# sephiroce/srf

Hardware: AMD Instinct MI355X
Metric: acoustic frames/sec through SRF (123-d fbank, 3-iter DR) at 1/2/4/8 MI355X (higher is better)
Workload: dtype fp32; 1 GPU; wsj_c4: SRF L=6 PH=CH=16 DIM=32 LPAD=RPAD=2 DR iter=3, train step (fwd+bwd+allreduce+Adam); utterances_per_gpu=28, frames_per_utterance=800, global_batch=28, parallelism=dp1, launch=hipgraph (fwd+CTC+bwd)

## Files before the change

### srf_amd/csrc/route_dr.hip

```cpp
#include <algorithm>
#include <cmath>
#include <type_traits>

#include "srf_common.h"
#include "route_fwd32.h"
#include "../../include/srf.h"
#include "../../include/srf_prof.h"

namespace {

constexpr float kSquashEps = 1e-7f;

thread_local hipEvent_t* t_ev_start = nullptr;
thread_local hipEvent_t* t_ev_stop = nullptr;
thread_local int t_ev_n = 0;
constexpr int MODE_FWD = 0;
constexpr int MODE_BWD = 1;

using srf::DrGeom;

template <int KS>
__device__ __forceinline__ void load_vec(const float* __restrict__ p, float (&v)[KS]) {
  if constexpr (KS % 4 == 0) {
#pragma unroll
// ... 1402 lines not shown
  static_assert(VW == 0 || VW == 2, "0: per-lane loads, 2: image shared by two waves");
  constexpr int D = 32, RV = R - 1, NV = R + RV;
  constexpr int NG = VW == 2 ? 2 : 1;
  constexpr int NT = 256 * NG, CAPW = CAP * NG;
  constexpr int CG = RV * 2 * 4 * 16;
  constexpr int PQ = CG / 4 + 128;
  constexpr int PCB = CG * 4 + 2 * D * 16 * 2;
  constexpr int NQ = (CAPW * PQ + NT - 1) / NT;
  constexpr int IMG = NV * D * 16;
  __shared__ __attribute__((aligned(16))) unsigned char stg[2][CAPW * PCB];
  __shared__ __attribute__((aligned(16))) float vimg[VW == 0 ? 4 : 2 * 4 * IMG];
  const int JD = J * D;
  const size_t FJD = (size_t)F * JD;
  const int Fs = srf::fwd32_frame_stride(F);
  const size_t cblk = (size_t)in_n * JP * Fs;
  const int lane = threadIdx.x & 63, wv = (threadIdx.x >> 6) & 3, wg = threadIdx.x >> 8;
  const int n = lane & 31, h = lane >> 5;
#if SRF_GW16S_XCD
  const int n_cc = (in_n + CAPW - 1) / CAPW, n_tasks = n_cc * n_rt * S;
  const int task = (int)(blockIdx.x & 7) * (int)(gridDim.x >> 3) + (int)(blockIdx.x >> 3);
  if (task >= n_tasks) return;
  const int cc = task % n_cc;
  const int rtg = (task / n_cc) % n_rt;
  const int s = task / n_cc / n_rt;
#else
  int b = blockIdx.x;
  const int s = b % S;
  b /= S;
  const int rtg = b % n_rt;
  const int cc = b / n_rt;
#endif
  const int jw = rtg * 4 + wv;
  const bool wave_on = jw < J;
  const int j = min(jw, J - 1);
  const int row = j * D + n;
  const int Jeff = J - (mask_first ? 1 : 0);
  const float c0 = (wave_on && !(mask_first && j == 0)) ? 1.f / (float)Jeff : 0.f;
  const int i0 = cc * CAPW, ncap = min(in_n, i0 + CAPW) - i0, k0 = wg * CAP;
  const int NFT = Fp >> 4;
  const int ft0 = s * ft_per, ft1 = min(NFT, ft0 + ft_per);
  const int bx = (int)hdr[2];
  const int eg = srf_split_exp(*gumax);
  const float sg = srf_exp2i(eg);

  constexpr int NCPL = CAPW * CG / 4;
  const char* src[NQ];
  int dst[NQ];
  bool cpl[NQ];
#pragma unroll
  for (int q = 0; q < NQ; ++q) {
    const int idx = min(q * NT + (int)threadIdx.x, CAPW * PQ - 1);
    cpl[q] = (q + 1) * NT <= NCPL || (q * NT < NCPL && idx < NCPL);
    if (cpl[q]) {
      const int k = idx / (CG / 4), rem = idx - k * (CG / 4);
      const int i = i0 + min(k, ncap - 1);
      const int fq = rem & 3, jq = (rem >> 2) & 3, cg = rem >> 4;
      const int jj = min(rtg * 4 + jq, JP - 1);
      src[q] = reinterpret_cast<const char*>(((cg & 1) ? glst : cst) + (size_t)(cg >> 1) * cblk +
                                             ((size_t)i * JP + jj) * Fs + 4 * fq);
      dst[q] = k * PCB + rem * 16;
    } else {
      const int x = idx - NCPL, k = x >> 7, xr = x & 127;
      const int p = xr >> 6, e = (xr >> 1) & 31, hf = xr & 1;
      const int i = i0 + min(k, ncap - 1);
      src[q] = reinterpret_cast<const char*>(x16 + (((size_t)i * NFT * 2 + p) * 32 + e) * 16 + hf * 8);
      dst[q] = k * PCB + CG * 4 + p * (D * 16 * 2) + (e * 16 + ((hf ^ ((e >> 3) & 1)) * 8)) * 2;
    }
  }
  f4 sv[NQ];
  auto stage_load = [&](int ft) {
#pragma unroll
    for (int q = 0; q < NQ; ++q) sv[q] = *reinterpret_cast<const f4*>(src[q] + (size_t)ft * (cpl[q] ? 64 : 2 * 32 * 16 * 2));
  };
  auto stage_store = [&](int buf) {
#pragma unroll
    for (int q = 0; q < NQ; ++q) {
      const int idx = q * NT + threadIdx.x;
      if ((CAPW * PQ) % NT != 0 && idx >= CAPW * PQ) continue;
      *reinterpret_cast<f4*>(&stg[buf][dst[q]]) = cpl[q] ? sv[q] * sg : sv[q];
    }
  };
  const uint32_t nrec = (uint32_t)(FJD * 4);
  __amdgpu_buffer_rsrc_t rs_g[R], rs_v[RV];
#pragma unroll
  for (int r = 0; r < R; ++r) {
    rs_g[r] = __builtin_amdgcn_make_buffer_rsrc(const_cast<float*>(gs + (size_t)r * FJD), 0, (int)nrec, 0x00020000);
    if (r > 0)
      rs_v[r - 1] = __builtin_amdgcn_make_buffer_rsrc(const_cast<float*>(saved + (size_t)(2 * (r - 1) + 1) * FJD), 0,
                                                      (int)nrec, 0x00020000);
  }
  const uint32_t vo0 = (uint32_t)((8 * h) * JD + row) * 4;
  f2 nxa[NV][4], nxb[NV][4];
  auto vec_load = [&](f2 (&nx)[NV][4], int ft) {
#pragma unroll
    for (int v = 0; v < 8; ++v) {
      const uint32_t so = (uint32_t)((ft * 16 + v) * JD) * 4;
#pragma unroll
      for (int r = 0; r < R; ++r) {
        nx[r][v >> 1][v & 1] = __builtin_bit_cast(float, __builtin_amdgcn_raw_buffer_load_b32(rs_g[r], vo0, so, 0));
        if (r > 0) nx[R + r - 1][v >> 1][v & 1] = __builtin_bit_cast(float, __builtin_amdgcn_raw_buffer_load_b32(rs_v[r - 1], vo0, so, 0));
      }
    }
  };
  const int rq = lane & 7, fm = lane >> 3;
  const uint32_t wo0 = (uint32_t)((8 * wg + fm) * JD + j * D + 4 * rq) * 4;
  f4 vst[NV];
  auto img_load = [&](int ft) {
    const uint32_t so = (uint32_t)(ft * 16 * JD) * 4;
#pragma unroll
    for (int r = 0; r < R; ++r) {
      vst[r] = __builtin_bit_cast(f4, __builtin_amdgcn_raw_buffer_load_b128(rs_g[r], wo0, so, 0));
      if (r > 0) vst[R + r - 1] = __builtin_bit_cast(f4, __builtin_amdgcn_raw_buffer_load_b128(rs_v[r - 1], wo0, so, 0));
    }
  };
  const int iwo = 4 * rq * 16 + 4 * ((2 * wg + (fm >> 2)) ^ (rq & 3)) + (fm & 3);
  const int iro = n * 16 + 4 * ((2 * h) ^ ((n >> 2) & 3));
  auto img_store = [&](float* im, int v) {
#pragma unroll
    for (int c = 0; c < 4; ++c) im[v * (D * 16) + iwo + c * 16] = vst[v][c];
  };
  auto img_read = [&](const float* im, f2 (&nx)[NV][4]) {
#pragma unroll
    for (int v = 0; v < NV; ++v) {
      const f4 a = ld4(im + v * (D * 16) + iro), b = ld4(im + v * (D * 16) + (iro ^ 4));
      nx[v][0] = f2{a[0], a[1]}, nx[v][1] = f2{a[2], a[3]}, nx[v][2] = f2{b[0], b[1]}, nx[v][3] = f2{b[2], b[3]};
    }
  };

  f16v acc[CAP];
  float gb[CAP];
#pragma unroll
  for (int k = 0; k < CAP; ++k) {
    gb[k] = 0.f;
    acc[k] = f16v{};
  }
  float* const imw = vimg + wv * IMG;
  if (ft0 < ft1) {
    stage_load(ft0);
    if constexpr (VW == 0) vec_load(nxa, ft0);
    else img_load(ft0);
    stage_store(0);
    if (ft0 + 1 < ft1) stage_load(ft0 + 1);
    if constexpr (VW == 2) {
#pragma unroll
      for (int v = 0; v < NV; ++v) img_store(imw, v);
      img_load(min(ft0 + 1, ft1 - 1));
    }
  }
  const int xoff = CG * 4 + (n * 16 + ((h ^ ((n >> 3) & 1)) * 8)) * 2;
  const float s0 = c0 * sg;
  auto caps = [&](int buf, const f2 (&g0)[4], const f2 (&cur)[NV][4], bool img_next) {
    const unsigned char* sb = stg[buf] + k0 * PCB;
#pragma unroll
    for (int k = 0; k < CAP; ++k) {
      const unsigned char* ck = sb + k * PCB;
      const float* ckf = reinterpret_cast<const float*>(ck);
      f2 gu[4];
#pragma unroll
      for (int v = 0; v < 4; ++v) gu[v] = g0[v];
#pragma unroll
      for (int r = 0; r < RV; ++r) {
        const float* cp = ckf + ((r * 2 + 0) * 4 + wv) * 16 + 8 * h;
        const float* gp = ckf + ((r * 2 + 1) * 4 + wv) * 16 + 8 * h;
        const f4 ca = ld4(cp), cb = ld4(cp + 4), ga = ld4(gp), gbv = ld4(gp + 4);
        const f2 c2[4] = {f2{ca[0], ca[1]}, f2{ca[2], ca[3]}, f2{cb[0], cb[1]}, f2{cb[2], cb[3]}};
        const f2 g2[4] = {f2{ga[0], ga[1]}, f2{ga[2], ga[3]}, f2{gbv[0], gbv[1]}, f2{gbv[2], gbv[3]}};
#pragma unroll
        for (int v = 0; v < 4; ++v) {
          gu[v] = __builtin_elementwise_fma(c2[v], cur[r + 1][v], gu[v]);
          gu[v] = __builtin_elementwise_fma(g2[v], cur[R + r][v], gu[v]);
        }
      }
      const f2 gq = (gu[0] + gu[1]) + (gu[2] + gu[3]);
      gb[k] += gq[0] + gq[1];
      h8 bh, bl;
      split8h(gu, bh, bl);
      const h8 xh = *reinterpret_cast<const h8*>(ck + xoff);
      const h8 xl = *reinterpret_cast<const h8*>(ck + xoff + D * 16 * 2);
      acc[k] = mfma32h(xh, bh, acc[k]);
      acc[k] = mfma32h(xh, bl, acc[k]);
      acc[k] = mfma32h(xl, bh, acc[k]);
      if constexpr (VW == 2) {
        if (img_next) {
#pragma unroll
          for (int v = 0; v < NV; ++v)
            if (v * CAP / NV == k) img_store(imw + (buf ^ 1) * (4 * IMG), v);
        }
      }
    }
  };
  auto tile = [&](auto bufc, const f2 (&cur)[NV][4], f2 (&nxt)[NV][4], int ft) {
    constexpr int buf = decltype(bufc)::value;
    f2 g0[4];
#pragma unroll
    for (int v = 0; v < 4; ++v) g0[v] = cur[0][v] * s0;
    __syncthreads();
    if (ft + 1 < ft1) {
      stage_store(buf ^ 1);
      if (ft + 2 < ft1) stage_load(ft + 2);
    }
    vec_load(nxt, ft + 1 < ft1 ? ft + 1 : ft);
    caps(buf, g0, cur, false);
  };
  auto tile_img = [&](auto bufc, int ft) {
    constexpr int buf = decltype(bufc)::value;
    f2 cur[NV][4], g0[4];
    __syncthreads();
    img_read(imw + buf * (4 * IMG), cur);
    if (ft + 1 < ft1) {
      stage_store(buf ^ 1);
      if (ft + 2 < ft1) stage_load(ft + 2);
    }
#pragma unroll
    for (int v = 0; v < 4; ++v) g0[v] = cur[0][v] * s0;
    caps(buf, g0, cur, ft + 1 < ft1);
    __builtin_amdgcn_sched_barrier(0);
    img_load(min(ft + 2, ft1 - 1));
  };
  using S0 = std::integral_constant<int, 0>;
  using S1 = std::integral_constant<int, 1>;
  for (int ft = ft0; ft < ft1; ft += 2) {
    if constexpr (VW == 0) tile(S0{}, nxa, nxb, ft);
    else tile_img(S0{}, ft);
    if (ft + 1 >= ft1) break;
    if constexpr (VW == 0) tile(S1{}, nxb, nxa, ft + 1);
    else tile_img(S1{}, ft + 1);
  }
  float* gw = gwp + (size_t)s * pstride;
  float* gbo = gbp + (size_t)s * pstride;
  const float un = srf_exp2i(-(bx + eg)), ug = srf_exp2i(-eg);
#pragma unroll
  for (int k = 0; k < CAP; ++k) {
    const float a = gb[k];
    float pa, pb;
    xpair32(a, pa, pb);
    if (k0 + k >= ncap || !wave_on) continue;
    const int i = i0 + k0 + k;
    if (h == 0) gbo[(size_t)i * JD + row] = (pa + pb) * ug;
#pragma unroll
    for (int q = 0; q < 4; ++q)
      st4(gw + ((size_t)i * JD + row) * D + 8 * q + 4 * h,
          f4{acc[k][4 * q] * un, acc[k][4 * q + 1] * un, acc[k][4 * q + 2] * un, acc[k][4 * q + 3] * un});
  }
}

__global__ void gw_reduce_kernel(const float* __restrict__ part, int S, size_t n4, size_t stride, float* __restrict__ gW,
                                 size_t nw4, float* __restrict__ gb) {
  const size_t idx = (size_t)blockIdx.x * blockDim.x + threadIdx.x;
  if (idx >= n4) return;
  f4 a = ld4(part + idx * 4);
  for (int s = 1; s < S; ++s) a += ld4(part + (size_t)s * stride + idx * 4);
  if (idx < nw4)
    st4(gW + idx * 4, a);
  else
    st4(gb + (idx - nw4) * 4, a);
}

template <int Q>
__device__ __forceinline__ float qsum(float v) {
#pragma unroll
  for (int o = 1; o < Q; o <<= 1) v += __shfl_xor(v, o, 64);
  return v;
}

struct SlabSplit {
  int n;
  int G, U, in_n, JD;
};

__device__ __forceinline__ int slab_count(const SlabSplit& sp, size_t FJD, size_t off) {
  if (sp.G <= 0) return sp.n;
  const uint32_t f = FJD <= 0xffffffffu ? (uint32_t)off / (uint32_t)sp.JD : (uint32_t)(off / (size_t)sp.JD);
  return srf::bal_tile_slots((int)(f >> 5), sp.in_n, sp.U, sp.G);
}

__device__ __forceinline__ f4 sum_slab4(const float* __restrict__ slab, const SlabSplit& sp, size_t FJD, size_t off) {
  const int n = slab_count(sp, FJD, off);
  f4 a = ld4(slab + off);
#pragma unroll 4
  for (int c = 1; c < n; ++c) a += ld4(slab + (size_t)c * FJD + off);
  return a;
}

template <int DOUT>
__global__ void fwd_finish_kernel(const float* __restrict__ slab, SlabSplit sp, size_t FJD,
                                  const float* __restrict__ vc_in, float* __restrict__ s_out,
                                  float* __restrict__ vc_out, float* __restrict__ v_out) {
  constexpr int Q = DOUT / 4;
  const size_t idx = (size_t)blockIdx.x * blockDim.x + threadIdx.x;
  const bool ok = idx < FJD / 4;
  const size_t off = (ok ? idx : 0) * 4;
  const f4 sv = sum_slab4(slab, sp, FJD, off);
  const float n2 = qsum<Q>((sv.x * sv.x + sv.y * sv.y) + (sv.z * sv.z + sv.w * sv.w));
  if (!ok) return;
  const float fac = n2 / (1.f + n2) / sqrtf(n2 + kSquashEps);
  const f4 v = sv * fac;
  st4(s_out + off, sv);
  if (vc_out) st4(vc_out + off, vc_in ? v + ld4(vc_in + off) : v);
  if (v_out) st4(v_out + off, v);
}

template <int DOUT>
__global__ void bwd_finish_kernel(const float* __restrict__ slab, SlabSplit sp, size_t FJD,
                                  const float* __restrict__ a_init, float* __restrict__ A,
                                  const float* __restrict__ s, float* __restrict__ gs, float* __restrict__ zero4,
                                  size_t nz4, float* __restrict__ zero1) {
  constexpr int Q = DOUT / 4;
  const size_t idx = (size_t)blockIdx.x * blockDim.x + threadIdx.x;
  if (idx < nz4) st4(zero4 + idx * 4, f4{0.f, 0.f, 0.f, 0.f});
  if (zero1 != nullptr && idx == 0) *zero1 = 0.f;
  const bool ok = idx < FJD / 4;
  const size_t off = (ok ? idx : 0) * 4;
  f4 a;
  if (a_init) {
    a = ld4(a_init + off);
    if (ok) st4(A + off, f4{0.f, 0.f, 0.f, 0.f});
  } else {
    a = ld4(A + off) + sum_slab4(slab, sp, FJD, off);
    if (ok) st4(A + off, a);
  }
  const f4 sv = ld4(s + off);
  const float n2 = qsum<Q>((sv.x * sv.x + sv.y * sv.y) + (sv.z * sv.z + sv.w * sv.w));
  const float sa = qsum<Q>((sv.x * a.x + sv.y * a.y) + (sv.z * a.z + sv.w * a.w));
  if (!ok) return;
  const float rs = 1.f / sqrtf(n2 + kSquashEps);
  const float ip = 1.f / (1.f + n2);
  const float gfac = n2 * ip * rs;
  const float dg2 = 2.f * rs * ip * (ip - 0.5f * n2 / (n2 + kSquashEps)) * sa;
  st4(gs + off, a * gfac + sv * dg2);
}

struct PassCfg {
  int TW, NW;
};

PassCfg pass_cfg(const DrGeom& g) {
  const int NT = g.NT();
  int TW = 8;
  int NW = (NT + TW - 1) / TW;
  if (NW > 8) {
    TW = 16;
    NW = (NT + TW - 1) / TW;
  }
  return {TW, NW};
}

int auto_chunks(const DrGeom& g, int NW) {
  const int n_ftiles = (g.F() + 15) / 16;
  const int wg_per_cu = std::max(1, 8 / NW);
  const int slots = 256 * wg_per_cu;
  int best = 1;
  double best_cost = 1e30;
  for (int c = 1; c <= std::min(g.in_n(), 96); ++c) {
    const int rounds = (n_ftiles * c + slots - 1) / slots;
    const int len = (g.in_n() + c - 1) / c;
    double cost = (double)rounds * (len + 2);
    if (8 % c != 0 && c % 8 != 0) cost *= 1.05;
    cost *= 1.0 + 0.002 * c;
    if (cost < best_cost) {
      best_cost = cost;
      best = c;
    }
  }
  return best;
}

template <int D, int TW, int MODE>
void launch_pass(const DrGeom& g, int NW, int n_chunks, const float* emb, const float* W, const float* bias, int r,
                 const float* vc, const float* gsv, float* slab, float* stats, int want_acc, hipStream_t st) {
  const int n_ftiles = (g.F() + 15) / 16;
  const int chunk_len = (g.in_n() + n_chunks - 1) / n_chunks;
  const size_t shmem = (NW > 1) ? (size_t)2 * NW * 48 * sizeof(float) : 16;
  auto kern = r == 0 ? route_pass_kernel<D, D, TW, MODE, true> : route_pass_kernel<D, D, TW, MODE, false>;
  hipLaunchKernelGGL(kern, dim3(n_ftiles * n_chunks), dim3(64 * NW), shmem, st,
                     emb, W, bias, g.F(), g.T, g.N, g.lpad, g.in_n(), g.J, n_chunks, chunk_len, g.mask_first, r,
                     vc, gsv, slab, stats, want_acc);
}

template <int D, int MODE>
void dispatch_pass(const DrGeom& g, const PassCfg& pc, int n_chunks, const float* emb, const float* W,
                   const float* bias, int r, const float* vc, const float* gsv, float* slab, float* stats,
                   int want_acc, hipStream_t st) {
  if (pc.TW == 8)
    launch_pass<D, 8, MODE>(g, pc.NW, n_chunks, emb, W, bias, r, vc, gsv, slab, stats, want_acc, st);
  else
    launch_pass<D, 16, MODE>(g, pc.NW, n_chunks, emb, W, bias, r, vc, gsv, slab, stats, want_acc, st);
}

template <int D>
void launch_fwd_finish(const DrGeom& g, const float* slab, const SlabSplit& sp, const float* vc_in, float* s_out,
                       float* vc_out, float* v_out, hipStream_t st) {
  const size_t FJD = (size_t)g.F() * g.JD();
  hipLaunchKernelGGL((fwd_finish_kernel<D>), dim3((FJD / 4 + 255) / 256), dim3(256), 0, st, slab, sp, FJD,
                     vc_in, s_out, vc_out, v_out);
}

template <int D>
void launch_bwd_finish(const DrGeom& g, const float* slab, const SlabSplit& sp, const float* a_init, float* A,
                       const float* s, float* gs, hipStream_t st, float* zero = nullptr, size_t n_zero = 0,
                       float* zero1 = nullptr) {
  const size_t FJD = (size_t)g.F() * g.JD();
  const size_t nz4 = zero ? n_zero / 4 : 0;
  const size_t n = std::max(FJD / 4, nz4);
  hipLaunchKernelGGL((bwd_finish_kernel<D>), dim3((n + 255) / 256), dim3(256), 0, st, slab, sp, FJD, a_init,
                     A, s, gs, zero, nz4, zero1);
}

constexpr int gu_tw(int d) { return d >= 64 ? 4 : 2; }
constexpr int kGuNW = 4;

inline int gu_wgroups(const DrGeom& g) { return (g.NT() + kGuNW * gu_tw(g.dout) - 1) / (kGuNW * gu_tw(g.dout)); }
inline int padded_frames(const DrGeom& g) { return (g.F() + 15) / 16 * 16; }
inline int gu_window(const DrGeom& g) { return g.lpad + g.rpad + 1; }
inline size_t gu_lds_bytes(const DrGeom& g, int nw, int n_per) {
  return (size_t)nw * (15 + gu_window(g)) * gu_row_stride(n_per, g.din) * sizeof(float);
}
constexpr size_t kGuLdsMax = 64 * 1024;

int gu_n_per(const DrGeom& g, int nw) {
  const int base = (g.F() + 15) / 16 * gu_wgroups(g);
  const int slots = 256 * 4;
  int best = 1;
  double best_cost = 1e30;
  for (int n_per = 1; n_per <= g.N; ++n_per) {
    if (n_per > 1 && gu_lds_bytes(g, nw, n_per) > kGuLdsMax) break;
    const int chunks = (g.N + n_per - 1) / n_per;
    const int rounds = (base * chunks + slots - 1) / slots;
    const double cost = (double)rounds * (gu_window(g) * n_per + 4);
    if (cost < best_cost) {
      best_cost = cost;
      best = n_per;
    }
  }
  return best;
}

inline size_t gux16_lds_bytes(const DrGeom& g, int n_per) {
  return (size_t)kGux16NW * (31 + gu_window(g)) * (n_per * 32 + 4) * sizeof(float);
}
constexpr size_t kGux16LdsMax = (160 / kGux16Occ - 4) * 1024;
int gux16_n_per(const DrGeom& g, int jgpw) {
  const int base = (g.F() + 31) / 32 * ((g.J + kGux16NW - 1) / kGux16NW / jgpw);
  const int slots = 256 * kGux16Occ;
  int best = 1;
  double best_cost = 1e30;
  for (int n_per = 1; n_per <= g.N; ++n_per) {
    if (n_per > 1 && gux16_lds_bytes(g, n_per) > kGux16LdsMax) break;
    const int chunks = (g.N + n_per - 1) / n_per;
    const int rounds = (base * chunks + slots - 1) / slots;
    const double cost = (double)rounds * (gu_window(g) * n_per * jgpw + 4);
    if (cost < best_cost) {
      best_cost = cost;
      best = n_per;
    }
  }
  return best;
}

struct Gw2Plan {
  int cap, n_rt, n_cc, S, ft_per;
  size_t pstride;
};
constexpr int gw3_capsules(int d) { return d <= 16 ? 8 : 4; }

enum class GxPass {
  kRecompute,
  kStored,
  kStored16,
};
enum class GwPass {
  kFromGu,
  kGw2,
  kGw3,
  kGw16s,
};

struct BwdWs {
  size_t A, gs, slab, stats, gu_t, xT, WT;
  size_t gumax;
  size_t p32;
  size_t gl;
  size_t gwpart;
  size_t bytes;
};

struct DrPlan {
  DrGeom g;
  bool fwd32;
  srf::Fwd32Plan p32;
  srf::Fwd32Cpl cpl;
  Gw2Plan gw2;
  bool can_store;
  bool couplings;
  PassCfg pc;
  int chunks;
  int plan_arg;
  GxPass gx;
  GwPass gw;
  size_t fwd_bytes;
  BwdWs ws;
  int JP() const { return p32.JDp / g.dout; }
  const float* hdr(const float* cpl_base) const { return srf::fwd32_hdr(p32, cpl_base + cpl.planes); }
};

#ifndef SRF_GUX16_JGPW
#define SRF_GUX16_JGPW 2
#endif
template <int R>
void launch_gux16(const DrGeom& g, const float* WT, const float* hdr, const float* saved, const float* gs,
                  float* g_emb, const float* cst, const float* glst, int JP, float* gumax, hipStream_t st) {
  const int n_all = (g.J + kGux16NW - 1) / kGux16NW;
  const int jgpw = n_all % SRF_GUX16_JGPW == 0 ? SRF_GUX16_JGPW : 1;
  const int n_wgroups = n_all / jgpw;
  const int n_per = gux16_n_per(g, jgpw);
  const int n_chunks = (g.N + n_per - 1) / n_per;
  int grid = (g.F() + 31) / 32 * n_wgroups * n_chunks;
  if (SRF_GUX16_XCD) grid = (grid + 7) / 8 * 8;
  hipLaunchKernelGGL((route_gux16_kernel<R>), dim3(grid), dim3(64 * kGux16NW), gux16_lds_bytes(g, n_per), st, WT, hdr,
                     g.F(), g.T, g.N, g.lpad, g.in_n(), g.J, g.mask_first, n_wgroups, n_chunks, n_per, saved, gs, g_emb,
                     cst, glst, JP, gumax, jgpw);
}

template <int D, int R>
void launch_gu(const DrPlan& p, const float* emb, const float* W, const float* WT, const float* bias,
               const float* saved, const float* gs, const float* stats, float* gu_t, float* g_emb, hipStream_t st,
               const float* cst, const float* glst, const float* hdr, float* gumax) {
  const DrGeom& g = p.g;
  if constexpr (D == 32 && R >= 2 && R <= 4) {
    if (p.gx == GxPass::kStored16) {
      launch_gux16<R>(g, WT, hdr, saved, gs, g_emb, cst, glst, p.JP(), gumax, st);
      return;
    }
  }
  const int n_ftiles = (g.F() + 15) / 16;
  const int n_wgroups = gu_wgroups(g);
  constexpr int TW = gu_tw(D);
  const int nw = std::min(kGuNW, (g.NT() + TW - 1) / TW);
  const int n_per = gu_n_per(g, nw);
  const int n_chunks = (g.N + n_per - 1) / n_per;
  const int nslots = 15 + gu_window(g);
  const size_t lds = gu_lds_bytes(g, nw, n_per);
  if constexpr (R >= 2 && D <= 32) {
    if (p.gx == GxPass::kStored) {
      hipLaunchKernelGGL((route_gux_kernel<D, TW, R>), dim3(n_ftiles * n_wgroups * n_chunks), dim3(64 * nw), lds, st,
                         WT, g.F(), g.T, g.N, g.lpad, g.in_n(), g.J, g.mask_first, n_wgroups, n_chunks, n_per, saved,
                         gs, g_emb, nslots, cst, glst, p.JP());
      return;
    }
  }
  const bool ldsacc = lds <= kGuLdsMax;
  hipLaunchKernelGGL((ldsacc ? route_gu_kernel<D, D, TW, R, true> : route_gu_kernel<D, D, TW, R, false>),
                     dim3(n_ftiles * n_wgroups * n_chunks), dim3(64 * nw), ldsacc ? lds : 0, st, emb, W, WT, bias, g.F(),
                     padded_frames(g), g.T, g.N, g.lpad, g.rpad, g.in_n(), g.J, g.mask_first, n_wgroups, n_chunks, n_per,
                     saved, gs, stats, gu_t, g_emb, nslots, nullptr, nullptr, 0);
}

template <int V>
using Int = std::integral_constant<int, V>;

template <class Fn>
auto dispatch_iters(int iters, Fn&& fn) {
  switch (iters) {
    case 1: return fn(Int<1>{});
    case 2: return fn(Int<2>{});
    case 3: return fn(Int<3>{});
    case 4: return fn(Int<4>{});
    default: return fn(Int<5>{});
  }
}
template <class Fn>
int dispatch_din(int din, Fn&& fn) {
  switch (din) {
    case 8: return fn(Int<8>{});
    case 16: return fn(Int<16>{});
    case 32: return fn(Int<32>{});
    default: return fn(Int<64>{});
  }
}

template <int D>
int launch_gw2(const DrPlan& pl, const float* xT, const float* saved, const float* gs, const float* cst,
               const float* glst, float* gwp, float* gbp, hipStream_t st, const float* hdr, const float* gumax) {
  static_assert(D <= 32, "couplings are stored by the 32x32 forward");
  const DrGeom& g = pl.g;
  const Gw2Plan& p = pl.gw2;
  const int JP = pl.JP(), Fp = padded_frames(g);
  const int grid = p.n_rt * p.n_cc * p.S;
  if constexpr (D == 32) {
    if (pl.gw == GwPass::kGw16s) {
      constexpr int VW = SRF_GW16S_LDSVEC, NG = VW == 2 ? 2 : 1;
      const int tasks = p.n_rt * ((p.n_cc + NG - 1) / NG) * p.S;
      const int grid16 = SRF_GW16S_XCD ? (tasks + 7) / 8 * 8 : tasks;
      const _Float16* x16 = reinterpret_cast<const _Float16*>(xT);
      hipLaunchKernelGGL((g.iters == 2 ? route_gw16s_kernel<2, kGw16Cap, VW> : route_gw16s_kernel<3, kGw16Cap, VW>),
                         dim3(grid16), dim3(256 * NG), 0, st, x16, hdr, gumax, saved, gs, cst, glst, g.F(), Fp, g.in_n(),
                         g.J, g.mask_first, JP, p.n_rt, p.S, p.ft_per, gwp, gbp, p.pstride);
      SRF_LAUNCH_CHECK("route_gw16s");
      return SRF_OK;
    }
  }
  if (pl.gw == GwPass::kGw3) {
    constexpr int CAP = gw3_capsules(D);
    hipLaunchKernelGGL((g.iters == 2 ? route_gw3_kernel<D, 2, CAP> : route_gw3_kernel<D, 3, CAP>), dim3(grid), dim3(256),
                       0, st, xT, saved, gs, cst, glst, g.F(), Fp, g.in_n(), g.J, g.mask_first, JP, p.n_rt, p.S, p.ft_per,
                       gwp, gbp, p.pstride);
    SRF_LAUNCH_CHECK("route_gw3");
    return SRF_OK;
  }
  hipLaunchKernelGGL((g.iters == 4 ? route_gw2_kernel<D, 4> : route_gw2_kernel<D, 5>), dim3(grid), dim3(256), 0, st, xT,
                     saved, gs, cst, glst, g.F(), Fp, g.in_n(), g.J, g.mask_first, JP, p.n_rt, p.n_cc, p.S, p.ft_per, gwp,
                     gbp, p.pstride);
  SRF_LAUNCH_CHECK("route_gw2");
  return SRF_OK;
}


inline bool use_fwd32(const DrGeom& g) { return srf::fwd32_supported(g.din, g.dout, g.J); }

inline bool use_gux16(const DrGeom& g) {
  return g.din == 32 && g.dout == 32 && g.iters >= 2 && g.iters <= 4 &&
         gux16_lds_bytes(g, 1) <= kGux16LdsMax;
}
inline bool use_gw16s(const DrGeom& g) { return use_gux16(g) && g.iters <= 3; }

inline int gw3_cap(const DrGeom& g) { return g.iters <= 3 && g.din <= 32 ? gw3_capsules(g.din) : 0; }

Gw2Plan gw2_plan(const DrGeom& g, GwPass kind) {
  const bool g16 = kind == GwPass::kGw16s, g3 = kind == GwPass::kGw3;
  Gw2Plan p{};
  const int NT = g.NT();
  const int NCT = g16 ? 2 : (g.din + 15) / 16;
  p.n_rt = g16 ? (g.J + 3) / 4 : (NT + 3) / 4;
  p.cap = g16 ? kGw16Cap : g3 ? gw3_capsules(g.din) : (g.din <= 16 ? 8 : 4);
  const int slots = g16 ? 512 : g3 ? 2 * 768 : 512;
  const double per_tile = g16 ? 120.0 : 200.0;
  p.n_cc = (g.in_n() + p.cap - 1) / p.cap;
  const int NFT = padded_frames(g) / 16;
  p.pstride = (size_t)g.in_n() * g.JD() * (g.din + 1);
  const int base = p.n_rt * p.n_cc;
  double best = 1e30;
  for (int S0 = 1; S0 <= NFT; ++S0) {
    const int ft_per = (NFT + S0 - 1) / S0;
    const int S = (NFT + ft_per - 1) / ft_per;
    const int rounds = (base * S + slots - 1) / slots;
    const double work = (double)rounds * ft_per * p.cap * NCT * per_tile / 2.4e9;
    const double slab = S > 1 ? 2.0 * S * p.pstride * 4 / 4e12 : 0.0;
    if (work + slab < best) {
      best = work + slab;
      p.S = S;
      p.ft_per = ft_per;
    }
  }
  return p;
}

inline bool couplings_ok(const DrGeom& g, const srf::Fwd32Cpl& cpl) {
  if (!use_fwd32(g) || g.iters < 2 || g.din > 32) return false;
  constexpr size_t kLim = size_t(1) << 31;
  const int TW = gu_tw(g.dout);
  const int nw = std::min(kGuNW, (g.NT() + TW - 1) / TW);
  return gu_lds_bytes(g, nw, 1) <= kGuLdsMax && cpl.total * 4 < kLim && (size_t)g.F() * g.JD() * 4 * g.iters < kLim;
}

inline bool plan_balanced(int n_chunks) { return n_chunks > 0 && (n_chunks & srf::kBalFlag) != 0; }
inline bool plan_arg_ok(const DrPlan& p, int n_chunks) {
  return plan_balanced(n_chunks) ? p.fwd32 : (n_chunks >= 1 && n_chunks <= p.g.in_n());
}

void resolve(DrPlan& p, const DrGeom& g, int n_chunks, bool have_couplings) {
  p = DrPlan{};
  p.g = g;
  p.fwd32 = use_fwd32(g);
  p.pc = pass_cfg(g);
  p.chunks = plan_balanced(n_chunks) ? auto_chunks(g, p.pc.NW) : n_chunks;
  p.fwd_bytes = plan_balanced(n_chunks) ? 0 : (size_t)n_chunks * ((size_t)g.B * g.T + 1) * g.J * g.dout * sizeof(float);
  GwPass stored_gw = GwPass::kGw2;
  if (p.fwd32) {
    p.p32 = srf::fwd32_plan(g, n_chunks);
    p.fwd_bytes = std::max(p.fwd_bytes, srf::fwd32_workspace(p.p32));
    p.cpl = srf::fwd32_cpl_layout(p.p32, g);
    stored_gw = use_gw16s(g) ? GwPass::kGw16s : gw3_cap(g) ? GwPass::kGw3 : GwPass::kGw2;
    p.gw2 = gw2_plan(g, stored_gw);
  }
  p.plan_arg = p.fwd32 ? p.p32.plan_arg : n_chunks == 0 ? auto_chunks(g, p.pc.NW) : p.chunks;
  p.can_store = couplings_ok(g, p.cpl);
  p.couplings = have_couplings && p.can_store;
  p.gx = !p.couplings ? GxPass::kRecompute : use_gux16(g) ? GxPass::kStored16 : GxPass::kStored;
  p.gw = p.couplings ? stored_gw : GwPass::kFromGu;

  const size_t F = g.F(), JD = g.JD(), in_n = g.in_n(), Fp = padded_frames(g);
  size_t off = 0;
  auto take = [&](size_t nfloat) {
    const size_t o = off;
    off += srf::align_up(nfloat * sizeof(float), 256);
    return o / sizeof(float);
  };
  BwdWs& w = p.ws;
  w.A = take(F * JD);
  w.gs = take((size_t)g.iters * F * JD);
  w.slab = take((size_t)p.chunks * F * JD);
  w.stats = take((size_t)(g.iters - 1) * F * in_n * 2);
  w.gu_t = take(in_n * (size_t)g.NT() * 16 * Fp);
  w.xT = take(in_n * g.din * Fp);
  w.WT = take(in_n * JD * g.din);
  w.gumax = take(64);
  if (p.fwd32) {
    w.p32 = take((srf::fwd32_scratch_bytes(p.p32) + 3) / 4);
    w.gl = take((size_t)std::max(g.iters - 1, 1) * srf::fwd32_frame_stride(g.F()) * in_n * p.JP());
    w.gwpart = take((size_t)p.gw2.S * p.gw2.pstride);
  }
  w.bytes = off;
}

int check_geom(const DrGeom& g) {
  SRF_REQUIRE(g.B > 0 && g.T > 0 && g.N > 0 && g.J > 1, "bad shape B=%d T=%d N=%d J=%d", g.B, g.T, g.N, g.J);
  SRF_REQUIRE(g.lpad >= 0 && g.rpad >= 0, "negative window pad");
  SRF_REQUIRE(g.iters >= 1 && g.iters <= 5, "routing iterations must be in [1,5], got %d", g.iters);
  SRF_REQUIRE(g.din == 8 || g.din == 16 || g.din == 32 || g.din == 64, "unsupported in_d %d", g.din);
  SRF_REQUIRE(g.dout == g.din, "in_d (%d) != out_d (%d) is not supported", g.din, g.dout);
  SRF_REQUIRE((long long)g.F() * g.in_n() * g.JD() < (1LL << 40), "problem too large");
  return SRF_OK;
}

inline SlabSplit uniform_split(int n) { return SlabSplit{n, 0, 0, 0, 0}; }
inline SlabSplit pass_split(const DrGeom& g, const srf::Fwd32Plan& p) {
  return p.bal_G > 0 ? SlabSplit{p.n_slots, p.bal_G, p.bal_U, g.in_n(), g.JD()} : uniform_split(p.n_chunks);
}

template <int D>
int fwd_impl(const DrPlan& p, const float* emb, const float* W, const float* bias, float* v_out, float* saved,
             float* couplings, float* slab, hipStream_t st) {
  const DrGeom& g = p.g;
  const srf::Fwd32Plan& plan = p.p32;
  const srf::Fwd32Cpl& cl = p.cpl;
  const size_t FJD = (size_t)g.F() * g.JD();
  hipEvent_t* ev0 = t_ev_start;
  hipEvent_t* ev1 = t_ev_stop;
  const int nev = t_ev_n;
  t_ev_start = t_ev_stop = nullptr;
  t_ev_n = 0;
  float* bsum = nullptr;
  void* planes = slab;
  void* scratch = slab;
  if (p.fwd32) {
    float *WT = nullptr, *xT = nullptr;
    if (p.couplings) {
      planes = couplings + cl.planes;
      WT = couplings + cl.WT;
      xT = couplings + cl.xT;
    } else {
      scratch = static_cast<char*>(static_cast<void*>(slab)) + srf::fwd32_planes_bytes(plan);
    }
    const int rc = srf::fwd32_prepare(plan, g, emb, W, bias, planes, scratch, WT, xT, st,
                                      p.gx == GxPass::kStored16, p.gw == GwPass::kGw16s);
    if (rc) return rc;
  } else {
    bsum = slab + (size_t)p.chunks * FJD;
    const int chunk_len = (g.in_n() + p.chunks - 1) / p.chunks;
    hipLaunchKernelGGL(bias_chunk_sum_kernel, dim3((p.chunks * g.JD() + 255) / 256), dim3(256), 0, st, bias,
                       g.in_n(), g.JD(), p.chunks, chunk_len, bsum);
    SRF_LAUNCH_CHECK("bias_chunk_sum");
  }
  for (int r = 0; r < g.iters; ++r) {
    const float* vc = r > 0 ? saved + (size_t)(2 * (r - 1) + 1) * FJD : nullptr;
    if (r < nev) SRF_HIP_TRY(hipEventRecord(ev0[r], st));
    if (p.fwd32 && r == 0 && srf::fwd32_first_full_supported(plan, g)) {
      const int rc = srf::fwd32_first_full(plan, g, planes, scratch, saved, saved + FJD,
                                           g.iters == 1 ? v_out : nullptr, st);
      if (rc) return rc;
      if (r < nev) SRF_HIP_TRY(hipEventRecord(ev1[r], st));
      continue;
    }
    if (p.fwd32) {
      float *cst = nullptr, *lzst = nullptr;
      if (p.couplings && r > 0) {
        const size_t blk = (size_t)srf::fwd32_frame_stride(g.F()) * g.in_n();
        cst = couplings + cl.c + (size_t)(r - 1) * blk * p.JP();
        lzst = couplings + cl.lz + (size_t)(r - 1) * blk;
      }
      const int rc = srf::fwd32_pass(plan, g, r == 0, planes, scratch, vc, cst, lzst, st);
      if (rc) return rc;
    } else {
      dispatch_pass<D, MODE_FWD>(g, p.pc, p.chunks, emb, W, bias, r, vc, r == 0 ? bsum : nullptr, slab, nullptr, 1, st);
    }
    SRF_LAUNCH_CHECK("route_pass(fwd)");
    if (r < nev) SRF_HIP_TRY(hipEventRecord(ev1[r], st));
    const bool last = r == g.iters - 1;
    launch_fwd_finish<D>(g, p.fwd32 ? srf::fwd32_slab(plan, scratch) : slab,
                         !p.fwd32 ? uniform_split(p.chunks) : r == 0 ? uniform_split(plan.n_chunks) : pass_split(g, plan),
                         vc, saved + (size_t)(2 * r) * FJD, last ? nullptr : saved + (size_t)(2 * r + 1) * FJD,
                         last ? v_out : nullptr, st);
    SRF_LAUNCH_CHECK("fwd_finish");
  }
  return SRF_OK;
}

template <int D>
int bwd_weights_impl(const DrPlan& p, const float* emb, float* g_W, float* g_bias, float* ws, hipStream_t st,
                     const float* saved, const float* couplings) {
  const DrGeom& g = p.g;
  const BwdWs& w = p.ws;
  const int Fp = padded_frames(g);
  if constexpr (D <= 32) {
    if (p.gw != GwPass::kFromGu) {
      const Gw2Plan& gp = p.gw2;
      const bool direct = gp.S == 1;
      float* gwp = direct ? g_W : ws + w.gwpart;
      float* gbp = direct ? g_bias : ws + w.gwpart + (size_t)g.in_n() * g.JD() * g.din;
      const int rc = launch_gw2<D>(p, couplings + p.cpl.xT, saved, ws + w.gs, couplings + p.cpl.c, ws + w.gl, gwp, gbp,
                                   st, p.hdr(couplings), ws + w.gumax);
      if (rc || direct) return rc;
      const size_t nw4 = (size_t)g.in_n() * g.JD() * g.din / 4, n4 = gp.pstride / 4;
      hipLaunchKernelGGL(gw_reduce_kernel, dim3((n4 + 255) / 256), dim3(256), 0, st, ws + w.gwpart, gp.S, n4,
                         gp.pstride, g_W, nw4, g_bias);
      SRF_LAUNCH_CHECK("gw_reduce");
      return SRF_OK;
    }
  }
  {
    SRF_REQUIRE(g.din <= 64, "window_xt tile holds din <= 64, got %d", g.din);
    const int tiles = (Fp + kXtFrames - 1) / kXtFrames;
    hipLaunchKernelGGL(window_xt_kernel, dim3(g.in_n() * tiles), dim3(256), 0, st, emb, g.F(), Fp, g.T, g.N, g.din,
                       g.lpad, g.in_n(), ws + w.xT);
    SRF_LAUNCH_CHECK("window_xt");
  }
  {
    const int tasks = g.in_n() * g.NT();
    hipLaunchKernelGGL((route_gw_kernel<D>), dim3((tasks + 3) / 4), dim3(256), 0, st, ws + w.gu_t, ws + w.xT, Fp,
                       g.in_n(), g.JD(), g_W, g_bias);
    SRF_LAUNCH_CHECK("route_gw");
  }
  return SRF_OK;
}

template <int D>
int bwd_impl(const DrPlan& p, const float* emb, const float* W, const float* bias, const float* saved,
             const float* couplings, const float* g_v, float* g_emb, float* g_W, float* g_bias, float* ws,
             hipStream_t st, bool with_weights) {
  const DrGeom& g = p.g;
  const BwdWs& w = p.ws;
  const srf::Fwd32Plan& plan = p.p32;
  const srf::Fwd32Cpl& cl = p.cpl;
  const size_t FJD = (size_t)g.F() * g.JD();
  const int R = g.iters;
  const bool p32 = p.couplings;
  float* const gsv = ws + w.gs;
  const size_t n_emb = (size_t)g.F() * g.N * g.din;
  launch_bwd_finish<D>(g, nullptr, uniform_split(1), g_v, ws + w.A, saved + (size_t)(2 * (R - 1)) * FJD,
                       gsv + (size_t)(R - 1) * FJD, st, p32 ? g_emb : nullptr, n_emb, p32 ? ws + w.gumax : nullptr);
  SRF_LAUNCH_CHECK("bwd_finish");
  for (int r = R - 1; r >= 1; --r) {
    const float* vc = saved + (size_t)(2 * (r - 1) + 1) * FJD;
    float* stats_r = ws + w.stats + (size_t)(r - 1) * g.F() * g.in_n() * 2;
    if (p32) {
      const size_t blk = (size_t)srf::fwd32_frame_stride(g.F()) * g.in_n();
      const int JP = p.JP();
      const int rc = srf::bwd32_pass(plan, g, couplings + cl.planes, ws + w.p32,
                                     couplings + cl.c + (size_t)(r - 1) * blk * JP,
                                     couplings + cl.lz + (size_t)(r - 1) * blk, gsv + (size_t)r * FJD, stats_r,
                                     ws + w.gl + (size_t)(r - 1) * blk * JP, st);
      if (rc) return rc;
      launch_bwd_finish<D>(g, srf::fwd32_slab(plan, ws + w.p32), pass_split(g, plan), nullptr, ws + w.A,
                           saved + (size_t)(2 * (r - 1)) * FJD, gsv + (size_t)(r - 1) * FJD, st);
    } else {
      dispatch_pass<D, MODE_BWD>(g, p.pc, p.chunks, emb, W, bias, r, vc, gsv + (size_t)r * FJD, ws + w.slab, stats_r, 1,
                                 st);
      SRF_LAUNCH_CHECK("route_pass(bwd)");
      launch_bwd_finish<D>(g, ws + w.slab, uniform_split(p.chunks), nullptr, ws + w.A,
                           saved + (size_t)(2 * (r - 1)) * FJD, gsv + (size_t)(r - 1) * FJD, st);
    }
    SRF_LAUNCH_CHECK("bwd_finish");
  }
  if (!p32) {
    const size_t total = (size_t)g.in_n() * g.JD() * g.din + n_emb;
    hipLaunchKernelGGL(transpose_w_kernel, dim3((total + 255) / 256), dim3(256), 0, st, W, g.in_n(), g.JD(), g.din,
                       ws + w.WT, g_emb, n_emb);
    SRF_LAUNCH_CHECK("transpose_w");
  }
  dispatch_iters(R, [&](auto r) {
    launch_gu<D, r>(p, emb, W, p32 ? couplings + cl.WT : ws + w.WT, bias, saved, gsv, ws + w.stats, ws + w.gu_t, g_emb,
                    st, p32 ? couplings + cl.c : nullptr, p32 ? ws + w.gl : nullptr,
                    p32 ? p.hdr(couplings) : nullptr, ws + w.gumax);
  });
  SRF_LAUNCH_CHECK("route_gu");
  return with_weights ? bwd_weights_impl<D>(p, emb, g_W, g_bias, ws, st, saved, couplings) : SRF_OK;
}

int enter(DrPlan& p, const DrGeom& g, int n_chunks, bool pointers, bool have_couplings, bool forward,
          size_t workspace_bytes) {
  if (const int rc = check_geom(g)) return rc;
  SRF_REQUIRE(pointers, "null pointer argument");
  resolve(p, g, n_chunks, have_couplings);
  SRF_REQUIRE(plan_arg_ok(p, n_chunks), "n_chunks %d: neither in [1, %d] nor a balanced plan of the 32x32 passes",
              n_chunks, g.in_n());
  const size_t need = forward ? p.fwd_bytes : p.ws.bytes;
  if (workspace_bytes < need) {
    srf::set_error("%s workspace too small: %zu < %zu", forward ? "forward" : "backward", workspace_bytes, need);
    return SRF_EWORKSPACE;
  }
  return SRF_OK;
}

int route_dr_bwd_entry(const float* emb, const float* W, const float* bias, int B, int T, int N, int din, int lpad,
                       int rpad, int J, int dout, int iters, int mask_first, int n_chunks, const float* saved,
                       const float* couplings, const float* g_v, float* g_emb, float* g_W, float* g_bias,
                       void* workspace, size_t workspace_bytes, void* stream, bool with_weights) {
  DrPlan p;
  const int rc = enter(p, DrGeom{B, T, N, din, lpad, rpad, J, dout, iters, mask_first ? 1 : 0}, n_chunks,
                       emb && W && bias && saved && g_v && g_emb && g_W && g_bias && workspace, couplings != nullptr,
                       false, workspace_bytes);
  if (rc) return rc;
  return dispatch_din(din, [&](auto D) {
    return bwd_impl<D>(p, emb, W, bias, saved, couplings, g_v, g_emb, g_W, g_bias, static_cast<float*>(workspace),
                       static_cast<hipStream_t>(stream), with_weights);
  });
}

DrPlan query(int B, int T, int N, int din, int lpad, int rpad, int J, int dout, int iters, int n_chunks) {
  DrPlan p;
  resolve(p, DrGeom{B, T, N, din, lpad, rpad, J, dout, iters, 0}, n_chunks, false);
  return p;
}

}

extern "C" {

int srf_route_dr_set_timing_events(void* const* starts, void* const* stops, int n) {
  SRF_REQUIRE(n >= 0 && (n == 0 || (starts && stops)), "bad timing event arrays");
  t_ev_start = (hipEvent_t*)starts;
  t_ev_stop = (hipEvent_t*)stops;
  t_ev_n = n;
  return SRF_OK;
}

int srf_route_dr_auto_chunks(int B, int T, int N, int din, int lpad, int rpad, int J, int dout) {
  return query(B, T, N, din, lpad, rpad, J, dout, 1, 0).plan_arg;
}

int srf_route_dr_split_table(int B, int T, int N, int din, int lpad, int rpad, int J, int dout, int n_chunks,
                             int* info, int* table, int capacity) {
  const bool shape_ok = B > 0 && T > 0 && N > 0 && lpad >= 0 && rpad >= 0;
  const DrPlan plan = shape_ok ? query(B, T, N, din, lpad, rpad, J, dout, 1, n_chunks) : DrPlan{};
  SRF_REQUIRE(shape_ok && plan.fwd32, "split_table: not a 32x32-pass shape");
  SRF_REQUIRE(n_chunks == 0 || plan_arg_ok(plan, n_chunks), "split_table: bad plan argument %d", n_chunks);
  SRF_REQUIRE(info != nullptr && capacity >= 0 && (table != nullptr || capacity == 0), "split_table: null argument");
  const srf::Fwd32Plan& p = plan.p32;
  const int in_n = plan.g.in_n();
  const bool bal = p.bal_G > 0;
  const int n_wg = bal ? p.bal_G : p.n_ftiles * p.n_chunks;
  info[0] = bal ? 1 : 0;
  info[1] = n_wg;
  info[2] = p.n_ftiles * in_n;
  info[3] = p.n_slots;
  info[4] = p.plan_arg;
  int n = 0;
  auto emit = [&](int w, int ft, int i0, int i1, int slot) {
    if (n < capacity) {
      int* row = table + (size_t)n * 5;
      row[0] = w, row[1] = ft, row[2] = i0, row[3] = i1, row[4] = slot;
    }
    ++n;
  };
  for (int w = 0; w < n_wg; ++w) {
    if (!bal) {
      const int ft = w / p.n_chunks, slot = w - ft * p.n_chunks;
      const int i0 = slot * p.chunk_len;
      emit(w, ft, std::min(i0, in_n), std::min(in_n, i0 + p.chunk_len), slot);
      continue;
    }
    int u = srf::bal_first(w, p.bal_U, p.bal_G);
    const int u1 = srf::bal_first(w + 1, p.bal_U, p.bal_G);
    while (u < u1) {
      const int ft = u / in_n, i0 = u - ft * in_n, i1 = std::min(in_n, i0 + (u1 - u));
      emit(w, ft, i0, i1, w - srf::bal_owner(ft * in_n, p.bal_U, p.bal_G));
      u += i1 - i0;
    }
  }
  return n;
}

size_t srf_route_dr_saved_floats(int B, int T, int J, int dout, int iters) {
  return (size_t)2 * iters * B * T * J * dout;
}

size_t srf_route_dr_fwd_workspace(int B, int T, int N, int din, int lpad, int rpad, int J, int dout, int iters,
                                  int n_chunks) {
  (void)iters;
  return query(B, T, N, din, lpad, rpad, J, dout, 1, n_chunks).fwd_bytes;
}

size_t srf_route_dr_bwd_workspace(int B, int T, int N, int din, int lpad, int rpad, int J, int dout, int iters,
                                  int n_chunks) {
  return query(B, T, N, din, lpad, rpad, J, dout, iters, n_chunks).ws.bytes;
}

size_t srf_route_dr_coupling_floats(int B, int T, int N, int din, int lpad, int rpad, int J, int dout, int iters) {
  const DrPlan p = query(B, T, N, din, lpad, rpad, J, dout, iters, 0);
  return p.can_store ? p.cpl.total : 0;
}

int srf_route_dr_operand_layout(int B, int T, int N, int din, int lpad, int rpad, int J, int dout, int iters,
                                long long* out) {
  SRF_REQUIRE(out != nullptr, "operand_layout: null argument");
  DrPlan p;
  const DrGeom g{B, T, N, din, lpad, rpad, J, dout, iters, 0};
  if (const int rc = check_geom(g)) return rc;
  resolve(p, g, 0, true);
  if (!p.couplings) {
    srf::set_error("operand_layout: no coupling storage for this shape");
    return SRF_EUNSUPPORTED;
  }
  const srf::Fwd32Shape& s = p.p32;
  const size_t in_n = g.in_n(), Fp = padded_frames(g);
  const size_t pl = p.cpl.planes;
  const size_t v[SRF_DR_LAYOUT_N] = {pl,
                                     2 * in_n * s.JDp * g.din * 2,
                                     pl + s.ws_w / 4,
                                     in_n * s.JDp * 8,
                                     pl + (s.ws_w + s.ws_b) / 4,
                                     2 * s.xplane * 2,
                                     pl + (s.ws_w + s.ws_b + s.ws_x) / 4,
                                     3 * sizeof(float),
                                     p.cpl.WT,
                                     in_n * g.din * ((size_t)g.NT() * 16) * 4,
                                     p.cpl.xT,
                                     in_n * g.din * Fp * 4,
                                     (size_t)s.JDp,
                                     s.xplane,
                                     Fp,
                                     p.gx == GxPass::kStored16 ? 1u : 0u,
                                     p.gw == GwPass::kGw16s ? 1u : 0u};
  for (int k = 0; k < SRF_DR_LAYOUT_N; ++k) out[k] = (long long)v[k];
  return SRF_OK;
}

int srf_route_dr_fwd(const float* emb, const float* W, const float* bias, int B, int T, int N, int din, int lpad,
                     int rpad, int J, int dout, int iters, int mask_first, int n_chunks, float* v_out, float* saved,
                     void* workspace, size_t workspace_bytes, void* stream) {
  return srf_route_dr_fwd_ex(emb, W, bias, B, T, N, din, lpad, rpad, J, dout, iters, mask_first, n_chunks, v_out,
                             saved, nullptr, workspace, workspace_bytes, stream);
}

int srf_route_dr_fwd_ex(const float* emb, const float* W, const float* bias, int B, int T, int N, int din, int lpad,
                        int rpad, int J, int dout, int iters, int mask_first, int n_chunks, float* v_out,
                        float* saved, float* couplings, void* workspace, size_t workspace_bytes, void* stream) {
  DrPlan p;
  const int rc = enter(p, DrGeom{B, T, N, din, lpad, rpad, J, dout, iters, mask_first ? 1 : 0}, n_chunks,
                       emb && W && bias && v_out && saved && workspace, couplings != nullptr, true, workspace_bytes);
  if (rc) return rc;
  return dispatch_din(din, [&](auto D) {
    return fwd_impl<D>(p, emb, W, bias, v_out, saved, couplings, static_cast<float*>(workspace),
                       static_cast<hipStream_t>(stream));
  });
}

int srf_route_dr_bwd(const float* emb, const float* W, const float* bias, int B, int T, int N, int din, int lpad,
                     int rpad, int J, int dout, int iters, int mask_first, int n_chunks, const float* saved,
                     const float* g_v, float* g_emb, float* g_W, float* g_bias, void* workspace,
                     size_t workspace_bytes, void* stream) {
  return route_dr_bwd_entry(emb, W, bias, B, T, N, din, lpad, rpad, J, dout, iters, mask_first, n_chunks, saved,
                            nullptr, g_v, g_emb, g_W, g_bias, workspace, workspace_bytes, stream, true);
}

int srf_route_dr_bwd_ex(const float* emb, const float* W, const float* bias, int B, int T, int N, int din, int lpad,
                        int rpad, int J, int dout, int iters, int mask_first, int n_chunks, const float* saved,
                        const float* couplings, const float* g_v, float* g_emb, float* g_W, float* g_bias,
                        void* workspace, size_t workspace_bytes, void* stream) {
  return route_dr_bwd_entry(emb, W, bias, B, T, N, din, lpad, rpad, J, dout, iters, mask_first, n_chunks, saved,
                            couplings, g_v, g_emb, g_W, g_bias, workspace, workspace_bytes, stream, true);
}

int srf_route_dr_bwd_data(const float* emb, const float* W, const float* bias, int B, int T, int N, int din,
                          int lpad, int rpad, int J, int dout, int iters, int mask_first, int n_chunks,
                          const float* saved, const float* g_v, float* g_emb, void* workspace,
                          size_t workspace_bytes, void* stream) {
  return srf_route_dr_bwd_data_ex(emb, W, bias, B, T, N, din, lpad, rpad, J, dout, iters, mask_first, n_chunks, saved,
                                  nullptr, g_v, g_emb, workspace, workspace_bytes, stream);
}

int srf_route_dr_bwd_data_ex(const float* emb, const float* W, const float* bias, int B, int T, int N, int din,
                             int lpad, int rpad, int J, int dout, int iters, int mask_first, int n_chunks,
                             const float* saved, const float* couplings, const float* g_v, float* g_emb,
                             void* workspace, size_t workspace_bytes, void* stream) {
  float* unused = reinterpret_cast<float*>(workspace);
  return route_dr_bwd_entry(emb, W, bias, B, T, N, din, lpad, rpad, J, dout, iters, mask_first, n_chunks, saved,
                            couplings, g_v, g_emb, unused, unused, workspace, workspace_bytes, stream, false);
}

int srf_route_dr_bwd_weights(const float* emb, int B, int T, int N, int din, int lpad, int rpad, int J, int dout,
                             int iters, int mask_first, int n_chunks, float* g_W, float* g_bias, void* workspace,
                             size_t workspace_bytes, void* stream) {
  return srf_route_dr_bwd_weights_ex(emb, B, T, N, din, lpad, rpad, J, dout, iters, mask_first, n_chunks, nullptr,
                                     nullptr, g_W, g_bias, workspace, workspace_bytes, stream);
}

int srf_route_dr_bwd_weights_ex(const float* emb, int B, int T, int N, int din, int lpad, int rpad, int J, int dout,
                                int iters, int mask_first, int n_chunks, const float* saved, const float* couplings,
                                float* g_W, float* g_bias, void* workspace, size_t workspace_bytes, void* stream) {
  DrPlan p;
  const int rc = enter(p, DrGeom{B, T, N, din, lpad, rpad, J, dout, iters, mask_first ? 1 : 0}, n_chunks,
                       emb && g_W && g_bias && workspace, couplings != nullptr && saved != nullptr, false,
                       workspace_bytes);
  if (rc) return rc;
  return dispatch_din(din, [&](auto D) {
    return bwd_weights_impl<D>(p, emb, g_W, g_bias, static_cast<float*>(workspace),
                               static_cast<hipStream_t>(stream), saved, couplings);
  });
}

}
```

### srf_amd/csrc/route_fwd32.h

```cpp
#pragma once
#include <hip/hip_runtime.h>
#include <cstddef>
#include <cstdint>

namespace srf {

struct DrGeom {
  int B, T, N, din, lpad, rpad, J, dout, iters, mask_first;
  int F() const { return B * T; }
  int in_n() const { return N * (lpad + rpad + 1); }
  int JD() const { return J * dout; }
  int NT() const { return (J * dout + 15) / 16; }
};

constexpr int kFwd32TW = 4;
__host__ __device__ inline int fwd32_frame_stride(int F) { return (F + 31) / 32 * 32; }

__host__ __device__ inline int bal_first(int w, int U, int G) {
  return (int)((uint32_t)w * (uint32_t)U / (uint32_t)G);
}
__host__ __device__ inline int bal_owner(int u, int U, int G) {
  return (int)((((uint32_t)u + 1u) * (uint32_t)G - 1u) / (uint32_t)U);
}
__host__ __device__ inline int bal_tile_slots(int ft, int in_n, int U, int G) {
  return bal_owner((ft + 1) * in_n - 1, U, G) - bal_owner(ft * in_n, U, G) + 1;
}
constexpr int kBalFlag = 1 << 20;

struct Fwd32Shape {
  int NW;
  int TW;
  int JDp;
  int xpad;
  int n_ftiles;
  size_t xplane;
  size_t ws_w, ws_b, ws_x, ws_h;
};
struct Fwd32Split {
  int n_chunks, chunk_len;
  int bal_G, bal_U;
  int n_slots;
  int plan_arg;
  size_t ws_bsum, ws_slab;
};
struct Fwd32Plan : Fwd32Shape, Fwd32Split {};

bool fwd32_supported(int din, int dout, int J);
Fwd32Plan fwd32_plan(const DrGeom& g, int n_chunks = 0);
size_t fwd32_planes_bytes(const Fwd32Shape& p);
size_t fwd32_scratch_bytes(const Fwd32Split& p);
size_t fwd32_workspace(const Fwd32Plan& p);
size_t fwd32_lds(const Fwd32Shape& p);
float* fwd32_slab(const Fwd32Split& p, void* scratch);
const float* fwd32_hdr(const Fwd32Shape& p, const void* planes);
int fwd32_prepare(const Fwd32Plan& p, const DrGeom& g, const float* emb, const float* W, const float* bias,
                  void* planes, void* scratch, float* WT, float* xT, hipStream_t st, bool wt16 = false,
                  bool xt16 = false);
int fwd32_pass(const Fwd32Plan& p, const DrGeom& g, bool first, const void* planes, void* scratch, const float* vc,
               float* cst, float* lzst, hipStream_t st);
bool fwd32_first_full_supported(const Fwd32Shape& p, const DrGeom& g);
int fwd32_first_full(const Fwd32Plan& p, const DrGeom& g, const void* planes, void* scratch, float* s_out,
                     float* vc_out, float* v_out, hipStream_t st);
struct Fwd32Cpl {
  size_t c, lz, planes, WT, xT, total;
};
Fwd32Cpl fwd32_cpl_layout(const Fwd32Shape& p, const DrGeom& g);
int bwd32_pass(const Fwd32Plan& p, const DrGeom& g, const void* planes, void* scratch, const float* cst,
               const float* lz, const float* gs, float* stats, float* glst, hipStream_t st);

}
```

### srf_amd/csrc/route_fwd32.hip

```cpp
#include <cmath>
#include <cstdint>
#include <cstdlib>
#include <algorithm>
#include <type_traits>

#include "srf_common.h"
#include "route_fwd32.h"


#ifndef SRF_DR_IL
#define SRF_DR_IL 1
#endif

#ifndef SRF_DR_BAL_AUTO
#define SRF_DR_BAL_AUTO 1
#endif

#ifndef SRF_PREP32_ONEPASS
#define SRF_PREP32_ONEPASS 1
#endif

namespace {

typedef __bf16 bf8 __attribute__((ext_vector_type(8)));
// ... 170 lines not shown
  }
  if (blk == 0 && tid < 8) {
    const h8 z = {};
    *reinterpret_cast<h8*>(P.xs + (size_t)(tid >> 2) * P.xplane + (P.xplane - 32) + (tid & 3) * 8) = z;
  }
  const float sc = exp2i(wave_split_exp(P.part, 1));
#pragma unroll
  for (int it = 0; it < kIt; ++it) {
    const int k = tid + it * 256, r = k >> 3, e4 = k & 7;
    const int fr = f0 - P.lpad + r;
    if (r >= nrow) continue;
    uint32_t w[4];
    split4w(v[it], sc, w);
    if (P.xT) {
#pragma unroll
      for (int j = 0; j < 4; ++j) img[(4 * e4 + j) * kXImgStride + r] = w[j];
    }
    if (r >= P.lpad && r < P.lpad + kXtTile && fr < P.F) {
      _Float16* d = P.xs + ((size_t)n * P.F + fr) * 32 + 4 * e4;
      *reinterpret_cast<u2v*>(d) = u2v{pack_hi(w[0], w[1]), pack_hi(w[2], w[3])};
      *reinterpret_cast<u2v*>(d + P.xplane) = u2v{pack_lo(w[0], w[1]), pack_lo(w[2], w[3])};
    }
  }
  if (!P.xT) return;
  __syncthreads();
  const int e = tid & 31, hf = (tid >> 5) & 1, kb = tid >> 6;
  const int fb = f0 + kb * 16;
  if (fb >= P.Fp) return;
  int t8[8];
  {
    const u4v a = *reinterpret_cast<const u4v*>(&tt[kb * 16 + hf * 8]);
    const u4v b = *reinterpret_cast<const u4v*>(&tt[kb * 16 + hf * 8 + 4]);
#pragma unroll
    for (int q = 0; q < 4; ++q) t8[q] = (int)a[q] - P.lpad, t8[4 + q] = (int)b[q] - P.lpad;
  }
  _Float16* x16 = reinterpret_cast<_Float16*>(P.xT);
  const uint32_t* col = img + e * kXImgStride + kb * 16 + hf * 8;
  const int nwin = P.lpad + P.rpad + 1;
  for (int w = 0; w < nwin; ++w) {
    uint32_t c[8];
#pragma unroll
    for (int q = 0; q < 8; ++q) c[q] = (uint32_t)(t8[q] + w) < (uint32_t)P.T ? col[w + q] : 0u;
    const size_t i = (size_t)w * P.N + n;
    const size_t base = ((i * (P.Fp / 16) + fb / 16) * 2 * 32 + e) * 16 + hf * 8;
    *reinterpret_cast<u4v*>(x16 + base) =
        u4v{pack_hi(c[0], c[1]), pack_hi(c[2], c[3]), pack_hi(c[4], c[5]), pack_hi(c[6], c[7])};
    *reinterpret_cast<u4v*>(x16 + base + 32 * 16) =
        u4v{pack_lo(c[0], c[1]), pack_lo(c[2], c[3]), pack_lo(c[4], c[5]), pack_lo(c[6], c[7])};
  }
}

__device__ __forceinline__ void prep_w_rows(const PrepArgs& P, int blk, uint32_t* lds) {
  const int i = blk / P.w_bpc, rb = blk - i * P.w_bpc;
  const int lane = threadIdx.x & 63, wv = threadIdx.x >> 6;
  const int e4 = lane & 7, g = lane >> 3;
  const int rw0 = rb * 256 + wv * 64;
  const bool active = rw0 < P.JDp;
  uint32_t* const t = lds + wv * 64 * kWTileStride;
  f4 v[8];
#pragma unroll
  for (int k = 0; k < 8; ++k) {
    const int row = rw0 + g * 8 + k;
    v[k] = f4{0.f, 0.f, 0.f, 0.f};
    if (row < P.JD) v[k] = *reinterpret_cast<const f4*>(P.W + ((size_t)i * P.JD + row) * 32 + 4 * e4);
  }
  const float s = exp2i(wave_split_exp(P.part, 0));
#pragma unroll
  for (int k = 0; k < 8; ++k) {
    uint32_t w[4];
    split4w(v[k], s, w);
    *reinterpret_cast<u4v*>(t + (g * 8 + k) * kWTileStride + 4 * e4) = u4v{w[0], w[1], w[2], w[3]};
  }
  __syncthreads();
  if (!active) return;
  const size_t nw = (size_t)P.in_n * P.JDp * 32;
#pragma unroll
  for (int it = 0; it < 4; ++it) {
    const int rl = it * 16 + (lane >> 2), c8 = (lane & 3) * 8;
    const u4v a = *reinterpret_cast<const u4v*>(t + rl * kWTileStride + c8);
    const u4v b = *reinterpret_cast<const u4v*>(t + rl * kWTileStride + c8 + 4);
    _Float16* d = P.Ws + ((size_t)i * P.JDp + rw0 + rl) * 32 + c8;
    *reinterpret_cast<u4v*>(d) = u4v{pack_hi(a[0], a[1]), pack_hi(a[2], a[3]), pack_hi(b[0], b[1]), pack_hi(b[2], b[3])};
    *reinterpret_cast<u4v*>(d + nw) =
        u4v{pack_lo(a[0], a[1]), pack_lo(a[2], a[3]), pack_lo(b[0], b[1]), pack_lo(b[2], b[3])};
  }
  if (P.WT == nullptr) return;
  const int nt16 = (P.JD + 15) / 16;
  const int e = lane & 31;
#pragma unroll
  for (int it = 0; it < 4; ++it) {
    const int g2 = it * 2 + (lane >> 5);
    const int r0 = rw0 + g2 * 8;
    if (r0 >= nt16 * 16) continue;
    uint32_t c[8];
#pragma unroll
    for (int q = 0; q < 8; ++q) c[q] = t[(g2 * 8 + q) * kWTileStride + e];
    _Float16* d = reinterpret_cast<_Float16*>(P.WT) + (((size_t)i * nt16 * 2 + r0 / 8) * 32 + e) * 8;
    *reinterpret_cast<u4v*>(d) = u4v{pack_hi(c[0], c[1]), pack_hi(c[2], c[3]), pack_hi(c[4], c[5]), pack_hi(c[6], c[7])};
    *reinterpret_cast<u4v*>(d + P.n_e * 8) =
        u4v{pack_lo(c[0], c[1]), pack_lo(c[2], c[3]), pack_lo(c[4], c[5]), pack_lo(c[6], c[7])};
  }
}

__global__ __launch_bounds__(256) void prep32_onepass_kernel(PrepArgs P) {
  __shared__ __attribute__((aligned(16))) uint32_t lds[kPrepLdsWords];
  int blk = blockIdx.x;
  if (blk < P.n_xblk) return prep_x_tile(P, blk, lds);
  blk -= P.n_xblk;
  if (blk < P.n_wblk) return prep_w_rows(P, blk, lds);
  blk -= P.n_wblk;
  const int aw = wave_split_exp(P.part, 0), bx = wave_split_exp(P.part, 1);
  if (blk == 0 && threadIdx.x == 0) {
    P.hdr[0] = exp2i(-(aw + bx));
    P.hdr[1] = (float)aw;
    P.hdr[2] = (float)bx;
  }
  size_t idx = (size_t)blk * blockDim.x + threadIdx.x;
  if (idx < P.n_b) return prep_bs(P, idx, aw, bx);
  idx -= P.n_b;
  if (idx < P.n_c) prep_bsum(P, idx);
}

__global__ __launch_bounds__(256) void prep32_kernel(PrepArgs P) {
  if (P.n_f && blockIdx.x >= P.xt_block0) {
    __shared__ float tile[kXtTile][32 + 1];
    __shared__ int sbx;
    const int ntile = (P.Fp + kXtTile - 1) / kXtTile;
    const int blk = blockIdx.x - (int)P.xt_block0;
    const int i = blk / ntile, f0 = (blk - i * ntile) * kXtTile;
    const int w = i / P.N, n = i - w * P.N;
    if (P.xt16 && threadIdx.x < 64) {
      float m = 0.f;
      for (int k = threadIdx.x; k < kAbsBlocks; k += 64) m = fmaxf(m, P.part[kAbsBlocks + k]);
#pragma unroll
      for (int o = 32; o >= 1; o >>= 1) m = fmaxf(m, __shfl_xor(m, o, 64));
      if (threadIdx.x == 0) sbx = split_exp(m);
    }
    for (int k = threadIdx.x; k < kXtTile * P.din; k += blockDim.x) {
      const int fl = k / P.din, e = k - fl * P.din;
      const int f = f0 + fl;
      float v = 0.f;
      if (f < P.F) {
        const int b = f / P.T, t = f - b * P.T;
        const int ts = t + w - P.lpad;
        if (ts >= 0 && ts < P.T) v = P.emb[((size_t)(b * P.T + ts) * P.N + n) * P.din + e];
      }
      tile[fl][e] = v;
    }
    __syncthreads();
    if (P.xt16) {
      const float sc = exp2i(sbx);
      _Float16* x16 = reinterpret_cast<_Float16*>(P.xT);
      for (int k = threadIdx.x; k < (kXtTile / 16) * 32 * 2; k += blockDim.x) {
        const int hf = k & 1, e = (k >> 1) & 31, kb = k >> 6;
        const int fb = f0 + kb * 16;
        if (fb >= P.Fp) continue;
        h8 p1, p2;
#pragma unroll
        for (int q = 0; q < 8; ++q) {
          _Float16 a1, a2;
          split2h(tile[kb * 16 + hf * 8 + q][e] * sc, a1, a2);
          p1[q] = a1;
          p2[q] = a2;
        }
        const size_t base = (((size_t)i * (P.Fp / 16) + fb / 16) * 2 * 32 + e) * 16 + hf * 8;
        *reinterpret_cast<h8*>(x16 + base) = p1;
        *reinterpret_cast<h8*>(x16 + base + 32 * 16) = p2;
      }
      return;
    }
    for (int k = threadIdx.x; k < kXtTile * P.din; k += blockDim.x) {
      const int e = k / kXtTile, fl = k - e * kXtTile;
      const int f = f0 + fl;
      if (f < P.Fp) P.xT[((size_t)i * P.din + e) * P.Fp + f] = tile[fl][e];
    }
    return;
  }
  __shared__ int sexp[2];
  const size_t b0 = (size_t)blockIdx.x * blockDim.x, b1 = b0 + blockDim.x;
  const size_t ec = P.n_a + P.n_b, sd = ec + P.n_c, ed = sd + P.n_d;
  const bool split_work = b0 < ec || (b1 > sd && b0 < ed) || (P.wt16 && b1 > ed && b0 < ed + P.n_e);
  if (split_work && threadIdx.x < 128) {
    const int y = threadIdx.x >> 6, l = threadIdx.x & 63;
    float m = 0.f;
    for (int k = l; k < kAbsBlocks; k += 64) m = fmaxf(m, P.part[y * kAbsBlocks + k]);
#pragma unroll
    for (int o = 32; o >= 1; o >>= 1) m = fmaxf(m, __shfl_xor(m, o, 64));
    if (l == 0) sexp[y] = split_exp(m);
  }
  if (split_work) __syncthreads();
  const int aw = split_work ? sexp[0] : 0, bx = split_work ? sexp[1] : 0;
  if (blockIdx.x == 0 && threadIdx.x == 0) {
    P.hdr[0] = exp2i(-(aw + bx));
    P.hdr[1] = (float)aw;
    P.hdr[2] = (float)bx;
  }
  size_t idx = (size_t)blockIdx.x * blockDim.x + threadIdx.x;
  if (idx < P.n_a) {
    const size_t e0 = idx * 8;
    const int e = e0 % P.din;
    const size_t rr = e0 / P.din;
    const int row = rr % P.JDp;
    const size_t i = rr / P.JDp;
    const size_t nw = (size_t)P.in_n * P.JDp * P.din;
    split8h(P.W + (i * P.JD + min(row, P.JD - 1)) * P.din + e, row < P.JD, exp2i(aw), P.Ws + e0, P.Ws + nw + e0);
    return;
  }
  idx -= P.n_a;
  if (idx < P.n_b) {
    prep_bs(P, idx, aw, bx);
    return;
  }
  idx -= P.n_b;
  if (idx < P.n_c) {
    prep_bsum(P, idx);
    return;
  }
  idx -= P.n_c;
  if (idx < P.n_d) {
    const size_t e0 = idx * 8;
    const size_t n_data = (size_t)P.F * P.N * P.din;
    const int e = e0 % P.din;
    const size_t rr = e0 / P.din;
    const int f = rr % P.F;
    const int n = rr / P.F;
    const bool ok = e0 < n_data;
    split8h(P.emb + ((size_t)(ok ? f : 0) * P.N + (ok ? n : 0)) * P.din + (ok ? e : 0), ok, exp2i(bx), P.xs + e0,
            P.xs + P.xplane + e0);
    return;
  }
  idx -= P.n_d;
  if (P.wt16 && idx < P.n_e) {
    const int e = idx % P.din;
    const size_t r1 = idx / P.din;
    const int h = r1 % 2;
    const size_t r2 = r1 / 2;
    const int nt16 = (P.JD + 15) / 16;
    const int t = r2 % nt16;
    const size_t i = r2 / nt16;
    const int row = t * 16 + 8 * h;
    const float* w = P.W + (i * P.JD + min(row, P.JD - 1)) * P.din + e;
    const float s = exp2i(aw);
    h8 p1, p2;
#pragma unroll
    for (int k = 0; k < 8; ++k) {
      _Float16 a1, a2;
      split2h(row + k < P.JD ? w[(size_t)k * P.din] * s : 0.f, a1, a2);
      p1[k] = a1;
      p2[k] = a2;
    }
    _Float16* d = reinterpret_cast<_Float16*>(P.WT);
    *reinterpret_cast<h8*>(d + idx * 8) = p1;
    *reinterpret_cast<h8*>(d + P.n_e * 8 + idx * 8) = p2;
    return;
  }
  if (idx < P.n_e) {
    const int e = idx % P.din;
    const size_t r1 = idx / P.din;
    const int g = r1 % 4;
    const size_t r2 = r1 / 4;
    const int nt16 = (P.JD + 15) / 16;
    const int t = r2 % nt16;
    const size_t i = r2 / nt16;
    const int row = t * 16 + 4 * g;
    const float* w = P.W + (i * P.JD + min(row, P.JD - 1)) * P.din + e;
    f4 v;
#pragma unroll
    for (int q = 0; q < 4; ++q) v[q] = row + q < P.JD ? w[(size_t)q * P.din] : 0.f;
    *reinterpret_cast<f4*>(P.WT + idx * 4) = v;
    return;
  }

}

constexpr int kTW = srf::kFwd32TW;
constexpr int kMaxNW = 32 / kTW;
constexpr int kWavesPerEU = 8 / kTW;

template <int DIN>
struct SplitFrags {
  static constexpr int NA = DIN / 8;
  static constexpr int NB = DIN == 32 ? 4 : 2;
};

template <int DIN, int TW>
struct Frags32 {
  h8 a[TW][SplitFrags<DIN>::NA];
  bf8 bias[TW];
  h8 b[SplitFrags<DIN>::NB];
};

struct Rsrc3 {
  __amdgpu_buffer_rsrc_t w, b, x;
};

__device__ __forceinline__ h8 hload(__amdgpu_buffer_rsrc_t rs, uint32_t voff, uint32_t soff) {
  return __builtin_bit_cast(h8, __builtin_amdgcn_raw_buffer_load_b128(rs, voff, soff, 0));
}

__device__ __forceinline__ __amdgpu_buffer_rsrc_t make_rsrc(const void* p, size_t bytes) {
  return __builtin_amdgcn_make_buffer_rsrc(const_cast<void*>(p), 0, (int)bytes, 0x00020000);
}

constexpr uint32_t kNoStore = 0x80000000u;
__device__ __forceinline__ void bstore(__amdgpu_buffer_rsrc_t rs, float v, uint32_t voff, uint32_t soff) {
  __builtin_amdgcn_raw_buffer_store_b32(__float_as_uint(v), rs, voff, soff, 0);
}

template <int DIN>
__device__ __forceinline__ uint32_t x_voff(int i, int N, int lpad, int T, int F, int f, int ft, bool fvalid, int h,
                                           uint32_t zero_off) {
  const int w = i / N, n = i - w * N;
  const int ts = ft + w - lpad;
  const bool ok = fvalid && ts >= 0 && ts < T;
  const uint32_t o = (uint32_t)(((n * F + f + w - lpad) * DIN) * 2 + (DIN >= 16 ? 16 * h : 0));
  return ok ? o : zero_off;
}

template <int DIN>
__device__ __forceinline__ void fetch_x(const Rsrc3& rs, uint32_t xvo, int h, uint32_t xplane_b, uint32_t zero_off,
                                        h8 (&b)[SplitFrags<DIN>::NB]) {
  if constexpr (DIN == 32) {
    b[0] = hload(rs.x, xvo, 0);
    b[1] = hload(rs.x, xvo, xplane_b);
    b[2] = hload(rs.x, xvo, 32);
    b[3] = hload(rs.x, xvo, xplane_b + 32);
  } else if constexpr (DIN == 16) {
    b[0] = hload(rs.x, xvo, 0);
    b[1] = hload(rs.x, xvo, xplane_b);
  } else {
    b[0] = hload(rs.x, xvo, 0);
    b[1] = hload(rs.x, h ? zero_off : xvo, h ? 0u : xplane_b);
  }
}

template <int DIN>
__device__ __forceinline__ void fetch_w(const Rsrc3& rs, uint32_t vo, int h, uint32_t wplane_b, uint32_t wcap_b,
                                        h8 (&a)[SplitFrags<DIN>::NA]) {
  if constexpr (DIN == 32) {
    a[0] = hload(rs.w, vo, wcap_b);
    a[1] = hload(rs.w, vo, wcap_b + wplane_b);
    a[2] = hload(rs.w, vo, wcap_b + 32);
    a[3] = hload(rs.w, vo, wcap_b + wplane_b + 32);
  } else if constexpr (DIN == 16) {
    a[0] = hload(rs.w, vo, wcap_b);
    a[1] = hload(rs.w, vo, wcap_b + wplane_b);
  } else {
    a[0] = hload(rs.w, vo + (h ? wplane_b : 0), wcap_b);
  }
}

template <int DIN, int TW, bool BIAS>
__device__ __forceinline__ void fetch32(const Rsrc3& rs, uint32_t wvo, uint32_t bvo, uint32_t xvo, int h,
                                        uint32_t wplane_b, uint32_t xplane_b, uint32_t zero_off, uint32_t wcap_b,
                                        uint32_t bcap_b, Frags32<DIN, TW>& fr) {
  constexpr uint32_t TSTEP = 32 * DIN * 2;
  fetch_x<DIN>(rs, xvo, h, xplane_b, zero_off, fr.b);
#pragma unroll
  for (int t = 0; t < TW; ++t) {
    fetch_w<DIN>(rs, wvo + t * TSTEP, h, wplane_b, wcap_b, fr.a[t]);
    if constexpr (BIAS) {
      const auto v2 = __builtin_amdgcn_raw_buffer_load_b64(rs.b, bvo + t * 32 * 8, bcap_b, 0);
      fr.bias[t] = __builtin_bit_cast(bf8, (unsigned __attribute__((ext_vector_type(4)))){v2[0], v2[1], 0u, 0u});
    }
  }
}

template <int DIN>
__device__ __forceinline__ f16v pose_chain(const h8 (&a)[SplitFrags<DIN>::NA], const h8 (&b)[SplitFrags<DIN>::NB],
                                           f16v acc) {
  if constexpr (DIN == 32) {
    acc = mfma32h(a[1], b[0], acc);
    acc = mfma32h(a[3], b[2], acc);
    acc = mfma32h(a[0], b[1], acc);
    acc = mfma32h(a[2], b[3], acc);
    acc = mfma32h(a[0], b[0], acc);
    acc = mfma32h(a[2], b[2], acc);
  } else if constexpr (DIN == 16) {
    acc = mfma32h(a[1], b[0], acc);
    acc = mfma32h(a[0], b[1], acc);
    acc = mfma32h(a[0], b[0], acc);
  } else {
    acc = mfma32h(a[0], b[1], acc);
    acc = mfma32h(a[0], b[0], acc);
  }
  return acc;
}

constexpr int kXlPiece = 1024;
__device__ __forceinline__ h8 xl_read(const char* p) {
  h8 r;
  asm volatile("ds_read_b128 %0, %1" : "=v"(r) : "v"((uint32_t)reinterpret_cast<uintptr_t>(p)));
  return r;
}
template <int DIN, int TW, bool XL = false, bool XJ = false>
__device__ __forceinline__ void pose_prog(Frags32<DIN, TW>& fr, const bf8& ones, f16v (&u)[TW],
                                          const Rsrc3& rs, uint32_t wvo, uint32_t bvo, uint32_t xvo, int h,
                                          uint32_t wplane_b, uint32_t xplane_b, uint32_t zero_off, uint32_t wcap_b,
                                          uint32_t bcap_b, const char* xl = nullptr) {
  constexpr uint32_t TSTEP = 32 * DIN * 2;
  static_assert(!XJ || (XL && DIN == 32), "XJ: the shared x fragments of din 32");
  if constexpr (XJ) {
#pragma unroll
    for (int q = 0; q < 4; ++q) fr.b[q] = xl_read(xl + q * kXlPiece);
  } else if constexpr (XL) {
    asm volatile("s_waitcnt lgkmcnt(0)" : "+v"(fr.b[0]), "+v"(fr.b[1]), "+v"(fr.b[2]), "+v"(fr.b[3]));
  }
#pragma unroll
  for (int t = 0; t < TW; ++t) u[t] = mfma32(fr.bias[t], ones, f16v{});
  __builtin_amdgcn_sched_barrier(0);
  {
#pragma unroll
    for (int t = 0; t < TW; ++t) {
      const auto v2 = __builtin_amdgcn_raw_buffer_load_b64(rs.b, bvo + t * 32 * 8, bcap_b, 0);
      fr.bias[t] = __builtin_bit_cast(bf8, (unsigned __attribute__((ext_vector_type(4)))){v2[0], v2[1], 0u, 0u});
    }
  }
  __builtin_amdgcn_sched_barrier(0);
  if constexpr (XJ)
    asm volatile("s_waitcnt lgkmcnt(0)" : "+v"(fr.b[0]), "+v"(fr.b[1]), "+v"(fr.b[2]), "+v"(fr.b[3]));
  if constexpr (DIN == 32) {
#pragma unroll
    for (int t = 0; t < TW; ++t) {
      u[t] = mfma32h(fr.a[t][1], fr.b[0], u[t]);
      u[t] = mfma32h(fr.a[t][3], fr.b[2], u[t]);
    }
    __builtin_amdgcn_sched_barrier(0);
#pragma unroll
    for (int t = 0; t < TW; ++t) {
      fr.a[t][1] = hload(rs.w, wvo + t * TSTEP, wcap_b + wplane_b);
      fr.a[t][3] = hload(rs.w, wvo + t * TSTEP, wcap_b + wplane_b + 32);
    }
    __builtin_amdgcn_sched_barrier(0);
#pragma unroll
    for (int t = 0; t < TW; ++t) {
      u[t] = mfma32h(fr.a[t][0], fr.b[1], u[t]);
      u[t] = mfma32h(fr.a[t][2], fr.b[3], u[t]);
    }
    __builtin_amdgcn_sched_barrier(0);
    if constexpr (XJ) {
    } else if constexpr (XL) {
      fr.b[1] = xl_read(xl + 1 * kXlPiece);
      fr.b[3] = xl_read(xl + 3 * kXlPiece);
    } else {
      fr.b[1] = hload(rs.x, xvo, xplane_b);
      fr.b[3] = hload(rs.x, xvo, xplane_b + 32);
    }
    __builtin_amdgcn_sched_barrier(0);
#pragma unroll
    for (int t = 0; t < TW; ++t) {
      u[t] = mfma32h(fr.a[t][0], fr.b[0], u[t]);
      u[t] = mfma32h(fr.a[t][2], fr.b[2], u[t]);
    }
    __builtin_amdgcn_sched_barrier(0);
#pragma unroll
    for (int t = 0; t < TW; ++t) {
      fr.a[t][0] = hload(rs.w, wvo + t * TSTEP, wcap_b);
      fr.a[t][2] = hload(rs.w, wvo + t * TSTEP, wcap_b + 32);
    }
    if constexpr (XJ) {
    } else if constexpr (XL) {
      fr.b[0] = xl_read(xl);
      fr.b[2] = xl_read(xl + 2 * kXlPiece);
    } else {
      fr.b[0] = hload(rs.x, xvo, 0);
      fr.b[2] = hload(rs.x, xvo, 32);
    }
    __builtin_amdgcn_sched_barrier(0);
    return;
  } else if constexpr (DIN == 16) {
#pragma unroll
    for (int t = 0; t < TW; ++t) u[t] = mfma32h(fr.a[t][1], fr.b[0], u[t]);
    __builtin_amdgcn_sched_barrier(0);
    {
#pragma unroll
      for (int t = 0; t < TW; ++t) fr.a[t][1] = hload(rs.w, wvo + t * TSTEP, wcap_b + wplane_b);
    }
    __builtin_amdgcn_sched_barrier(0);
#pragma unroll
    for (int t = 0; t < TW; ++t) u[t] = mfma32h(fr.a[t][0], fr.b[1], u[t]);
    __builtin_amdgcn_sched_barrier(0);
    fr.b[1] = hload(rs.x, xvo, xplane_b);
    __builtin_amdgcn_sched_barrier(0);
  } else {
#pragma unroll
    for (int t = 0; t < TW; ++t) u[t] = mfma32h(fr.a[t][0], fr.b[1], u[t]);
    __builtin_amdgcn_sched_barrier(0);
    fr.b[1] = hload(rs.x, h ? zero_off : xvo, h ? 0u : xplane_b);
    __builtin_amdgcn_sched_barrier(0);
  }
#pragma unroll
  for (int t = 0; t < TW; ++t) u[t] = mfma32h(fr.a[t][0], fr.b[0], u[t]);
  __builtin_amdgcn_sched_barrier(0);
  {
#pragma unroll
    for (int t = 0; t < TW; ++t) fr.a[t][0] = hload(rs.w, wvo + t * TSTEP + (DIN == 8 && h ? wplane_b : 0), wcap_b);
    fr.b[0] = hload(rs.x, xvo, 0);
  }
  __builtin_amdgcn_sched_barrier(0);
}

template <int K, int V>
__device__ __forceinline__ void mfma_valu_hint() {
#pragma unroll
  for (int k = 0; k < K; ++k) {
    __builtin_amdgcn_sched_group_barrier(0x008, 1, 0);
    __builtin_amdgcn_sched_group_barrier(0x002, V, 0);
  }
}

template <int TW, int V1, int V2, int V3, class Fill>
__device__ __forceinline__ void pose_prog32i(Frags32<32, TW>& fr, const bf8& ones, f16v (&u)[TW], const Rsrc3& rs,
                                             uint32_t wvo, uint32_t bvo, uint32_t wplane_b, uint32_t wcap_b,
                                             uint32_t bcap_b, const char* xl, Fill&& fill) {
  constexpr uint32_t TSTEP = 32 * 32 * 2;
  asm volatile("s_waitcnt lgkmcnt(0)" : "+v"(fr.b[0]), "+v"(fr.b[1]), "+v"(fr.b[2]), "+v"(fr.b[3]));
  fill(std::integral_constant<int, 0>{});
#pragma unroll
  for (int t = 0; t < TW; ++t) u[t] = mfma32(fr.bias[t], ones, f16v{});
  __builtin_amdgcn_sched_barrier(0);
#pragma unroll
  for (int t = 0; t < TW; ++t) {
    const auto v2 = __builtin_amdgcn_raw_buffer_load_b64(rs.b, bvo + t * 32 * 8, bcap_b, 0);
    fr.bias[t] = __builtin_bit_cast(bf8, (unsigned __attribute__((ext_vector_type(4)))){v2[0], v2[1], 0u, 0u});
  }
  __builtin_amdgcn_sched_barrier(0);
#pragma unroll
  for (int t = 0; t < TW; ++t) {
    u[t] = mfma32h(fr.a[t][1], fr.b[0], u[t]);
    u[t] = mfma32h(fr.a[t][3], fr.b[2], u[t]);
  }
  fill(std::integral_constant<int, 1>{});
  mfma_valu_hint<2 * TW, V1>();
  __builtin_amdgcn_sched_barrier(0);
#pragma unroll
  for (int t = 0; t < TW; ++t) {
    fr.a[t][1] = hload(rs.w, wvo + t * TSTEP, wcap_b + wplane_b);
    fr.a[t][3] = hload(rs.w, wvo + t * TSTEP, wcap_b + wplane_b + 32);
  }
  __builtin_amdgcn_sched_barrier(0);
#pragma unroll
  for (int t = 0; t < TW; ++t) {
    u[t] = mfma32h(fr.a[t][0], fr.b[1], u[t]);
    u[t] = mfma32h(fr.a[t][2], fr.b[3], u[t]);
  }
  fill(std::integral_constant<int, 2>{});
  mfma_valu_hint<2 * TW, V2>();
  __builtin_amdgcn_sched_barrier(0);
  fr.b[1] = xl_read(xl + 1 * kXlPiece);
  fr.b[3] = xl_read(xl + 3 * kXlPiece);
  __builtin_amdgcn_sched_barrier(0);
#pragma unroll
  for (int t = 0; t < TW; ++t) {
    u[t] = mfma32h(fr.a[t][0], fr.b[0], u[t]);
    u[t] = mfma32h(fr.a[t][2], fr.b[2], u[t]);
  }
  fill(std::integral_constant<int, 3>{});
  mfma_valu_hint<2 * TW, V3>();
  __builtin_amdgcn_sched_barrier(0);
#pragma unroll
  for (int t = 0; t < TW; ++t) {
    fr.a[t][0] = hload(rs.w, wvo + t * TSTEP, wcap_b);
    fr.a[t][2] = hload(rs.w, wvo + t * TSTEP, wcap_b + 32);
  }
  fr.b[0] = xl_read(xl);
  fr.b[2] = xl_read(xl + 2 * kXlPiece);
  __builtin_amdgcn_sched_barrier(0);
}

__device__ __forceinline__ bf8 ones_frag(int h) {
  const __bf16 o = (__bf16)(h == 0 ? 1.f : 0.f), z = (__bf16)0.f;
  bf8 v = {o, o, o, z, z, z, z, z};
  return v;
}

template <int DOUT>
__device__ __forceinline__ constexpr int kpart(int t, int v) {
  return DOUT == 8 ? 4 * t + (v >> 2) : DOUT == 16 ? 2 * t + (v >> 3) : t;
}

struct Args32 {
  const void *Ws, *bs, *xs;
  const float* hdr;
  size_t ws_bytes, bs_bytes, xs_bytes;
  uint32_t wplane_b, xplane_b, zero_off;
  int F, T, N, lpad, in_n, J, JDp, n_chunks, chunk_len, mask_first, n_tgroups;
  const float* vc;
  const float* bsum;
  float* slab;
  float* cst;
  float* lzst;
  int JP, Fs;
  int bal_G, bal_U;
};

struct Seg32 {
  int ft, i0, i1, slot;
};

typedef const __attribute__((address_space(4))) char* kernarg_ptr;
template <class T>
__device__ __forceinline__ const __attribute__((address_space(4))) T* kernarg_reload(uint32_t off) {
  kernarg_ptr p = (kernarg_ptr)__builtin_amdgcn_kernarg_segment_ptr();
  asm volatile("" : "+s"(p));
  return (const __attribute__((address_space(4))) T*)(p + off);
}

template <class ArgsT>
__device__ __forceinline__ Seg32 seg32_at(const ArgsT& A, int bid, int u, int u1) {
  int ft, i0, i1, slot;
  if (A.bal_G > 0) {
    ft = (int)((uint32_t)u / (uint32_t)A.in_n);
    i0 = u - ft * A.in_n;
    i1 = min(A.in_n, i0 + (u1 - u));
    slot = bid - srf::bal_owner(ft * A.in_n, A.bal_U, A.bal_G);
  } else {
    ft = bid / A.n_chunks;
    slot = bid - ft * A.n_chunks;
    i0 = slot * A.chunk_len;
    i1 = min(A.in_n, i0 + A.chunk_len);
  }
  return Seg32{__builtin_amdgcn_readfirstlane(ft), __builtin_amdgcn_readfirstlane(i0),
               __builtin_amdgcn_readfirstlane(i1), __builtin_amdgcn_readfirstlane(slot)};
}

struct SegWalk {
  int u;
  __device__ __forceinline__ SegWalk(const Args32& A) : u(0) {
    if (A.bal_G > 0) u = __builtin_amdgcn_readfirstlane(srf::bal_first((int)blockIdx.x, A.bal_U, A.bal_G));
  }
  __device__ __forceinline__ Seg32 seg() const {
    const auto* K = kernarg_reload<Args32>(0);
    const int bid = blockIdx.x;
    return seg32_at(*K, bid, u, K->bal_G > 0 ? srf::bal_first(bid + 1, K->bal_U, K->bal_G) : 0);
  }
  __device__ __forceinline__ bool next(const Seg32& sg) {
    const auto* K = kernarg_reload<Args32>(0);
    if (K->bal_G <= 0) return false;
    u += sg.i1 - sg.i0;
    if (u >= __builtin_amdgcn_readfirstlane(srf::bal_first((int)blockIdx.x + 1, K->bal_U, K->bal_G))) return false;
    asm volatile("s_waitcnt vmcnt(0)" ::: "memory");
    __syncthreads();
    return true;
  }
};



constexpr int kFTW = 2;
constexpr int kFFB = 2;

template <int DIN>
struct FirstFrags {
  h8 a[kFTW][SplitFrags<DIN>::NA];
  h8 b[kFFB][SplitFrags<DIN>::NB];
};

template <int DIN, int DOUT>
__global__ __launch_bounds__(256) __attribute__((amdgpu_waves_per_eu(2))) void route_fwd32_first_kernel(Args32 A) {
  const int lane = threadIdx.x & 63, r = lane & 31, h = lane >> 5;
  int blk = blockIdx.x;
  {
    const int nb = gridDim.x, q = nb >> 3, rem = nb & 7, x = blk & 7, idx = blk >> 3;
    blk = (x < rem ? x * (q + 1) : rem * (q + 1) + (x - rem) * q) + idx;
  }
  const int task = blk * 4 + (threadIdx.x >> 6);
  const int nfp = (A.F + 32 * kFFB - 1) / (32 * kFFB);
  const int tg = task % A.n_tgroups;
  const int rest = task / A.n_tgroups;
  const int fp = rest % nfp, chunk = rest / nfp;
  if (chunk >= A.n_chunks) return;
  const int tbase = tg * kFTW;
  const int JD = A.J * DOUT;
  const Rsrc3 rs{make_rsrc(A.Ws, A.ws_bytes), make_rsrc(A.bs, A.bs_bytes), make_rsrc(A.xs, A.xs_bytes)};
  int f[kFFB], ftt[kFFB];
  bool fv[kFFB];
#pragma unroll
  for (int b = 0; b < kFFB; ++b) {
    f[b] = (fp * kFFB + b) * 32 + r;
    const int fc = min(f[b], A.F - 1);
    ftt[b] = fc - (fc / A.T) * A.T;
    fv[b] = f[b] < A.F;
  }
  const uint32_t wvo = (uint32_t)(((tbase * 32 + r) * DIN + (DIN >= 16 ? 8 * h : 0)) * 2);
  const int i0 = chunk * A.chunk_len, i1 = min(A.in_n, i0 + A.chunk_len);
  const uint32_t capb = (uint32_t)A.JDp * DIN * 2;
  constexpr uint32_t TSTEP = 32 * DIN * 2;
  f16v acc[kFTW][kFFB];
#pragma unroll
  for (int t = 0; t < kFTW; ++t)
#pragma unroll
    for (int b = 0; b < kFFB; ++b) acc[t][b] = f16v{};
  auto fetch = [&](int i, FirstFrags<DIN>& fr) {
#pragma unroll
    for (int b = 0; b < kFFB; ++b)
      fetch_x<DIN>(rs, x_voff<DIN>(i, A.N, A.lpad, A.T, A.F, f[b], ftt[b], fv[b], h, A.zero_off), h, A.xplane_b,
                   A.zero_off, fr.b[b]);
#pragma unroll
    for (int t = 0; t < kFTW; ++t) fetch_w<DIN>(rs, wvo + t * TSTEP, h, A.wplane_b, (uint32_t)i * capb, fr.a[t]);
  };
  auto mfmas = [&](const FirstFrags<DIN>& fr) {
#pragma unroll
    for (int t = 0; t < kFTW; ++t)
#pragma unroll
      for (int b = 0; b < kFFB; ++b) acc[t][b] = pose_chain<DIN>(fr.a[t], fr.b[b], acc[t][b]);
  };
  if (i0 < i1) {
    FirstFrags<DIN> f0, f1;
    fetch(i0, f0);
    int i = i0;
    for (; i + 1 < i1; i += 2) {
      fetch(i + 1, f1);
      mfmas(f0);
      if (i + 2 < i1) fetch(i + 2, f0);
      mfmas(f1);
    }
    if (i < i1) mfmas(f0);
  }
  const int Jeff = A.J - (A.mask_first ? 1 : 0);
  const float inv = A.hdr[0];
#pragma unroll
  for (int t = 0; t < kFTW; ++t)
#pragma unroll
    for (int q = 0; q < 4; ++q) {
      const int row = (tbase + t) * 32 + 8 * q + 4 * h;
      const int j = row / DOUT;
      const float c0 = (j < A.J && !(A.mask_first && j == 0)) ? 1.f / (float)Jeff : 0.f;
      if (row < JD) {
        const f4 bsv = *reinterpret_cast<const f4*>(A.bsum + (size_t)chunk * JD + row);
#pragma unroll
        for (int b = 0; b < kFFB; ++b) {
          if (!fv[b]) continue;
          f4 v = {acc[t][b][4 * q], acc[t][b][4 * q + 1], acc[t][b][4 * q + 2], acc[t][b][4 * q + 3]};
          *reinterpret_cast<f4*>(A.slab + ((size_t)chunk * A.F + f[b]) * JD + row) = (v * inv + bsv) * c0;
        }
      }
    }
}

constexpr int kFfBM = 128;
constexpr int kFfA = 2 * kFfBM * 64;
template <int BN>
constexpr int ff_stage() { return kFfA + 2 * BN * 64; }


__device__ __forceinline__ uint32_t ff_slot(int r, int c) { return (uint32_t)(4 * r + (c ^ ((r >> 2) & 3))); }

__device__ __forceinline__ void glds16(const void* src, char* lds_dst) {
  __builtin_amdgcn_global_load_lds((const __attribute__((address_space(1))) void*)src,
                                   (__attribute__((address_space(3))) void*)lds_dst, 16, 0, 0);
}

__device__ __forceinline__ void x_dma(const char* xs, uint32_t xplane_b, uint32_t xvo, int wv, char* dst) {
  const int q = __builtin_amdgcn_readfirstlane(wv) & 3;
  const char* base = xs + (q & 1) * xplane_b + (q >> 1) * 32;
  const uint32_t m0 = __builtin_amdgcn_readfirstlane((uint32_t)reinterpret_cast<uintptr_t>(dst + q * kXlPiece));
  asm volatile("s_mov_b32 m0, %0\n\ts_nop 0\n\tglobal_load_lds_dwordx4 %1, %2" ::"s"(m0), "v"(xvo), "s"(base)
               : "memory", "m0");
}
__device__ __forceinline__ int lane_asm() {
  int lid;
  asm volatile("v_mbcnt_lo_u32_b32 %0, -1, 0\n\tv_mbcnt_hi_u32_b32 %0, -1, %0" : "=v"(lid));
  return lid;
}
template <int K = 0>
__device__ __forceinline__ void xl_wait() {
  asm volatile("s_waitcnt vmcnt(%0)" ::"n"(K) : "memory");
}

template <int BN, int CPS = 1>
__global__ __launch_bounds__(64 * 2 * (BN / 32)) void route_fwd32_first_full_kernel(
    Args32 A, float* __restrict__ s_out, float* __restrict__ vc_out, float* __restrict__ v_out) {
  constexpr int NWF = BN / 32, NWV = 2 * NWF;
  constexpr int NPA = kFfA / 1024, NPB = 2 * BN * 64 / 1024, NP = NPA + NPB;
  constexpr int NPW = (NP + NWV - 1) / NWV;
  constexpr int BPP = BN / 16;
  constexpr int kCap = ff_stage<BN>();
  constexpr int kStage = CPS * kCap;
  extern __shared__ __attribute__((aligned(16))) char smem[];
  const int tid = threadIdx.x, lane = tid & 63, wv = tid >> 6;
  const int r32 = lane & 31, h = lane >> 5;
  const int n_rt = A.JDp / kFfBM;
  int blk = blockIdx.x;
  {
    const int nb = gridDim.x, q = nb >> 3, rem = nb & 7, x = blk & 7, idx = blk >> 3;
    blk = (x < rem ? x * (q + 1) : rem * (q + 1) + (x - rem) * q) + idx;
  }
  const int rt = blk % n_rt, ft = blk / n_rt;
  const int row0 = rt * kFfBM, f0 = ft * BN;
  const int wr = wv / NWF, wc = wv - wr * NWF;
  const char* Wb = static_cast<const char*>(A.Ws);
  const char* Xb = static_cast<const char*>(A.xs);
  const size_t capb = (size_t)A.JDp * 64;
  uint32_t src_o[NPW];
  const char* src_b[NPW];
  bool is_b[NPW], live[NPW];
  int bf_[NPW], btt[NPW];
  bool bok[NPW];
#pragma unroll
  for (int k = 0; k < NPW; ++k) {
    const int q = wv + k * NWV;
    live[k] = q < NP;
    is_b[k] = q >= NPA;
    if (!is_b[k]) {
      const int slot = (q & 7) * 64 + lane, r = slot >> 2, c = (slot & 3) ^ ((r >> 2) & 3);
      src_b[k] = Wb + (size_t)(q >> 3) * A.wplane_b;
      src_o[k] = (uint32_t)((row0 + r) * 64 + c * 16);
      bf_[k] = 0, btt[k] = 0, bok[k] = false;
    } else {
      const int qb = q - NPA;
      const int slot = (qb % BPP) * 64 + lane, r = slot >> 2, c = (slot & 3) ^ ((r >> 2) & 3);
      src_b[k] = Xb + (size_t)(qb / BPP) * A.xplane_b;
      src_o[k] = (uint32_t)(c * 16);
      bf_[k] = f0 + r;
      bok[k] = bf_[k] < A.F;
      const int fc = min(bf_[k], A.F - 1);
      btt[k] = fc - (fc / A.T) * A.T;
    }
  }
  auto stage = [&](int i0, int buf) {
#pragma unroll
    for (int c = 0; c < CPS; ++c) {
      const int i = min(i0 + c, A.in_n - 1);
      char* dst = smem + buf * kStage + c * kCap;
#pragma unroll
      for (int k = 0; k < NPW; ++k) {
        if (!live[k]) continue;
        const int q = wv + k * NWV;
        if (!is_b[k])
          glds16(src_b[k] + (size_t)i * capb + src_o[k], dst + q * 1024);
        else
          glds16(src_b[k] +
                     x_voff<32>(i, A.N, A.lpad, A.T, A.F, bf_[k], btt[k], bok[k] && i0 + c < A.in_n, 0,
                                A.zero_off) +
                     src_o[k],
                 dst + q * 1024);
      }
    }
  };
  auto afrag = [&](const char* base, int t, int plane, int sstep) -> h8 {
    const int r = wr * 64 + t * 32 + r32;
    return *reinterpret_cast<const h8*>(base + plane * (kFfBM * 64) + ff_slot(r, 2 * sstep + h) * 16);
  };
  auto bfrag = [&](const char* base, int plane, int sstep) -> h8 {
    const int r = wc * 32 + r32;
    return *reinterpret_cast<const h8*>(base + kFfA + plane * (BN * 64) + ff_slot(r, 2 * sstep + h) * 16);
  };
  f16v acc[2] = {f16v{}, f16v{}};
  const int n_in = A.in_n;
  stage(0, 0);
  for (int i = 0, buf = 0; i < n_in; i += CPS, buf ^= 1) {
    asm volatile("s_waitcnt vmcnt(0)" ::: "memory");
    __syncthreads();
    if (i + CPS < n_in) stage(i + CPS, buf ^ 1);
    auto frags = [&](const char* base, h8 (&b)[4], h8 (&a)[2][4]) {
#pragma unroll
      for (int s = 0; s < 4; ++s) b[s] = bfrag(base, s & 1, s >> 1);
#pragma unroll
      for (int t = 0; t < 2; ++t)
#pragma unroll
        for (int s = 0; s < 4; ++s) a[t][s] = afrag(base, t, s & 1, s >> 1);
    };
    auto pose2 = [&](const h8 (&a)[2][4], const h8 (&b)[4]) {
      constexpr int ka[6] = {1, 3, 0, 2, 0, 2}, kb[6] = {0, 2, 1, 3, 0, 2};
#pragma unroll
      for (int k = 0; k < 6; ++k)
#pragma unroll
        for (int t = 0; t < 2; ++t) acc[t] = mfma32h(a[t][ka[k]], b[kb[k]], acc[t]);
    };
    const char* base0 = smem + buf * kStage;
    h8 b0[4], a0[2][4];
    frags(base0, b0, a0);
    if constexpr (CPS == 2) {
      h8 b1[4], a1[2][4];
      __builtin_amdgcn_sched_barrier(0);
      frags(base0 + kCap, b1, a1);
      pose2(a0, b0);
#pragma unroll
      for (int k = 0; k < 12; ++k) {
        __builtin_amdgcn_sched_group_barrier(0x008, 1, 0);
        __builtin_amdgcn_sched_group_barrier(0x100, 1, 0);
      }
      __builtin_amdgcn_sched_barrier(0);
      pose2(a1, b1);
    } else {
      pose2(a0, b0);
    }
  }
  const int f = f0 + wc * 32 + r32;
  const bool fv = f < A.F;
  const int JD = A.J * 32;
  const int Jeff = A.J - (A.mask_first ? 1 : 0);
  const float inv = A.hdr[0];
#pragma unroll
  for (int t = 0; t < 2; ++t) {
    const int rbase = row0 + wr * 64 + t * 32;
    const int j = rbase / 32;
    const float c0 = (j < A.J && !(A.mask_first && j == 0)) ? 1.f / (float)Jeff : 0.f;
    f4 sv[4];
    float n2 = 0.f;
#pragma unroll
    for (int q = 0; q < 4; ++q) {
      const int row = rbase + 8 * q + 4 * h;
      f4 bs = {0.f, 0.f, 0.f, 0.f};
      if (row < JD)
        for (int ch = 0; ch < A.n_chunks; ++ch) bs += *reinterpret_cast<const f4*>(A.bsum + (size_t)ch * JD + row);
      const f4 u = {acc[t][4 * q], acc[t][4 * q + 1], acc[t][4 * q + 2], acc[t][4 * q + 3]};
      sv[q] = (u * inv + bs) * c0;
      n2 += (sv[q].x * sv[q].x + sv[q].y * sv[q].y) + (sv[q].z * sv[q].z + sv[q].w * sv[q].w);
    }
    n2 = xor32_sum(n2);
    const float fac = n2 / (1.f + n2) / sqrtf(n2 + 1e-7f);
    if (fv && rbase < JD) {
#pragma unroll
      for (int q = 0; q < 4; ++q) {
        const size_t o = (size_t)f * JD + rbase + 8 * q + 4 * h;
        *reinterpret_cast<f4*>(s_out + o) = sv[q];
        const f4 v = sv[q] * fac;
        *reinterpret_cast<f4*>(vc_out + o) = v;
        if (v_out) *reinterpret_cast<f4*>(v_out + o) = v;
      }
    }
  }
}

template <int DIN, int DOUT, int NW, int TW>
__global__ __launch_bounds__(64 * NW) __attribute__((amdgpu_waves_per_eu(kWavesPerEU))) void route_fwd32_kernel(Args32 A) {
  constexpr int CP = TW * 32 / DOUT;
  constexpr int OWN = CP / 2;
  extern __shared__ __attribute__((aligned(16))) float lds[];
  const int wv = threadIdx.x >> 6;
  const int wvu = __builtin_amdgcn_readfirstlane(wv);
  const int tbase = __builtin_amdgcn_readfirstlane(wv * TW);
  const int j0 = tbase * 32 / DOUT;
  const Rsrc3 rs{make_rsrc(A.Ws, A.ws_bytes), make_rsrc(A.bs, A.bs_bytes), make_rsrc(A.xs, A.xs_bytes)};
  if (DIN <= 16 && NW > 1 && wv >= NW / 2) __builtin_amdgcn_s_setprio(1);
  const __amdgpu_buffer_rsrc_t crs = make_rsrc(A.cst, A.cst ? (size_t)A.in_n * A.JP * A.Fs * 4 : 0);
  const __amdgpu_buffer_rsrc_t lzs = make_rsrc(A.lzst, A.cst ? (size_t)A.in_n * A.Fs * 4 : 0);

  f4* vcl = reinterpret_cast<f4*>(lds) + (size_t)tbase * 4 * 64;
  float2* st = reinterpret_cast<float2*>(lds + (size_t)NW * TW * 4 * 64 * 4);
  constexpr bool XJ = DIN == 32 && NW > 1;
  __shared__ __attribute__((aligned(16))) char xls[XJ ? 2 * 4 * kXlPiece : 16];
  const char* xs_b = static_cast<const char*>(A.xs);
  auto xbuf = [&](int c) { return xls + (c & 1) * 4 * kXlPiece; };
  for (SegWalk sw(A);;) {
  const Seg32 sg = sw.seg();
  const int ft = sg.ft, i0 = sg.i0, i1 = sg.i1;
  const int lane = lane_asm(), r = lane & 31, h = lane >> 5;
  const uint32_t wvo = (uint32_t)(((tbase * 32 + r) * DIN + (DIN >= 16 ? 8 * h : 0)) * 2);
  const uint32_t bvo = (uint32_t)((tbase * 32 + r) * 8);
  const int JD = kernarg_reload<Args32>(0)->J * DOUT;
  const int Tk = kernarg_reload<Args32>(0)->T;
  const int f = ft * 32 + r;
  const int fc = min(f, A.F - 1);
  const int fb = fc / Tk, ftt = fc - fb * Tk;
  const bool fvalid = f < A.F;
  auto xsrc = [&](int c) { return x_voff<DIN>(min(c, i1 - 1), A.N, A.lpad, A.T, A.F, f, ftt, fvalid, h, A.zero_off); };
#pragma unroll
  for (int t = 0; t < TW; ++t)
#pragma unroll
    for (int q = 0; q < 4; ++q) {
      const int row = (tbase + t) * 32 + 8 * q + 4 * h;
      f4 v = {0.f, 0.f, 0.f, 0.f};
      if (fvalid && row < JD) v = *reinterpret_cast<const f4*>(kernarg_reload<Args32>(0)->vc + (size_t)f * JD + row);
      vcl[(t * 4 + q) * 64 + lane] = v;
    }
  float mk[OWN];
#pragma unroll
  for (int a = 0; a < OWN; ++a) {
    const int j = j0 + 2 * a + h;
    mk[a] = (j < A.J && !(A.mask_first && j == 0)) ? 0.f : -INFINITY;
  }
  const bf8 ones = ones_frag(h);
  const float inv = A.hdr[0];
  f16v acc[TW];
#pragma unroll
  for (int t = 0; t < TW; ++t) acc[t] = f16v{};
  int par = 0;
  if (i0 < i1) {
    Frags32<DIN, TW> fr;
    fetch32<DIN, TW, true>(rs, wvo, bvo, x_voff<DIN>(i0, A.N, A.lpad, A.T, A.F, f, ftt, fvalid, h, A.zero_off), h,
                           A.wplane_b, A.xplane_b, A.zero_off, (uint32_t)i0 * A.JDp * DIN * 2, (uint32_t)i0 * A.JDp * 8,
                           fr);
    if constexpr (XJ) {
      x_dma(xs_b, A.xplane_b, xsrc(i0), wv, xbuf(i0));
      x_dma(xs_b, A.xplane_b, xsrc(i0 + 1), wv, xbuf(i0 + 1));
      xl_wait();
      __syncthreads();
    }
    for (int i = i0; i < i1; ++i) {
      f16v u[TW];
      f2 P2[CP];
#pragma unroll
      for (int k = 0; k < CP; ++k) P2[k] = f2{0.f, 0.f};
      if constexpr (DIN <= 16) {
      {
        constexpr uint32_t TSTEP = 32 * DIN * 2;
        const int in = min(i + 1, i1 - 1);
        const uint32_t wcap = (uint32_t)in * A.JDp * DIN * 2, bcap = (uint32_t)in * A.JDp * 8;
        const uint32_t xvn = x_voff<DIN>(in, A.N, A.lpad, A.T, A.F, f, ftt, fvalid, h, A.zero_off);
        f4 vv[4];
        auto dots = [&](int t) {
#pragma unroll
          for (int q = 0; q < 4; ++q) {
            const int k = kpart<DOUT>(t, 4 * q);
            P2[k] += f2{u[t][4 * q], u[t][4 * q + 1]} * f2{vv[q].x, vv[q].y};
            P2[k] += f2{u[t][4 * q + 2], u[t][4 * q + 3]} * f2{vv[q].z, vv[q].w};
          }
        };
#pragma unroll
        for (int t = 0; t < TW; ++t) {
          if (t > 0) {
#pragma unroll
            for (int q = 0; q < 4; ++q) vv[q] = vcl[((t - 1) * 4 + q) * 64 + lane];
          }
          __builtin_amdgcn_sched_barrier(0);
          u[t] = pose_chain<DIN>(fr.a[t], fr.b, mfma32(fr.bias[t], ones, f16v{}));
          __builtin_amdgcn_sched_barrier(0);
          fetch_w<DIN>(rs, wvo + t * TSTEP, h, A.wplane_b, wcap, fr.a[t]);
          {
            const auto v2 = __builtin_amdgcn_raw_buffer_load_b64(rs.b, bvo + t * 32 * 8, bcap, 0);
            fr.bias[t] = __builtin_bit_cast(bf8, (unsigned __attribute__((ext_vector_type(4)))){v2[0], v2[1], 0u, 0u});
          }
          if (t == TW - 1) fetch_x<DIN>(rs, xvn, h, A.xplane_b, A.zero_off, fr.b);
          __builtin_amdgcn_sched_barrier(0);
          if (t > 0) dots(t - 1);
          __builtin_amdgcn_sched_barrier(0);
        }
#pragma unroll
        for (int q = 0; q < 4; ++q) vv[q] = vcl[((TW - 1) * 4 + q) * 64 + lane];
        dots(TW - 1);
      }
      } else {
      const int in = min(i + 1, i1 - 1);
      pose_prog<DIN, TW, XJ, XJ>(fr, ones, u, rs, wvo, bvo,
                                 x_voff<DIN>(in, A.N, A.lpad, A.T, A.F, f, ftt, fvalid, h, A.zero_off), h,
                                 A.wplane_b, A.xplane_b, A.zero_off, (uint32_t)in * A.JDp * DIN * 2,
                                 (uint32_t)in * A.JDp * 8, xbuf(i) + lane * 16);
#pragma unroll
      for (int t = 0; t < TW; ++t)
#pragma unroll
        for (int q = 0; q < 4; ++q) {
          const f4 vv = vcl[(t * 4 + q) * 64 + lane];
          const int k = kpart<DOUT>(t, 4 * q);
          P2[k] += f2{u[t][4 * q], u[t][4 * q + 1]} * f2{vv.x, vv.y};
          P2[k] += f2{u[t][4 * q + 2], u[t][4 * q + 3]} * f2{vv.z, vv.w};
        }
      }
      float L[OWN], e[OWN];
      float m = -1e30f;
#pragma unroll
      for (int a = 0; a < OWN; ++a) {
        const float pa = P2[2 * a].x + P2[2 * a].y, pb = P2[2 * a + 1].x + P2[2 * a + 1].y;
        const auto sw = __builtin_amdgcn_permlane32_swap(__float_as_uint(pa), __float_as_uint(pb), false, false);
        L[a] = (__uint_as_float(sw[0]) + __uint_as_float(sw[1])) * inv + mk[a];
        m = fmaxf(m, L[a]);
      }
      float z = 0.f;
#pragma unroll
      for (int a = 0; a < OWN; ++a) {
        e[a] = __expf(L[a] - m);
        z += e[a];
      }
      float M, Z;
      {
        float m0, m1, z0, z1;
        xpair32(m, m0, m1);
        xpair32(z, z0, z1);
        M = fmaxf(m0, m1);
        Z = z0 * __expf(m0 - M) + z1 * __expf(m1 - M);
      }
      if constexpr (NW > 1) {
        int lid;
        asm volatile("v_mbcnt_lo_u32_b32 %0, -1, 0\n\tv_mbcnt_hi_u32_b32 %0, -1, %0" : "=v"(lid));
        const int sr = lid & 31, sh = lid >> 5;
        float2* slot = st + par * NW * 32;
        if (sh == 0) slot[wvu * 32 + sr] = make_float2(M, Z);
        if constexpr (XJ) xl_wait<5 * TW + OWN + 1>();
        __syncthreads();
        if constexpr (XJ) x_dma(xs_b, A.xplane_b, xsrc(i + 2), wv, xbuf(i + 2));
        constexpr int HW = NW / 2;
        float2 sv[HW];
#pragma unroll
        for (int w = 0; w < HW; ++w) sv[w] = slot[(sh * HW + w) * 32 + sr];
        float mh = sv[0].x;
#pragma unroll
        for (int w = 1; w < HW; ++w) mh = fmaxf(mh, sv[w].x);
        float zh = 0.f;
#pragma unroll
        for (int w = 0; w < HW; ++w) zh += sv[w].y * __expf(sv[w].x - mh);
        float m0, m1, z0, z1;
        xpair32(mh, m0, m1);
        xpair32(zh, z0, z1);
        const float MM = fmaxf(m0, m1);
        Z = z0 * __expf(m0 - MM) + z1 * __expf(m1 - MM);
        M = MM;
        par ^= 1;
      }
      __builtin_amdgcn_sched_barrier(0);
      const float sc = __expf(m - M) * __builtin_amdgcn_rcpf(Z);
      {
#pragma unroll
        for (int a = 0; a < OWN; ++a)
          bstore(crs, fvalid ? e[a] * sc : 0.f, (uint32_t)((j0 + h + 2 * a) * A.Fs + f) * 4u,
                 (uint32_t)i * A.JP * A.Fs * 4u);
        bstore(lzs, M + __builtin_amdgcn_logf(Z) * 0.69314718f, (h == 0 && wv == 0 && fvalid) ? (uint32_t)f * 4u : kNoStore,
               (uint32_t)i * A.Fs * 4u);
      }
      float c[CP];
#pragma unroll
      for (int a = 0; a < OWN; ++a) {
        float c0, c1;
        xpair32(e[a] * sc, c0, c1);
        c[2 * a] = c0;
        c[2 * a + 1] = c1;
      }
#pragma unroll
      for (int t = 0; t < TW; ++t)
#pragma unroll
        for (int v = 0; v < 16; v += 2) {
          const float cv = c[kpart<DOUT>(t, v)];
          f2 a2 = {acc[t][v], acc[t][v + 1]};
          a2 += f2{cv, cv} * f2{u[t][v], u[t][v + 1]};
          acc[t][v] = a2.x;
          acc[t][v + 1] = a2.y;
        }
    }
  }
  {
    const auto* K = kernarg_reload<Args32>(0);
    const int JD = K->J * DOUT;
    const int le = lane_asm(), fe = ft * 32 + (le & 31), he = le >> 5;
    float* const sl = K->slab + (size_t)sg.slot * A.F * JD;
#pragma unroll
    for (int t = 0; t < TW; ++t)
#pragma unroll
      for (int q = 0; q < 4; ++q) {
        const int row = (tbase + t) * 32 + 8 * q + 4 * he;
        if (fe < A.F && row < JD) {
          f4 v = {acc[t][4 * q], acc[t][4 * q + 1], acc[t][4 * q + 2], acc[t][4 * q + 3]};
          *reinterpret_cast<f4*>(sl + (size_t)fe * JD + row) = v * inv;
        }
      }
  }
  if (!sw.next(sg)) break;
  }
}


template <int DIN, int DOUT, int NW, int TW>
__global__ __launch_bounds__(64 * NW) __attribute__((amdgpu_waves_per_eu(kWavesPerEU))) void route_fwd32p_kernel(Args32 A) {
  constexpr int CP = TW * 32 / DOUT;
  constexpr int OWN = CP / 2;
  static_assert(NW > 1, "the pipelined pass exchanges softmax stats between waves");
  extern __shared__ __attribute__((aligned(16))) float lds[];
  const int lane = threadIdx.x & 63, wv = threadIdx.x >> 6;
  const int r = lane & 31, h = lane >> 5;
  const int tbase = __builtin_amdgcn_readfirstlane(wv * TW);
  const int j0 = tbase * 32 / DOUT;
  const Rsrc3 rs{make_rsrc(A.Ws, A.ws_bytes), make_rsrc(A.bs, A.bs_bytes), make_rsrc(A.xs, A.xs_bytes)};
  const uint32_t wvo = (uint32_t)(((tbase * 32 + r) * DIN + (DIN >= 16 ? 8 * h : 0)) * 2);
  const uint32_t bvo = (uint32_t)((tbase * 32 + r) * 8);
  const __amdgpu_buffer_rsrc_t crs = make_rsrc(A.cst, A.cst ? (size_t)A.in_n * A.JP * A.Fs * 4 : 0);
  const __amdgpu_buffer_rsrc_t lzs = make_rsrc(A.lzst, A.cst ? (size_t)A.in_n * A.Fs * 4 : 0);
  float2* st = reinterpret_cast<float2*>(lds);
  constexpr bool XL = DIN == 32;
  f4 vcr[TW][4];
  __shared__ __attribute__((aligned(16))) char xls[XL ? 2 * 4 * kXlPiece : 16];
  char* xb = xls;
  const char* xs_b = static_cast<const char*>(A.xs);
  auto xbuf = [&](int c) { return xb + (c & 1) * 4 * kXlPiece; };
  for (SegWalk sw(A);;) {
  const Seg32 sg = sw.seg();
  const int ft = sg.ft, i0 = sg.i0, i1 = sg.i1;
  const int JD = kernarg_reload<Args32>(0)->J * DOUT;
  const int f = ft * 32 + r;
  const int fc = min(f, A.F - 1);
  const int fb = fc / A.T, ftt = fc - fb * A.T;
  const bool fvalid = f < A.F;
  auto xsrc = [&](int c) { return x_voff<DIN>(min(c, i1 - 1), A.N, A.lpad, A.T, A.F, f, ftt, fvalid, h, A.zero_off); };
#pragma unroll
  for (int t = 0; t < TW; ++t)
#pragma unroll
    for (int q = 0; q < 4; ++q) {
      const int row = (tbase + t) * 32 + 8 * q + 4 * h;
      f4 v = {0.f, 0.f, 0.f, 0.f};
      if (fvalid && row < JD) v = *reinterpret_cast<const f4*>(kernarg_reload<Args32>(0)->vc + (size_t)f * JD + row);
      vcr[t][q] = v;
    }
  float mk[OWN];
#pragma unroll
  for (int a = 0; a < OWN; ++a) {
    const int j = j0 + 2 * a + h;
    mk[a] = (j < A.J && !(A.mask_first && j == 0)) ? 0.f : -INFINITY;
  }
  const bf8 ones = ones_frag(h);
  const float inv = A.hdr[0];
  f16v acc[TW];
#pragma unroll
  for (int t = 0; t < TW; ++t) acc[t] = f16v{};
  if (i0 < i1) {
    Frags32<DIN, TW> fr;
    fetch32<DIN, TW, true>(rs, wvo, bvo, x_voff<DIN>(i0, A.N, A.lpad, A.T, A.F, f, ftt, fvalid, h, A.zero_off), h,
                           A.wplane_b, A.xplane_b, A.zero_off, (uint32_t)i0 * A.JDp * DIN * 2, (uint32_t)i0 * A.JDp * 8,
                           fr);
    f16v uc[TW], un[TW];
    float e[OWN], m;
    if constexpr (XL) {
      x_dma(xs_b, A.xplane_b, xsrc(i0 + 1), wv, xbuf(i0 + 1));
      x_dma(xs_b, A.xplane_b, xsrc(i0 + 2), wv, xbuf(i0 + 2));
      xl_wait();
      __syncthreads();
    }
    auto logits = [&](const f16v (&u)[TW], int slot_par) {
      f2 P2[CP];
#pragma unroll
      for (int k = 0; k < CP; ++k) P2[k] = f2{0.f, 0.f};
#pragma unroll
      for (int t = 0; t < TW; ++t)
#pragma unroll
        for (int q = 0; q < 4; ++q) {
          const f4 vv = vcr[t][q];
          const int k = kpart<DOUT>(t, 4 * q);
          P2[k] += f2{u[t][4 * q], u[t][4 * q + 1]} * f2{vv.x, vv.y};
          P2[k] += f2{u[t][4 * q + 2], u[t][4 * q + 3]} * f2{vv.z, vv.w};
        }
      float L[OWN];
      m = -1e30f;
#pragma unroll
      for (int a = 0; a < OWN; ++a) {
        const float pa = P2[2 * a].x + P2[2 * a].y, pb = P2[2 * a + 1].x + P2[2 * a + 1].y;
        const auto sw = __builtin_amdgcn_permlane32_swap(__float_as_uint(pa), __float_as_uint(pb), false, false);
        L[a] = (__uint_as_float(sw[0]) + __uint_as_float(sw[1])) * inv + mk[a];
        m = fmaxf(m, L[a]);
      }
      float z = 0.f;
#pragma unroll
      for (int a = 0; a < OWN; ++a) {
        e[a] = __expf(L[a] - m);
        z += e[a];
      }
      float m0, m1, z0, z1;
      xpair32(m, m0, m1);
      xpair32(z, z0, z1);
      const float M = fmaxf(m0, m1);
      const float Z = z0 * __expf(m0 - M) + z1 * __expf(m1 - M);
      if (h == 0) st[(slot_par * NW + wv) * 32 + r] = make_float2(M, Z);
    };
    int par = 0;
    pose_prog<DIN, TW, XL>(fr, ones, uc, rs, wvo, bvo,
                           x_voff<DIN>(min(i0 + 1, i1 - 1), A.N, A.lpad, A.T, A.F, f, ftt, fvalid, h, A.zero_off), h,
                           A.wplane_b, A.xplane_b, A.zero_off, (uint32_t)min(i0 + 1, i1 - 1) * A.JDp * DIN * 2,
                           (uint32_t)min(i0 + 1, i1 - 1) * A.JDp * 8, xbuf(i0 + 1) + lane * 16);
    logits(uc, par);
    __syncthreads();
    auto step_il = [&](int i, f16v (&ucur)[TW], f16v (&unext)[TW]) __attribute__((always_inline)) {
      if constexpr (DIN == 32) {
      const bool more = i + 1 < i1;
      x_dma(xs_b, A.xplane_b, xsrc(i + 3), wv, xbuf(i + 3));
      constexpr int HW = NW / 2;
      float2 sv[HW];
      float M, Z, sc;
      float c[CP];
      auto cfma = [&](int t0, int t1) __attribute__((always_inline)) {
#pragma unroll
        for (int t = t0; t < t1; ++t) {
#pragma unroll
          for (int v = 0; v < 16; ++v) acc[t][v] = fmaf(c[kpart<DOUT>(t, v)], ucur[t][v], acc[t][v]);
          asm volatile("" : "+v"(acc[t]));
        }
      };
      auto fill = [&](auto stage) __attribute__((always_inline)) {
        constexpr int S = decltype(stage)::value;
        if constexpr (S == 0) {
          const float2* slot = st + par * NW * 32;
#pragma unroll
          for (int w = 0; w < HW; ++w) sv[w] = slot[(h * HW + w) * 32 + r];
        } else if constexpr (S == 1) {
          float mh = sv[0].x;
#pragma unroll
          for (int w = 1; w < HW; ++w) mh = fmaxf(mh, sv[w].x);
          float zh = 0.f;
#pragma unroll
          for (int w = 0; w < HW; ++w) zh += sv[w].y * __expf(sv[w].x - mh);
          float m0, m1, z0, z1;
          xpair32(mh, m0, m1);
          xpair32(zh, z0, z1);
          M = fmaxf(m0, m1);
          Z = z0 * __expf(m0 - M) + z1 * __expf(m1 - M);
          sc = __expf(m - M) * __builtin_amdgcn_rcpf(Z);
        } else if constexpr (S == 2) {
#pragma unroll
          for (int a = 0; a < OWN; ++a)
            bstore(crs, fvalid ? e[a] * sc : 0.f, (uint32_t)((j0 + h + 2 * a) * A.Fs + f) * 4u,
                   (uint32_t)i * A.JP * A.Fs * 4u);
          bstore(lzs, M + __builtin_amdgcn_logf(Z) * 0.69314718f,
                 (h == 0 && wv == 0 && fvalid) ? (uint32_t)f * 4u : kNoStore, (uint32_t)i * A.Fs * 4u);
#pragma unroll
          for (int a = 0; a < OWN; ++a) {
            float c0, c1;
            xpair32(e[a] * sc, c0, c1);
            c[2 * a] = c0;
            c[2 * a + 1] = c1;
          }
          cfma(0, TW / 2);
        } else {
          cfma(TW / 2, TW);
        }
      };
      {
        const int in = min(i + 2, i1 - 1);
        pose_prog32i<TW, 6, 6, 5>(fr, ones, unext, rs, wvo, bvo, A.wplane_b, (uint32_t)in * A.JDp * DIN * 2,
                                  (uint32_t)in * A.JDp * 8, xbuf(i + 2) + lane * 16, fill);
      }
      if (more) {
        par ^= 1;
        logits(unext, par);
        xl_wait<5 * TW + OWN + 1>();
        __syncthreads();
      }
      }
    };
    auto step = [&](int i, f16v (&ucur)[TW], f16v (&unext)[TW]) __attribute__((always_inline)) {
      const bool more = i + 1 < i1;
      if constexpr (XL)
        x_dma(xs_b, A.xplane_b, xsrc(i + 3), wv, xbuf(i + 3));
      if (more) {
        const int in = min(i + 2, i1 - 1);
        pose_prog<DIN, TW, XL>(fr, ones, unext, rs, wvo, bvo,
                               x_voff<DIN>(in, A.N, A.lpad, A.T, A.F, f, ftt, fvalid, h, A.zero_off), h, A.wplane_b,
                               A.xplane_b, A.zero_off, (uint32_t)in * A.JDp * DIN * 2, (uint32_t)in * A.JDp * 8,
                               xbuf(i + 2) + lane * 16);
      }
      float M, Z;
      {
        constexpr int HW = NW / 2;
        const float2* slot = st + par * NW * 32;
        float2 sv[HW];
#pragma unroll
        for (int w = 0; w < HW; ++w) sv[w] = slot[(h * HW + w) * 32 + r];
        float mh = sv[0].x;
#pragma unroll
        for (int w = 1; w < HW; ++w) mh = fmaxf(mh, sv[w].x);
        float zh = 0.f;
#pragma unroll
        for (int w = 0; w < HW; ++w) zh += sv[w].y * __expf(sv[w].x - mh);
        float m0, m1, z0, z1;
        xpair32(mh, m0, m1);
        xpair32(zh, z0, z1);
        M = fmaxf(m0, m1);
        Z = z0 * __expf(m0 - M) + z1 * __expf(m1 - M);
      }
      const float sc = __expf(m - M) * __builtin_amdgcn_rcpf(Z);
#pragma unroll
      for (int a = 0; a < OWN; ++a)
        bstore(crs, fvalid ? e[a] * sc : 0.f, (uint32_t)((j0 + h + 2 * a) * A.Fs + f) * 4u,
               (uint32_t)i * A.JP * A.Fs * 4u);
      bstore(lzs, M + __builtin_amdgcn_logf(Z) * 0.69314718f, (h == 0 && wv == 0 && fvalid) ? (uint32_t)f * 4u : kNoStore,
             (uint32_t)i * A.Fs * 4u);
      float c[CP];
#pragma unroll
      for (int a = 0; a < OWN; ++a) {
        float c0, c1;
        xpair32(e[a] * sc, c0, c1);
        c[2 * a] = c0;
        c[2 * a + 1] = c1;
      }
#pragma unroll
      for (int t = 0; t < TW; ++t)
#pragma unroll
        for (int v = 0; v < 16; v += 2) {
          const float cv = c[kpart<DOUT>(t, v)];
          f2 a2 = {acc[t][v], acc[t][v + 1]};
          a2 += f2{cv, cv} * f2{ucur[t][v], ucur[t][v + 1]};
          acc[t][v] = a2.x;
          acc[t][v + 1] = a2.y;
        }
      if (more) {
        par ^= 1;
        logits(unext, par);
        if constexpr (XL) xl_wait<5 * TW + OWN + 1>();
        __syncthreads();
      }
    };
    if constexpr (XL && SRF_DR_IL) {
      for (int i = i0; i < i1; i += 2) {
        step_il(i, uc, un);
        if (i + 1 < i1) step_il(i + 1, un, uc);
      }
    } else {
      for (int i = i0; i < i1; i += 2) {
        step(i, uc, un);
        if (i + 1 < i1) step(i + 1, un, uc);
      }
    }
    if constexpr (XL) xl_wait();
  }
  {
    const auto* K = kernarg_reload<Args32>(0);
    const int JD = K->J * DOUT;
    const int le = lane_asm(), fe = ft * 32 + (le & 31), he = le >> 5;
    float* const sl = K->slab + (size_t)sg.slot * A.F * JD;
#pragma unroll
    for (int t = 0; t < TW; ++t)
#pragma unroll
      for (int q = 0; q < 4; ++q) {
        const int row = (tbase + t) * 32 + 8 * q + 4 * he;
        if (fe < A.F && row < JD) {
          f4 v = {acc[t][4 * q], acc[t][4 * q + 1], acc[t][4 * q + 2], acc[t][4 * q + 3]};
          *reinterpret_cast<f4*>(sl + (size_t)fe * JD + row) = v * inv;
        }
      }
  }
  if (!sw.next(sg)) break;
  }
}

struct Bwd32Args {
  const float* cst;
  const float* lz;
  const float* gs;
  float* stats;
  float* glst;
};

template <int OWN>
__device__ __forceinline__ void load_c(const float* __restrict__ p, size_t fs, float (&c)[OWN]) {
#pragma unroll
  for (int a = 0; a < OWN; ++a) c[a] = p[2 * a * fs];
}

template <int DIN, int DOUT, int NW, int TW>
__global__ __launch_bounds__(64 * NW) __attribute__((amdgpu_waves_per_eu(kWavesPerEU))) void route_bwd32_kernel(
    Args32 A, Bwd32Args Bk) {
  constexpr int CP = TW * 32 / DOUT;
  constexpr int OWN = CP / 2;
  extern __shared__ __attribute__((aligned(16))) float lds[];
  const int wv = threadIdx.x >> 6;
  const int wvu = __builtin_amdgcn_readfirstlane(wv);
  const int tbase = __builtin_amdgcn_readfirstlane(wv * TW);
  const int j0 = tbase * 32 / DOUT;
  const Rsrc3 rs{make_rsrc(A.Ws, A.ws_bytes), make_rsrc(A.bs, A.bs_bytes), make_rsrc(A.xs, A.xs_bytes)};
  if (DIN <= 16 && NW > 1 && wv >= NW / 2) __builtin_amdgcn_s_setprio(1);
  const __amdgpu_buffer_rsrc_t lzr = make_rsrc(Bk.lz, (size_t)A.in_n * A.Fs * 4);

  f4* gsl = reinterpret_cast<f4*>(lds) + (size_t)tbase * 4 * 64;
  float* st = lds + (size_t)NW * TW * 4 * 64 * 4;
  constexpr bool XJ = DIN == 32 && NW > 1;
  __shared__ __attribute__((aligned(16))) char xls[XJ ? 2 * 4 * kXlPiece : 16];
  const char* xs_b = static_cast<const char*>(A.xs);
  auto xbuf = [&](int c) { return xls + (c & 1) * 4 * kXlPiece; };
  for (SegWalk sw(A);;) {
  const Seg32 sg = sw.seg();
  const int ft = sg.ft, i0 = sg.i0, i1 = sg.i1;
  const int lane = lane_asm(), r = lane & 31, h = lane >> 5;
  const uint32_t wvo = (uint32_t)(((tbase * 32 + r) * DIN + (DIN >= 16 ? 8 * h : 0)) * 2);
  const uint32_t bvo = (uint32_t)((tbase * 32 + r) * 8);
  const int JD = kernarg_reload<Args32>(0)->J * DOUT;
  const int Tk = kernarg_reload<Args32>(0)->T;
  const int f = ft * 32 + r;
  const int fc = min(f, A.F - 1);
  const int fb = fc / Tk, ftt = fc - fb * Tk;
  const bool fvalid = f < A.F;
  auto xsrc = [&](int c) { return x_voff<DIN>(min(c, i1 - 1), A.N, A.lpad, A.T, A.F, f, ftt, fvalid, h, A.zero_off); };
#pragma unroll
  for (int t = 0; t < TW; ++t)
#pragma unroll
    for (int q = 0; q < 4; ++q) {
      const int row = (tbase + t) * 32 + 8 * q + 4 * h;
      f4 v = {0.f, 0.f, 0.f, 0.f};
      if (fvalid && row < JD) v = *reinterpret_cast<const f4*>(kernarg_reload<Bwd32Args>(sizeof(Args32))->gs + (size_t)f * JD + row);
      gsl[(t * 4 + q) * 64 + lane] = v;
    }
  const bf8 ones = ones_frag(h);
  const float inv = A.hdr[0];
  f16v acc[TW];
#pragma unroll
  for (int t = 0; t < TW; ++t) acc[t] = f16v{};
  const float* crow = Bk.cst + (size_t)(j0 + h) * A.Fs + fc;
  const __amdgpu_buffer_rsrc_t sts = make_rsrc(Bk.stats, (size_t)A.F * A.in_n * 8);
  const size_t cstep = (size_t)A.JP * A.Fs;
  int par = 0;
  if (i0 < i1) {
    Frags32<DIN, TW> fr;
    fetch32<DIN, TW, true>(rs, wvo, bvo, x_voff<DIN>(i0, A.N, A.lpad, A.T, A.F, f, ftt, fvalid, h, A.zero_off), h,
                           A.wplane_b, A.xplane_b, A.zero_off, (uint32_t)i0 * A.JDp * DIN * 2, (uint32_t)i0 * A.JDp * 8,
                           fr);
    if constexpr (XJ) {
      x_dma(xs_b, A.xplane_b, xsrc(i0), wv, xbuf(i0));
      x_dma(xs_b, A.xplane_b, xsrc(i0 + 1), wv, xbuf(i0 + 1));
      xl_wait();
      __syncthreads();
    }
    for (int i = i0; i < i1; ++i) {
      f16v u[TW];
      f2 P2[CP];
#pragma unroll
      for (int k = 0; k < CP; ++k) P2[k] = f2{0.f, 0.f};
      float cc[OWN];
      if constexpr (DIN <= 16) {
      load_c<OWN>(crow + (size_t)i * cstep, A.Fs, cc);
      {
        constexpr uint32_t TSTEP = 32 * DIN * 2;
        const int in = min(i + 1, i1 - 1);
        const uint32_t wcap = (uint32_t)in * A.JDp * DIN * 2, bcap = (uint32_t)in * A.JDp * 8;
        const uint32_t xvn = x_voff<DIN>(in, A.N, A.lpad, A.T, A.F, f, ftt, fvalid, h, A.zero_off);
        f4 gq[4];
        auto dots = [&](int t) {
#pragma unroll
          for (int q = 0; q < 4; ++q) {
            const int k = kpart<DOUT>(t, 4 * q);
            P2[k] += f2{u[t][4 * q], u[t][4 * q + 1]} * f2{gq[q].x, gq[q].y};
            P2[k] += f2{u[t][4 * q + 2], u[t][4 * q + 3]} * f2{gq[q].z, gq[q].w};
          }
        };
#pragma unroll
        for (int t = 0; t < TW; ++t) {
          if (t > 0) {
#pragma unroll
            for (int q = 0; q < 4; ++q) gq[q] = gsl[((t - 1) * 4 + q) * 64 + lane];
          }
          __builtin_amdgcn_sched_barrier(0);
          u[t] = pose_chain<DIN>(fr.a[t], fr.b, mfma32(fr.bias[t], ones, f16v{}));
          __builtin_amdgcn_sched_barrier(0);
          fetch_w<DIN>(rs, wvo + t * TSTEP, h, A.wplane_b, wcap, fr.a[t]);
          {
            const auto v2 = __builtin_amdgcn_raw_buffer_load_b64(rs.b, bvo + t * 32 * 8, bcap, 0);
            fr.bias[t] = __builtin_bit_cast(bf8, (unsigned __attribute__((ext_vector_type(4)))){v2[0], v2[1], 0u, 0u});
          }
          if (t == TW - 1) fetch_x<DIN>(rs, xvn, h, A.xplane_b, A.zero_off, fr.b);
          __builtin_amdgcn_sched_barrier(0);
          if (t > 0) dots(t - 1);
          __builtin_amdgcn_sched_barrier(0);
        }
#pragma unroll
        for (int q = 0; q < 4; ++q) gq[q] = gsl[((TW - 1) * 4 + q) * 64 + lane];
        dots(TW - 1);
      }
      } else {
      const int in = min(i + 1, i1 - 1);
      pose_prog<DIN, TW, XJ, XJ>(fr, ones, u, rs, wvo, bvo,
                                 x_voff<DIN>(in, A.N, A.lpad, A.T, A.F, f, ftt, fvalid, h, A.zero_off), h,
                                 A.wplane_b, A.xplane_b, A.zero_off, (uint32_t)in * A.JDp * DIN * 2,
                                 (uint32_t)in * A.JDp * 8, xbuf(i) + lane_asm() * 16);
      load_c<OWN>(crow + (size_t)i * cstep, A.Fs, cc);
#pragma unroll
      for (int t = 0; t < TW; ++t)
#pragma unroll
        for (int q = 0; q < 4; ++q) {
          const f4 gv = gsl[(t * 4 + q) * 64 + lane];
          const int k = kpart<DOUT>(t, 4 * q);
          P2[k] += f2{u[t][4 * q], u[t][4 * q + 1]} * f2{gv.x, gv.y};
          P2[k] += f2{u[t][4 * q + 2], u[t][4 * q + 3]} * f2{gv.z, gv.w};
        }
      }
      float Q[OWN];
      float sp = 0.f;
#pragma unroll
      for (int a = 0; a < OWN; ++a) {
        const float pa = P2[2 * a].x + P2[2 * a].y, pb = P2[2 * a + 1].x + P2[2 * a + 1].y;
        const auto sw = __builtin_amdgcn_permlane32_swap(__float_as_uint(pa), __float_as_uint(pb), false, false);
        Q[a] = (__uint_as_float(sw[0]) + __uint_as_float(sw[1])) * inv;
        sp += cc[a] * Q[a];
      }
      float S;
      {
        float s0, s1;
        xpair32(sp, s0, s1);
        S = s0 + s1;
      }
      if constexpr (NW > 1) {
        int lid;
        asm volatile("v_mbcnt_lo_u32_b32 %0, -1, 0\n\tv_mbcnt_hi_u32_b32 %0, -1, %0" : "=v"(lid));
        const int sr = lid & 31, shf = lid >> 5;
        float* slot = st + par * NW * 32;
        if (shf == 0) slot[wvu * 32 + sr] = S;
        if constexpr (XJ) xl_wait();
        __syncthreads();
        if constexpr (XJ) x_dma(xs_b, A.xplane_b, xsrc(i + 2), wv, xbuf(i + 2));
        constexpr int HW = NW / 2;
        float sh = 0.f;
#pragma unroll
        for (int w = 0; w < HW; ++w) sh += slot[(shf * HW + w) * 32 + sr];
        float s0, s1;
        xpair32(sh, s0, s1);
        S = s0 + s1;
        par ^= 1;
      }
      const float lzv =
          __builtin_bit_cast(float, __builtin_amdgcn_raw_buffer_load_b32(lzr, (uint32_t)fc * 4u, (uint32_t)i * A.Fs * 4u, 0));
      __builtin_amdgcn_sched_barrier(0);
      {
        __builtin_amdgcn_raw_buffer_store_b64(
            (unsigned __attribute__((ext_vector_type(2)))){__float_as_uint(lzv), __float_as_uint(S)}, sts,
            (wv == 0 && h == 0 && fvalid) ? (uint32_t)(f * A.in_n) * 8u : kNoStore, (uint32_t)i * 8u, 0);
      }
      float gown[OWN];
#pragma unroll
      for (int a = 0; a < OWN; ++a) gown[a] = cc[a] * (Q[a] - S);
      {
        float* dst = Bk.glst + ((size_t)i * A.JP + j0 + h) * A.Fs + f;
#pragma unroll
        for (int a = 0; a < OWN; ++a) dst[(size_t)2 * a * A.Fs] = fvalid ? gown[a] : 0.f;
      }
      float g[CP];
#pragma unroll
      for (int a = 0; a < OWN; ++a) {
        float g0, g1;
        xpair32(gown[a], g0, g1);
        g[2 * a] = g0;
        g[2 * a + 1] = g1;
      }
#pragma unroll
      for (int t = 0; t < TW; ++t)
#pragma unroll
        for (int v = 0; v < 16; v += 2) {
          const float gv = g[kpart<DOUT>(t, v)];
          f2 a2 = {acc[t][v], acc[t][v + 1]};
          a2 += f2{gv, gv} * f2{u[t][v], u[t][v + 1]};
          acc[t][v] = a2.x;
          acc[t][v + 1] = a2.y;
        }
    }
  }
  {
    const auto* K = kernarg_reload<Args32>(0);
    const int JD = K->J * DOUT;
    const int le = lane_asm(), fe = ft * 32 + (le & 31), he = le >> 5;
    float* const sl = K->slab + (size_t)sg.slot * A.F * JD;
#pragma unroll
    for (int t = 0; t < TW; ++t)
#pragma unroll
      for (int q = 0; q < 4; ++q) {
        const int row = (tbase + t) * 32 + 8 * q + 4 * he;
        if (fe < A.F && row < JD) {
          f4 v = {acc[t][4 * q], acc[t][4 * q + 1], acc[t][4 * q + 2], acc[t][4 * q + 3]};
          *reinterpret_cast<f4*>(sl + (size_t)fe * JD + row) = v * inv;
        }
      }
  }
  if (!sw.next(sg)) break;
  }
}


template <int DIN, int DOUT, int NW, int TW>
__global__ __launch_bounds__(64 * NW) __attribute__((amdgpu_waves_per_eu(kWavesPerEU))) void route_bwd32p_kernel(
    Args32 A, Bwd32Args Bk) {
  constexpr int CP = TW * 32 / DOUT;
  constexpr int OWN = CP / 2;
  static_assert(NW > 1, "the pipelined pass exchanges sigma partials between waves");
  extern __shared__ __attribute__((aligned(16))) float lds[];
  const int lane = threadIdx.x & 63, wv = threadIdx.x >> 6;
  const int r = lane & 31, h = lane >> 5;
  const int tbase = __builtin_amdgcn_readfirstlane(wv * TW);
  const int j0 = tbase * 32 / DOUT;
  const Rsrc3 rs{make_rsrc(A.Ws, A.ws_bytes), make_rsrc(A.bs, A.bs_bytes), make_rsrc(A.xs, A.xs_bytes)};
  const uint32_t wvo = (uint32_t)(((tbase * 32 + r) * DIN + (DIN >= 16 ? 8 * h : 0)) * 2);
  const uint32_t bvo = (uint32_t)((tbase * 32 + r) * 8);
  f4* gsl = reinterpret_cast<f4*>(lds) + (size_t)wv * TW * 4 * 64;
  float* st = lds + (size_t)NW * TW * 4 * 64 * 4;
  constexpr bool XL = DIN == 32;
  __shared__ __attribute__((aligned(16))) char xls[XL ? 2 * 4 * kXlPiece : 16];
  char* xb = xls;
  const char* xs_b = static_cast<const char*>(A.xs);
  auto xbuf = [&](int c) { return xb + (c & 1) * 4 * kXlPiece; };
  for (SegWalk sw(A);;) {
  const Seg32 sg = sw.seg();
  const int ft = sg.ft, i0 = sg.i0, i1 = sg.i1;
  const int JD = kernarg_reload<Args32>(0)->J * DOUT;
  const int f = ft * 32 + r;
  const int fc = min(f, A.F - 1);
  const int fb = fc / A.T, ftt = fc - fb * A.T;
  const bool fvalid = f < A.F;
  auto xsrc = [&](int c) { return x_voff<DIN>(min(c, i1 - 1), A.N, A.lpad, A.T, A.F, f, ftt, fvalid, h, A.zero_off); };
#pragma unroll
  for (int t = 0; t < TW; ++t)
#pragma unroll
    for (int q = 0; q < 4; ++q) {
      const int row = (tbase + t) * 32 + 8 * q + 4 * h;
      f4 v = {0.f, 0.f, 0.f, 0.f};
      if (fvalid && row < JD) v = *reinterpret_cast<const f4*>(kernarg_reload<Bwd32Args>(sizeof(Args32))->gs + (size_t)f * JD + row);
      gsl[(t * 4 + q) * 64 + lane] = v;
    }
  const bf8 ones = ones_frag(h);
  const float inv = A.hdr[0];
  f16v acc[TW];
#pragma unroll
  for (int t = 0; t < TW; ++t) acc[t] = f16v{};
  const float* crow = Bk.cst + (size_t)(j0 + h) * A.Fs + fc;
  const __amdgpu_buffer_rsrc_t sts = make_rsrc(Bk.stats, (size_t)A.F * A.in_n * 8);
  const size_t cstep = (size_t)A.JP * A.Fs;
  if (i0 < i1) {
    Frags32<DIN, TW> fr;
    fetch32<DIN, TW, true>(rs, wvo, bvo, x_voff<DIN>(i0, A.N, A.lpad, A.T, A.F, f, ftt, fvalid, h, A.zero_off), h,
                           A.wplane_b, A.xplane_b, A.zero_off, (uint32_t)i0 * A.JDp * DIN * 2, (uint32_t)i0 * A.JDp * 8,
                           fr);
    f16v uc[TW], un[TW];
    float cc[OWN], cn[OWN], Q[OWN];
    auto dots = [&](const f16v (&u)[TW], const float (&c)[OWN], int slot_par) {
      f2 P2[CP];
#pragma unroll
      for (int k = 0; k < CP; ++k) P2[k] = f2{0.f, 0.f};
#pragma unroll
      for (int t = 0; t < TW; ++t)
#pragma unroll
        for (int q = 0; q < 4; ++q) {
          const f4 gv = gsl[(t * 4 + q) * 64 + lane];
          const int k = kpart<DOUT>(t, 4 * q);
          P2[k] += f2{u[t][4 * q], u[t][4 * q + 1]} * f2{gv.x, gv.y};
          P2[k] += f2{u[t][4 * q + 2], u[t][4 * q + 3]} * f2{gv.z, gv.w};
        }
      float sp = 0.f;
#pragma unroll
      for (int a = 0; a < OWN; ++a) {
        const float pa = P2[2 * a].x + P2[2 * a].y, pb = P2[2 * a + 1].x + P2[2 * a + 1].y;
        const auto sw = __builtin_amdgcn_permlane32_swap(__float_as_uint(pa), __float_as_uint(pb), false, false);
        Q[a] = (__uint_as_float(sw[0]) + __uint_as_float(sw[1])) * inv;
        sp += c[a] * Q[a];
      }
      float s0, s1;
      xpair32(sp, s0, s1);
      if (h == 0) st[(slot_par * NW + wv) * 32 + r] = s0 + s1;
    };
    int par = 0;
    if constexpr (XL) {
      x_dma(xs_b, A.xplane_b, xsrc(i0 + 1), wv, xbuf(i0 + 1));
      x_dma(xs_b, A.xplane_b, xsrc(i0 + 2), wv, xbuf(i0 + 2));
      xl_wait();
      __syncthreads();
    }
    load_c<OWN>(crow + (size_t)i0 * cstep, A.Fs, cc);
    pose_prog<DIN, TW, XL>(fr, ones, uc, rs, wvo, bvo,
                           x_voff<DIN>(min(i0 + 1, i1 - 1), A.N, A.lpad, A.T, A.F, f, ftt, fvalid, h, A.zero_off), h,
                           A.wplane_b, A.xplane_b, A.zero_off, (uint32_t)min(i0 + 1, i1 - 1) * A.JDp * DIN * 2,
                           (uint32_t)min(i0 + 1, i1 - 1) * A.JDp * 8, xbuf(i0 + 1) + lane * 16);
    dots(uc, cc, par);
    __syncthreads();
    auto step_il = [&](int i, f16v (&ucur)[TW], f16v (&unext)[TW], float (&ccur)[OWN], float (&cnext)[OWN])
        __attribute__((always_inline)) {
      if constexpr (DIN == 32) {
      const bool more = i + 1 < i1;
      x_dma(xs_b, A.xplane_b, xsrc(i + 3), wv, xbuf(i + 3));
      const float lzv = Bk.lz[(size_t)i * A.Fs + fc];
      load_c<OWN>(crow + (size_t)min(i + 1, i1 - 1) * cstep, A.Fs, cnext);
      constexpr int HW = NW / 2;
      float sv[HW];
      float g[CP];
      auto gfma = [&](int t0, int t1) __attribute__((always_inline)) {
#pragma unroll
        for (int t = t0; t < t1; ++t) {
#pragma unroll
          for (int v = 0; v < 16; ++v) acc[t][v] = fmaf(g[kpart<DOUT>(t, v)], ucur[t][v], acc[t][v]);
          asm volatile("" : "+v"(acc[t]));
        }
      };
      auto fill = [&](auto stage) __attribute__((always_inline)) {
        constexpr int S = decltype(stage)::value;
        if constexpr (S == 0) {
          const float* slot = st + par * NW * 32;
#pragma unroll
          for (int w = 0; w < HW; ++w) sv[w] = slot[(h * HW + w) * 32 + r];
        } else if constexpr (S == 1) {
          float sh = 0.f;
#pragma unroll
          for (int w = 0; w < HW; ++w) sh += sv[w];
          float s0, s1;
          xpair32(sh, s0, s1);
          const float Sg = s0 + s1;
          __builtin_amdgcn_raw_buffer_store_b64(
              (unsigned __attribute__((ext_vector_type(2)))){__float_as_uint(lzv), __float_as_uint(Sg)}, sts,
              (wv == 0 && h == 0 && fvalid) ? (uint32_t)(f * A.in_n) * 8u : kNoStore, (uint32_t)i * 8u, 0);
          float gown[OWN];
#pragma unroll
          for (int a = 0; a < OWN; ++a) gown[a] = ccur[a] * (Q[a] - Sg);
          float* dst = Bk.glst + ((size_t)i * A.JP + j0 + h) * A.Fs + f;
#pragma unroll
          for (int a = 0; a < OWN; ++a) dst[(size_t)2 * a * A.Fs] = fvalid ? gown[a] : 0.f;
#pragma unroll
          for (int a = 0; a < OWN; ++a) {
            float g0, g1;
            xpair32(gown[a], g0, g1);
            g[2 * a] = g0;
            g[2 * a + 1] = g1;
          }
        } else if constexpr (S == 2) {
          gfma(0, TW / 2);
        } else {
          gfma(TW / 2, TW);
        }
      };
      {
        const int in = min(i + 2, i1 - 1);
        pose_prog32i<TW, 4, 6, 6>(fr, ones, unext, rs, wvo, bvo, A.wplane_b, (uint32_t)in * A.JDp * DIN * 2,
                                  (uint32_t)in * A.JDp * 8, xbuf(i + 2) + lane * 16, fill);
      }
      if (more) {
        par ^= 1;
        dots(unext, cnext, par);
        xl_wait<1 + OWN + 5 * TW + 1 + OWN>();
        __syncthreads();
      }
      }
    };
    auto step = [&](int i, f16v (&ucur)[TW], f16v (&unext)[TW], float (&ccur)[OWN], float (&cnext)[OWN])
        __attribute__((always_inline)) {
      const bool more = i + 1 < i1;
      if constexpr (XL)
        x_dma(xs_b, A.xplane_b, xsrc(i + 3), wv, xbuf(i + 3));
      const float lzv = Bk.lz[(size_t)i * A.Fs + fc];
      {
        load_c<OWN>(crow + (size_t)min(i + 1, i1 - 1) * cstep, A.Fs, cnext);
        const int in = min(i + 2, i1 - 1);
        pose_prog<DIN, TW, XL>(fr, ones, unext, rs, wvo, bvo,
                               x_voff<DIN>(in, A.N, A.lpad, A.T, A.F, f, ftt, fvalid, h, A.zero_off), h, A.wplane_b,
                               A.xplane_b, A.zero_off, (uint32_t)in * A.JDp * DIN * 2, (uint32_t)in * A.JDp * 8,
                               xbuf(i + 2) + lane * 16);
      }
      float S;
      {
        constexpr int HW = NW / 2;
        const float* slot = st + par * NW * 32;
        float sh = 0.f;
#pragma unroll
        for (int w = 0; w < HW; ++w) sh += slot[(h * HW + w) * 32 + r];
        float s0, s1;
        xpair32(sh, s0, s1);
        S = s0 + s1;
      }
      __builtin_amdgcn_raw_buffer_store_b64(
          (unsigned __attribute__((ext_vector_type(2)))){__float_as_uint(lzv), __float_as_uint(S)}, sts,
          (wv == 0 && h == 0 && fvalid) ? (uint32_t)(f * A.in_n) * 8u : kNoStore, (uint32_t)i * 8u, 0);
      float gown[OWN];
#pragma unroll
      for (int a = 0; a < OWN; ++a) gown[a] = ccur[a] * (Q[a] - S);
      {
        float* dst = Bk.glst + ((size_t)i * A.JP + j0 + h) * A.Fs + f;
#pragma unroll
        for (int a = 0; a < OWN; ++a) dst[(size_t)2 * a * A.Fs] = fvalid ? gown[a] : 0.f;
      }
      float g[CP];
#pragma unroll
      for (int a = 0; a < OWN; ++a) {
        float g0, g1;
        xpair32(gown[a], g0, g1);
        g[2 * a] = g0;
        g[2 * a + 1] = g1;
      }
#pragma unroll
      for (int t = 0; t < TW; ++t)
#pragma unroll
        for (int v = 0; v < 16; v += 2) {
          const float gv = g[kpart<DOUT>(t, v)];
          f2 a2 = {acc[t][v], acc[t][v + 1]};
          a2 += f2{gv, gv} * f2{ucur[t][v], ucur[t][v + 1]};
          acc[t][v] = a2.x;
          acc[t][v + 1] = a2.y;
        }
      if (more) {
        par ^= 1;
        dots(unext, cnext, par);
        if constexpr (XL) xl_wait<1 + OWN + 5 * TW + 1 + OWN>();
        __syncthreads();
      }
    };
    if constexpr (XL && SRF_DR_IL) {
      for (int i = i0; i < i1; i += 2) {
        step_il(i, uc, un, cc, cn);
        if (i + 1 < i1) step_il(i + 1, un, uc, cn, cc);
      }
    } else {
      for (int i = i0; i < i1; i += 2) {
        step(i, uc, un, cc, cn);
        if (i + 1 < i1) step(i + 1, un, uc, cn, cc);
      }
    }
    if constexpr (XL) xl_wait();
  }
  {
    const auto* K = kernarg_reload<Args32>(0);
    const int JD = K->J * DOUT;
    const int le = lane_asm(), fe = ft * 32 + (le & 31), he = le >> 5;
    float* const sl = K->slab + (size_t)sg.slot * A.F * JD;
#pragma unroll
    for (int t = 0; t < TW; ++t)
#pragma unroll
      for (int q = 0; q < 4; ++q) {
        const int row = (tbase + t) * 32 + 8 * q + 4 * he;
        if (fe < A.F && row < JD) {
          f4 v = {acc[t][4 * q], acc[t][4 * q + 1], acc[t][4 * q + 2], acc[t][4 * q + 3]};
          *reinterpret_cast<f4*>(sl + (size_t)fe * JD + row) = v * inv;
        }
      }
  }
  if (!sw.next(sg)) break;
  }
}

}

namespace srf {

bool fwd32_supported(int din, int dout, int J) {
  return (din == 8 || din == 16 || din == 32) && (dout == 8 || dout == 16 || dout == 32) && din <= dout &&
         J * dout <= 32 * kTW * kMaxNW && (J * dout) % 8 == 0;
}

static int plan_tw(int din, int JD) {
  if (din <= 16) return JD <= 128 ? 2 : kTW;
  return (din == 32 && JD <= 32 * 2 * kMaxNW) ? 2 : kTW;
}

static Fwd32Shape fwd32_shape(const DrGeom& g) {
  Fwd32Shape p;
  const int NT = (g.JD() + 31) / 32;
  p.TW = plan_tw(g.din, g.JD());
  p.NW = 1;
  while (p.NW * p.TW < NT) p.NW *= 2;
  p.JDp = p.NW * p.TW * 32;
  p.xpad = g.din == 32 ? 32 : 16;
  p.n_ftiles = (g.F() + 31) / 32;
  p.xplane = (size_t)g.F() * g.N * g.din + p.xpad;
  p.ws_w = srf::align_up((size_t)2 * g.in_n() * p.JDp * g.din * 2, 256);
  p.ws_b = srf::align_up((size_t)g.in_n() * p.JDp * 4 * 2, 256);
  p.ws_x = srf::align_up((size_t)2 * p.xplane * 2, 256);
  p.ws_h = (size_t)(2 * kAbsBlocks + 64) * 4;
  return p;
}

Fwd32Plan fwd32_plan(const DrGeom& g, int n_chunks) {
  Fwd32Plan p;
  static_cast<Fwd32Shape&>(p) = fwd32_shape(g);
  const int in_n = g.in_n(), JD = g.JD(), F = g.F(), din = g.din, n_ftiles = p.n_ftiles;
  constexpr int kSegCost = 3;
  const int per_cu = std::max(1, std::min(8 / p.NW, (int)(160 * 1024 / fwd32_lds(p))));
  const int slots = p.NW > 1 ? 256 * per_cu : 1024;
  int best = 1;
  double best_cost = 1e30;
  const bool force_bal = n_chunks > 0 && (n_chunks & kBalFlag) != 0;
  const int forced = force_bal ? 0 : n_chunks;
  for (int c = 1; c <= std::min(in_n, 96); ++c) {
    const int rounds = (n_ftiles * c + slots - 1) / slots;
    const int len = (in_n + c - 1) / c;
    double cost = (double)rounds * (len + kSegCost) * (1.0 + 0.002 * c);
    if (forced > 0) cost = (c == std::min(forced, in_n)) ? 0.0 : 1.0;
    if (cost < best_cost) {
      best_cost = cost;
      best = c;
    }
  }
  p.n_chunks = best;
  p.chunk_len = (in_n + best - 1) / best;
  p.bal_G = 0;
  p.bal_U = 0;
  p.n_slots = best;
  p.plan_arg = best;
  {
    const long long U = (long long)n_ftiles * in_n;
    long long G = force_bal ? (n_chunks & (kBalFlag - 1)) : 0;
    if (G <= 0) G = slots;
    G = std::min(G, U);
    const bool fits = U * (G + 1) < (1ll << 31);
    if (fits && forced <= 0) {
      const int len = (int)((U + G - 1) / G);
      const int segs = (len - 1 + in_n - 1) / in_n + 1;
      int n_slots = 1;
      for (int ft = 0; ft < n_ftiles; ++ft) n_slots = std::max(n_slots, bal_tile_slots(ft, in_n, (int)U, (int)G));
      const double cost = (double)(len + kSegCost * segs) * (1.0 + 0.002 * n_slots);
      if (force_bal || (SRF_DR_BAL_AUTO && din == 32 && p.NW > 1 && p.TW == 2 && cost < best_cost)) {
        p.bal_G = (int)G;
        p.bal_U = (int)U;
        p.n_slots = n_slots;
        p.plan_arg = kBalFlag | (int)G;
      }
    }
  }
  p.ws_bsum = srf::align_up((size_t)best * JD * 4, 256);
  p.ws_slab = srf::align_up((size_t)std::max(best, p.n_slots) * F * JD * 4, 256);
  return p;
}

const float* fwd32_hdr(const Fwd32Shape& p, const void* planes) {
  return reinterpret_cast<const float*>(static_cast<const char*>(planes) + p.ws_w + p.ws_b + p.ws_x);
}
size_t fwd32_planes_bytes(const Fwd32Shape& p) { return p.ws_w + p.ws_b + p.ws_x + p.ws_h; }
size_t fwd32_scratch_bytes(const Fwd32Split& p) { return p.ws_bsum + p.ws_slab; }
size_t fwd32_workspace(const Fwd32Plan& p) { return fwd32_planes_bytes(p) + fwd32_scratch_bytes(p); }
float* fwd32_slab(const Fwd32Split& p, void* scratch) {
  return reinterpret_cast<float*>(static_cast<char*>(scratch) + p.ws_bsum);
}

size_t fwd32_lds(const Fwd32Shape& p) {
  return (size_t)p.NW * p.TW * 4 * 64 * 16 + (p.NW > 1 ? (size_t)2 * 32 * p.NW * 8 : 0);
}

int fwd32_prepare(const Fwd32Plan& p, const DrGeom& g, const float* emb, const float* W, const float* bias,
                  void* planes, void* scratch, float* WT, float* xT, hipStream_t st, bool wt16, bool xt16) {
  char* base = static_cast<char*>(planes);
  float* hdr = reinterpret_cast<float*>(base + p.ws_w + p.ws_b + p.ws_x);
  const int din = g.din;
  hipLaunchKernelGGL(absmax_kernel, dim3(kAbsBlocks, 2), dim3(kAbsThreads), 0, st, W,
                     (size_t)g.in_n() * g.JD() * din, emb, (size_t)g.F() * g.N * din, hdr + 64);
  SRF_LAUNCH_CHECK("absmax");
  PrepArgs P;
  P.W = W;
  P.bias = bias;
  P.emb = emb;
  P.Ws = reinterpret_cast<_Float16*>(base);
  P.bs = reinterpret_cast<__bf16*>(base + p.ws_w);
  P.xs = reinterpret_cast<_Float16*>(base + p.ws_w + p.ws_b);
  P.part = hdr + 64;
  P.hdr = hdr;
  P.bsum = reinterpret_cast<float*>(scratch);
  P.WT = WT;
  P.xT = xT;
  P.T = g.T;
  P.lpad = g.lpad;
  P.Fp = (g.F() + 15) / 16 * 16;
  P.in_n = g.in_n();
  P.JD = g.JD();
  P.JDp = p.JDp;
  P.din = din;
  P.n_chunks = p.n_chunks;
  P.chunk_len = p.chunk_len;
  P.F = g.F();
  P.N = g.N;
  P.xplane = p.xplane;
  P.n_a = (size_t)P.in_n * p.JDp * din / 8;
  P.n_b = (size_t)P.in_n * p.JDp;
  P.n_c = (size_t)p.n_chunks * P.JD;
  P.n_d = p.xplane / 8;
  SRF_REQUIRE(!wt16 || din == 32, "prep32: split W^T planes need din 32, got %d", din);
  P.wt16 = wt16 ? 1 : 0;
  SRF_REQUIRE(!xt16 || din == 32, "prep32: split x^T planes need din 32, got %d", din);
  P.xt16 = xt16 ? 1 : 0;
  P.n_e = WT ? (size_t)P.in_n * ((P.JD + 15) / 16) * (wt16 ? 2 : 4) * din : 0;
  P.rpad = g.rpad;
  P.n_xblk = P.n_wblk = P.w_bpc = 0;
  P.n_f = P.xt_block0 = 0;
  if (SRF_PREP32_ONEPASS && din == 32 && (!WT || wt16) && (!xT || xt16) && P.JD % 8 == 0 &&
      g.lpad + g.rpad <= kXHaloMax) {
    const size_t n_xblk = (size_t)((P.F + kXtTile - 1) / kXtTile) * P.N;
    P.w_bpc = (P.JDp + 255) / 256;
    const size_t n_wblk = (size_t)P.in_n * P.w_bpc;
    const size_t n_blk = n_xblk + n_wblk + (P.n_b + P.n_c + 255) / 256;
    SRF_REQUIRE(n_blk < (1ull << 31), "prep32: %zu blocks", n_blk);
    P.n_xblk = (int)n_xblk;
    P.n_wblk = (int)n_wblk;
    hipLaunchKernelGGL(prep32_onepass_kernel, dim3((unsigned)n_blk), dim3(256), 0, st, P);
    SRF_LAUNCH_CHECK("prep32_onepass");
    return SRF_OK;
  }
  SRF_REQUIRE(din <= 32, "prep32: xT tile holds din <= 32, got %d", din);
  P.n_f = xT ? (size_t)P.in_n * ((P.Fp + kXtTile - 1) / kXtTile) : 0;
  P.xt_block0 = (P.n_a + P.n_b + P.n_c + P.n_d + P.n_e + 255) / 256;
  hipLaunchKernelGGL(prep32_kernel, dim3(P.xt_block0 + P.n_f), dim3(256), 0, st, P);
  SRF_LAUNCH_CHECK("prep32");
  return SRF_OK;
}

template <int V>
using Int = std::integral_constant<int, V>;

template <class Fn>
static int dispatch_row(const DrGeom& g, const char* what, Fn&& fn) {
  if (g.din == g.dout) {
    switch (g.din) {
      case 8: return fn(Int<8>{}, Int<8>{});
      case 16: return fn(Int<16>{}, Int<16>{});
      case 32: return fn(Int<32>{}, Int<32>{});
    }
  }
  srf::set_error("%s: unsupported din %d dout %d", what, g.din, g.dout);
  return SRF_EUNSUPPORTED;
}

template <int DIN, class Fn>
static int dispatch_tiles(const Fwd32Shape& p, Fn&& fn) {
  if (p.TW == 2) {
    if constexpr (DIN <= 16) {
      return p.NW == 1 ? fn(Int<1>{}, Int<2>{}) : fn(Int<2>{}, Int<2>{});
    } else {
      switch (p.NW) {
        case 1: return fn(Int<1>{}, Int<2>{});
        case 2: return fn(Int<2>{}, Int<2>{});
        case 4: return fn(Int<4>{}, Int<2>{});
        default: return fn(Int<8>{}, Int<2>{});
      }
    }
  }
  switch (p.NW) {
    case 1: return fn(Int<1>{}, Int<kTW>{});
    case 2: return fn(Int<2>{}, Int<kTW>{});
    case 4: return fn(Int<4>{}, Int<kTW>{});
    default: return fn(Int<kMaxNW>{}, Int<kTW>{});
  }
}

template <int NW, int TW, class Kern, class... Args>
static int launch_rpass(const Fwd32Plan& p, const char* name, Kern piped, Kern plain, hipStream_t st,
                        const Args&... args) {
  const size_t lds = fwd32_lds(p);
  const Kern kern = (NW > 1 && TW <= 2) ? piped : plain;
  if (lds > 64 * 1024)
    SRF_HIP_TRY(hipFuncSetAttribute((const void*)kern, hipFuncAttributeMaxDynamicSharedMemorySize, (int)lds));
  hipLaunchKernelGGL(kern, dim3(p.bal_G > 0 ? p.bal_G : p.n_ftiles * p.n_chunks), dim3(64 * NW), lds, st, args...);
  SRF_LAUNCH_CHECK(name);
  return SRF_OK;
}

static Args32 make_args32(const Fwd32Plan& p, const DrGeom& g, const void* planes, void* scratch) {
  const int in_n = g.in_n();
  const char* base = static_cast<const char*>(planes);
  Args32 a{};
  a.Ws = base;
  a.bs = base + p.ws_w;
  a.xs = base + p.ws_w + p.ws_b;
  a.hdr = reinterpret_cast<const float*>(base + p.ws_w + p.ws_b + p.ws_x);
  a.ws_bytes = p.ws_w;
  a.bs_bytes = (size_t)in_n * p.JDp * 8;
  a.xs_bytes = 2 * p.xplane * 2;
  a.wplane_b = (uint32_t)((size_t)in_n * p.JDp * g.din * 2);
  a.xplane_b = (uint32_t)(p.xplane * 2);
  a.zero_off = (uint32_t)((p.xplane - p.xpad) * 2);
  a.F = g.F();
  a.T = g.T;
  a.N = g.N;
  a.lpad = g.lpad;
  a.in_n = in_n;
  a.J = g.J;
  a.JDp = p.JDp;
  a.n_chunks = p.n_chunks;
  a.chunk_len = p.chunk_len;
  a.mask_first = g.mask_first;
  a.n_tgroups = p.NW;
  a.vc = nullptr;
  a.bsum = reinterpret_cast<const float*>(scratch);
  a.slab = fwd32_slab(p, scratch);
  a.cst = nullptr;
  a.lzst = nullptr;
  a.JP = p.JDp / g.dout;
  a.Fs = fwd32_frame_stride(g.F());
  a.bal_G = p.bal_G;
  a.bal_U = p.bal_U;
  return a;
}

Fwd32Cpl fwd32_cpl_layout(const Fwd32Shape& p, const DrGeom& g) {
  Fwd32Cpl c{};
  const size_t in_n = g.in_n();
  const size_t blk = (size_t)fwd32_frame_stride(g.F()) * in_n;
  const int R1 = std::max(g.iters - 1, 0);
  c.c = 0;
  c.lz = (size_t)R1 * blk * (p.JDp / g.dout);
  size_t off = c.lz + (size_t)R1 * blk;
  off = (off + 63) / 64 * 64;
  c.planes = off;
  off += (fwd32_planes_bytes(p) + 255) / 256 * 64;
  c.WT = off;
  off += (in_n * g.din * ((g.JD() + 15) / 16 * 16) + 63) / 64 * 64;
  c.xT = off;
  off += (in_n * g.din * ((g.F() + 15) / 16 * 16) + 63) / 64 * 64;
  c.total = off;
  return c;
}

bool fwd32_first_full_supported(const Fwd32Shape& p, const DrGeom& g) {
  return g.din == 32 && g.dout == 32 && p.JDp % kFfBM == 0;
}

#ifndef SRF_FF_BN
#define SRF_FF_BN 0
#endif
static int ff_frames(int n_rt, int F) {
  if (SRF_FF_BN) return SRF_FF_BN;
  int dev = 0, cus = 256;
  if (hipGetDevice(&dev) != hipSuccess || hipDeviceGetAttribute(&cus, hipDeviceAttributeMultiprocessorCount, dev) != hipSuccess)
    cus = 256;
  for (int bn : {192, 128, 96})
    if ((long)n_rt * ((F + bn - 1) / bn) >= cus * 9 / 10) return bn;
  return 64;
}

int fwd32_first_full(const Fwd32Plan& p, const DrGeom& g, const void* planes, void* scratch, float* s_out,
                     float* vc_out, float* v_out, hipStream_t st) {
  SRF_REQUIRE(fwd32_first_full_supported(p, g), "fwd32_first_full: din %d dout %d JDp %d", g.din, g.dout, p.JDp);
  SRF_REQUIRE(2 * p.xplane * 2 < (1ull << 31) && p.ws_w < (1ull << 31), "fwd32: operand planes exceed 2 GiB");
  const Args32 a = make_args32(p, g, planes, scratch);
  const int bn = ff_frames(p.JDp / kFfBM, g.F());
  const int nb = (p.JDp / kFfBM) * ((g.F() + bn - 1) / bn);
#define SRF_FF_LAUNCH(BN)                                                                                          \
  if (bn == BN) {                                                                                                 \
    constexpr int CPS_ = BN >= 96 ? 2 : 1;                                                                        \
    const size_t lds = 2 * CPS_ * (size_t)ff_stage<BN>();                                                        \
    if (lds > 64 * 1024)                                                                                          \
      SRF_HIP_TRY(hipFuncSetAttribute((const void*)route_fwd32_first_full_kernel<BN, CPS_>,                       \
                                      hipFuncAttributeMaxDynamicSharedMemorySize, (int)lds));                      \
    hipLaunchKernelGGL((route_fwd32_first_full_kernel<BN, CPS_>), dim3(nb), dim3(64 * 2 * (BN / 32)), lds, st, a, \
                       s_out, vc_out, v_out);                                                                     \
  }
  SRF_FF_LAUNCH(64)
  SRF_FF_LAUNCH(96)
  SRF_FF_LAUNCH(128)
  SRF_FF_LAUNCH(192)
#undef SRF_FF_LAUNCH
  SRF_LAUNCH_CHECK("route_fwd32_first_full");
  return SRF_OK;
}

int fwd32_pass(const Fwd32Plan& p, const DrGeom& g, bool first, const void* planes, void* scratch, const float* vc,
               float* cst, float* lzst, hipStream_t st) {
  Args32 a = make_args32(p, g, planes, scratch);
  a.vc = vc;
  a.cst = first ? nullptr : cst;
  a.lzst = first ? nullptr : lzst;
  SRF_REQUIRE(2 * p.xplane * 2 < (1ull << 31) && p.ws_w < (1ull << 31), "fwd32: operand planes exceed 2 GiB");
  return dispatch_row(g, "fwd32", [&](auto di, auto dout) {
    if (first) {
      Args32 b = a;
      b.n_tgroups = p.JDp / (32 * kFTW);
      const int tasks = (p.n_ftiles + kFFB - 1) / kFFB * b.n_tgroups * p.n_chunks;
      hipLaunchKernelGGL((route_fwd32_first_kernel<di, dout>), dim3((tasks + 3) / 4), dim3(256), 0, st, b);
      SRF_LAUNCH_CHECK("route_fwd32_first");
      return SRF_OK;
    }
    return dispatch_tiles<di>(p, [&](auto nw, auto tw) {
      return launch_rpass<nw, tw>(p, "route_fwd32", route_fwd32p_kernel<di, dout, (nw > 1 ? nw : 2), (tw <= 2 ? tw : 2)>,
                                  route_fwd32_kernel<di, dout, nw, tw>, st, a);
    });
  });
}

int bwd32_pass(const Fwd32Plan& p, const DrGeom& g, const void* planes, void* scratch, const float* cst,
               const float* lz, const float* gs, float* stats, float* glst, hipStream_t st) {
  Args32 a = make_args32(p, g, planes, scratch);
  a.mask_first = 0;
  const Bwd32Args b{cst, lz, gs, stats, glst};
  return dispatch_row(g, "bwd32", [&](auto di, auto dout) {
    return dispatch_tiles<di>(p, [&](auto nw, auto tw) {
      return launch_rpass<nw, tw>(p, "route_bwd32", route_bwd32p_kernel<di, dout, (nw > 1 ? nw : 2), (tw <= 2 ? tw : 2)>,
                                  route_bwd32_kernel<di, dout, nw, tw>, st, a, b);
    });
  });
}

}
```

Baseline: 3.122 million frames/s.

## Drop unused log-partition and stats stores from fwd32/bwd32 route passes

Removes the per-frame log-partition (lz) store in the forward route kernels and the lz load plus stats store in the backward route kernels, which were apparently not consumed on the coupling path. The backward finish kernel now takes separate input and output accumulator pointers, so the first and last iterations skip reading or writing the A buffer and the initial zeroing store goes away. Wait counts are adjusted to match the fewer outstanding memory ops, and a c-load is moved earlier in one backward loop. The risk is that the stats buffer was still read by something downstream, and that the hand-tuned vmcnt values no longer match the issued loads.

```diff
diff --git a/srf_amd/csrc/route_dr.hip b/srf_amd/csrc/route_dr.hip
--- a/srf_amd/csrc/route_dr.hip
+++ b/srf_amd/csrc/route_dr.hip
@@ -1728,7 +1728,7 @@
 
 template <int DOUT>
 __global__ void bwd_finish_kernel(const float* __restrict__ slab, SlabSplit sp, size_t FJD,
-                                  const float* __restrict__ a_init, float* __restrict__ A,
+                                  const float* __restrict__ a_init, const float* a_in, float* a_out,
                                   const float* __restrict__ s, float* __restrict__ gs, float* __restrict__ zero4,
                                   size_t nz4, float* __restrict__ zero1) {
   constexpr int Q = DOUT / 4;
@@ -1740,10 +1740,10 @@
   f4 a;
   if (a_init) {
     a = ld4(a_init + off);
-    if (ok) st4(A + off, f4{0.f, 0.f, 0.f, 0.f});
   } else {
-    a = ld4(A + off) + sum_slab4(slab, sp, FJD, off);
-    if (ok) st4(A + off, a);
+    a = sum_slab4(slab, sp, FJD, off);
+    if (a_in) a = ld4(a_in + off) + a;
+    if (a_out && ok) st4(a_out + off, a);
   }
   const f4 sv = ld4(s + off);
   const float n2 = qsum<Q>((sv.x * sv.x + sv.y * sv.y) + (sv.z * sv.z + sv.w * sv.w));
@@ -1822,14 +1822,14 @@
 }
 
 template <int D>
-void launch_bwd_finish(const DrGeom& g, const float* slab, const SlabSplit& sp, const float* a_init, float* A,
-                       const float* s, float* gs, hipStream_t st, float* zero = nullptr, size_t n_zero = 0,
-                       float* zero1 = nullptr) {
+void launch_bwd_finish(const DrGeom& g, const float* slab, const SlabSplit& sp, const float* a_init,
+                       const float* a_in, float* a_out, const float* s, float* gs, hipStream_t st,
+                       float* zero = nullptr, size_t n_zero = 0, float* zero1 = nullptr) {
   const size_t FJD = (size_t)g.F() * g.JD();
   const size_t nz4 = zero ? n_zero / 4 : 0;
   const size_t n = std::max(FJD / 4, nz4);
   hipLaunchKernelGGL((bwd_finish_kernel<D>), dim3((n + 255) / 256), dim3(256), 0, st, slab, sp, FJD, a_init,
-                     A, s, gs, zero, nz4, zero1);
+                     a_in, a_out, s, gs, zero, nz4, zero1);
 }
 
 constexpr int gu_tw(int d) { return d >= 64 ? 4 : 2; }
@@ -2198,13 +2198,12 @@
       continue;
     }
     if (p.fwd32) {
-      float *cst = nullptr, *lzst = nullptr;
+      float* cst = nullptr;
       if (p.couplings && r > 0) {
         const size_t blk = (size_t)srf::fwd32_frame_stride(g.F()) * g.in_n();
         cst = couplings + cl.c + (size_t)(r - 1) * blk * p.JP();
-        lzst = couplings + cl.lz + (size_t)(r - 1) * blk;
-      }
-      const int rc = srf::fwd32_pass(plan, g, r == 0, planes, scratch, vc, cst, lzst, st);
+      }
+      const int rc = srf::fwd32_pass(plan, g, r == 0, planes, scratch, vc, cst, st);
       if (rc) return rc;
     } else {
       dispatch_pass<D, MODE_FWD>(g, p.pc, p.chunks, emb, W, bias, r, vc, r == 0 ? bsum : nullptr, slab, nullptr, 1, st);
@@ -2272,27 +2271,28 @@
   const bool p32 = p.couplings;
   float* const gsv = ws + w.gs;
   const size_t n_emb = (size_t)g.F() * g.N * g.din;
-  launch_bwd_finish<D>(g, nullptr, uniform_split(1), g_v, ws + w.A, saved + (size_t)(2 * (R - 1)) * FJD,
+  launch_bwd_finish<D>(g, nullptr, uniform_split(1), g_v, nullptr, nullptr, saved + (size_t)(2 * (R - 1)) * FJD,
                        gsv + (size_t)(R - 1) * FJD, st, p32 ? g_emb : nullptr, n_emb, p32 ? ws + w.gumax : nullptr);
   SRF_LAUNCH_CHECK("bwd_finish");
   for (int r = R - 1; r >= 1; --r) {
     const float* vc = saved + (size_t)(2 * (r - 1) + 1) * FJD;
     float* stats_r = ws + w.stats + (size_t)(r - 1) * g.F() * g.in_n() * 2;
+    const float* a_in = r == R - 1 ? nullptr : ws + w.A;
+    float* a_out = r == 1 ? nullptr : ws + w.A;
     if (p32) {
       const size_t blk = (size_t)srf::fwd32_frame_stride(g.F()) * g.in_n();
       const int JP = p.JP();
       const int rc = srf::bwd32_pass(plan, g, couplings + cl.planes, ws + w.p32,
-                                     couplings + cl.c + (size_t)(r - 1) * blk * JP,
-                                     couplings + cl.lz + (size_t)(r - 1) * blk, gsv + (size_t)r * FJD, stats_r,
+                                     couplings + cl.c + (size_t)(r - 1) * blk * JP, gsv + (size_t)r * FJD,
                                      ws + w.gl + (size_t)(r - 1) * blk * JP, st);
       if (rc) return rc;
-      launch_bwd_finish<D>(g, srf::fwd32_slab(plan, ws + w.p32), pass_split(g, plan), nullptr, ws + w.A,
+      launch_bwd_finish<D>(g, srf::fwd32_slab(plan, ws + w.p32), pass_split(g, plan), nullptr, a_in, a_out,
                            saved + (size_t)(2 * (r - 1)) * FJD, gsv + (size_t)(r - 1) * FJD, st);
     } else {
       dispatch_pass<D, MODE_BWD>(g, p.pc, p.chunks, emb, W, bias, r, vc, gsv + (size_t)r * FJD, ws + w.slab, stats_r, 1,
                                  st);
       SRF_LAUNCH_CHECK("route_pass(bwd)");
-      launch_bwd_finish<D>(g, ws + w.slab, uniform_split(p.chunks), nullptr, ws + w.A,
+      launch_bwd_finish<D>(g, ws + w.slab, uniform_split(p.chunks), nullptr, a_in, a_out,
                            saved + (size_t)(2 * (r - 1)) * FJD, gsv + (size_t)(r - 1) * FJD, st);
     }
     SRF_LAUNCH_CHECK("bwd_finish");
diff --git a/srf_amd/csrc/route_fwd32.h b/srf_amd/csrc/route_fwd32.h
--- a/srf_amd/csrc/route_fwd32.h
+++ b/srf_amd/csrc/route_fwd32.h
@@ -57,7 +57,7 @@
                   void* planes, void* scratch, float* WT, float* xT, hipStream_t st, bool wt16 = false,
                   bool xt16 = false);
 int fwd32_pass(const Fwd32Plan& p, const DrGeom& g, bool first, const void* planes, void* scratch, const float* vc,
-               float* cst, float* lzst, hipStream_t st);
+               float* cst, hipStream_t st);
 bool fwd32_first_full_supported(const Fwd32Shape& p, const DrGeom& g);
 int fwd32_first_full(const Fwd32Plan& p, const DrGeom& g, const void* planes, void* scratch, float* s_out,
                      float* vc_out, float* v_out, hipStream_t st);
@@ -66,6 +66,6 @@
 };
 Fwd32Cpl fwd32_cpl_layout(const Fwd32Shape& p, const DrGeom& g);
 int bwd32_pass(const Fwd32Plan& p, const DrGeom& g, const void* planes, void* scratch, const float* cst,
-               const float* lz, const float* gs, float* stats, float* glst, hipStream_t st);
+               const float* gs, float* glst, hipStream_t st);
 
 }
diff --git a/srf_amd/csrc/route_fwd32.hip b/srf_amd/csrc/route_fwd32.hip
--- a/srf_amd/csrc/route_fwd32.hip
+++ b/srf_amd/csrc/route_fwd32.hip
@@ -496,7 +496,6 @@
   return __builtin_amdgcn_make_buffer_rsrc(const_cast<void*>(p), 0, (int)bytes, 0x00020000);
 }
 
-constexpr uint32_t kNoStore = 0x80000000u;
 __device__ __forceinline__ void bstore(__amdgpu_buffer_rsrc_t rs, float v, uint32_t voff, uint32_t soff) {
   __builtin_amdgcn_raw_buffer_store_b32(__float_as_uint(v), rs, voff, soff, 0);
 }
@@ -783,7 +782,6 @@
   const float* bsum;
   float* slab;
   float* cst;
-  float* lzst;
   int JP, Fs;
   int bal_G, bal_U;
 };
@@ -960,6 +958,9 @@
 template <int K = 0>
 __device__ __forceinline__ void xl_wait() {
   asm volatile("s_waitcnt vmcnt(%0)" ::"n"(K) : "memory");
+}
+__device__ __forceinline__ void xl_wait_all() {
+  __builtin_amdgcn_s_waitcnt(0x0F70);
 }
 
 template <int BN, int CPS = 1>
@@ -1130,7 +1131,6 @@
   const Rsrc3 rs{make_rsrc(A.Ws, A.ws_bytes), make_rsrc(A.bs, A.bs_bytes), make_rsrc(A.xs, A.xs_bytes)};
   if (DIN <= 16 && NW > 1 && wv >= NW / 2) __builtin_amdgcn_s_setprio(1);
   const __amdgpu_buffer_rsrc_t crs = make_rsrc(A.cst, A.cst ? (size_t)A.in_n * A.JP * A.Fs * 4 : 0);
-  const __amdgpu_buffer_rsrc_t lzs = make_rsrc(A.lzst, A.cst ? (size_t)A.in_n * A.Fs * 4 : 0);
 
   f4* vcl = reinterpret_cast<f4*>(lds) + (size_t)tbase * 4 * 64;
   float2* st = reinterpret_cast<float2*>(lds + (size_t)NW * TW * 4 * 64 * 4);
@@ -1271,7 +1271,7 @@
         const int sr = lid & 31, sh = lid >> 5;
         float2* slot = st + par * NW * 32;
         if (sh == 0) slot[wvu * 32 + sr] = make_float2(M, Z);
-        if constexpr (XJ) xl_wait<5 * TW + OWN + 1>();
+        if constexpr (XJ) xl_wait<5 * TW + OWN>();
         __syncthreads();
         if constexpr (XJ) x_dma(xs_b, A.xplane_b, xsrc(i + 2), wv, xbuf(i + 2));
         constexpr int HW = NW / 2;
@@ -1299,8 +1299,6 @@
         for (int a = 0; a < OWN; ++a)
           bstore(crs, fvalid ? e[a] * sc : 0.f, (uint32_t)((j0 + h + 2 * a) * A.Fs + f) * 4u,
                  (uint32_t)i * A.JP * A.Fs * 4u);
-        bstore(lzs, M + __builtin_amdgcn_logf(Z) * 0.69314718f, (h == 0 && wv == 0 && fvalid) ? (uint32_t)f * 4u : kNoStore,
-               (uint32_t)i * A.Fs * 4u);
       }
       float c[CP];
 #pragma unroll
@@ -1357,7 +1355,6 @@
   const uint32_t wvo = (uint32_t)(((tbase * 32 + r) * DIN + (DIN >= 16 ? 8 * h : 0)) * 2);
   const uint32_t bvo = (uint32_t)((tbase * 32 + r) * 8);
   const __amdgpu_buffer_rsrc_t crs = make_rsrc(A.cst, A.cst ? (size_t)A.in_n * A.JP * A.Fs * 4 : 0);
-  const __amdgpu_buffer_rsrc_t lzs = make_rsrc(A.lzst, A.cst ? (size_t)A.in_n * A.Fs * 4 : 0);
   float2* st = reinterpret_cast<float2*>(lds);
   constexpr bool XL = DIN == 32;
   f4 vcr[TW][4];
@@ -1489,8 +1486,6 @@
           for (int a = 0; a < OWN; ++a)
             bstore(crs, fvalid ? e[a] * sc : 0.f, (uint32_t)((j0 + h + 2 * a) * A.Fs + f) * 4u,
                    (uint32_t)i * A.JP * A.Fs * 4u);
-          bstore(lzs, M + __builtin_amdgcn_logf(Z) * 0.69314718f,
-                 (h == 0 && wv == 0 && fvalid) ? (uint32_t)f * 4u : kNoStore, (uint32_t)i * A.Fs * 4u);
 #pragma unroll
           for (int a = 0; a < OWN; ++a) {
             float c0, c1;
@@ -1511,7 +1506,7 @@
       if (more) {
         par ^= 1;
         logits(unext, par);
-        xl_wait<5 * TW + OWN + 1>();
+        xl_wait<5 * TW + OWN>();
         __syncthreads();
       }
       }
@@ -1551,8 +1546,6 @@
       for (int a = 0; a < OWN; ++a)
         bstore(crs, fvalid ? e[a] * sc : 0.f, (uint32_t)((j0 + h + 2 * a) * A.Fs + f) * 4u,
                (uint32_t)i * A.JP * A.Fs * 4u);
-      bstore(lzs, M + __builtin_amdgcn_logf(Z) * 0.69314718f, (h == 0 && wv == 0 && fvalid) ? (uint32_t)f * 4u : kNoStore,
-             (uint32_t)i * A.Fs * 4u);
       float c[CP];
 #pragma unroll
       for (int a = 0; a < OWN; ++a) {
@@ -1574,7 +1567,7 @@
       if (more) {
         par ^= 1;
         logits(unext, par);
-        if constexpr (XL) xl_wait<5 * TW + OWN + 1>();
+        if constexpr (XL) xl_wait<5 * TW + OWN>();
         __syncthreads();
       }
     };
@@ -1613,9 +1606,7 @@
 
 struct Bwd32Args {
   const float* cst;
-  const float* lz;
   const float* gs;
-  float* stats;
   float* glst;
 };
 
@@ -1637,7 +1628,6 @@
   const int j0 = tbase * 32 / DOUT;
   const Rsrc3 rs{make_rsrc(A.Ws, A.ws_bytes), make_rsrc(A.bs, A.bs_bytes), make_rsrc(A.xs, A.xs_bytes)};
   if (DIN <= 16 && NW > 1 && wv >= NW / 2) __builtin_amdgcn_s_setprio(1);
-  const __amdgpu_buffer_rsrc_t lzr = make_rsrc(Bk.lz, (size_t)A.in_n * A.Fs * 4);
 
   f4* gsl = reinterpret_cast<f4*>(lds) + (size_t)tbase * 4 * 64;
   float* st = lds + (size_t)NW * TW * 4 * 64 * 4;
@@ -1673,7 +1663,6 @@
 #pragma unroll
   for (int t = 0; t < TW; ++t) acc[t] = f16v{};
   const float* crow = Bk.cst + (size_t)(j0 + h) * A.Fs + fc;
-  const __amdgpu_buffer_rsrc_t sts = make_rsrc(Bk.stats, (size_t)A.F * A.in_n * 8);
   const size_t cstep = (size_t)A.JP * A.Fs;
   int par = 0;
   if (i0 < i1) {
@@ -1684,7 +1673,7 @@
     if constexpr (XJ) {
       x_dma(xs_b, A.xplane_b, xsrc(i0), wv, xbuf(i0));
       x_dma(xs_b, A.xplane_b, xsrc(i0 + 1), wv, xbuf(i0 + 1));
-      xl_wait();
+      xl_wait_all();
       __syncthreads();
     }
     for (int i = i0; i < i1; ++i) {
@@ -1733,12 +1722,13 @@
         dots(TW - 1);
       }
       } else {
+      load_c<OWN>(crow + (size_t)i * cstep, A.Fs, cc);
+      __builtin_amdgcn_sched_barrier(0);
       const int in = min(i + 1, i1 - 1);
       pose_prog<DIN, TW, XJ, XJ>(fr, ones, u, rs, wvo, bvo,
                                  x_voff<DIN>(in, A.N, A.lpad, A.T, A.F, f, ftt, fvalid, h, A.zero_off), h,
                                  A.wplane_b, A.xplane_b, A.zero_off, (uint32_t)in * A.JDp * DIN * 2,
                                  (uint32_t)in * A.JDp * 8, xbuf(i) + lane_asm() * 16);
-      load_c<OWN>(crow + (size_t)i * cstep, A.Fs, cc);
 #pragma unroll
       for (int t = 0; t < TW; ++t)
 #pragma unroll
@@ -1770,7 +1760,7 @@
         const int sr = lid & 31, shf = lid >> 5;
         float* slot = st + par * NW * 32;
         if (shf == 0) slot[wvu * 32 + sr] = S;
-        if constexpr (XJ) xl_wait();
+        if constexpr (XJ) xl_wait<OWN + OWN + 5 * TW>();
         __syncthreads();
         if constexpr (XJ) x_dma(xs_b, A.xplane_b, xsrc(i + 2), wv, xbuf(i + 2));
         constexpr int HW = NW / 2;
@@ -1782,14 +1772,7 @@
         S = s0 + s1;
         par ^= 1;
       }
-      const float lzv =
-          __builtin_bit_cast(float, __builtin_amdgcn_raw_buffer_load_b32(lzr, (uint32_t)fc * 4u, (uint32_t)i * A.Fs * 4u, 0));
       __builtin_amdgcn_sched_barrier(0);
-      {
-        __builtin_amdgcn_raw_buffer_store_b64(
-            (unsigned __attribute__((ext_vector_type(2)))){__float_as_uint(lzv), __float_as_uint(S)}, sts,
-            (wv == 0 && h == 0 && fvalid) ? (uint32_t)(f * A.in_n) * 8u : kNoStore, (uint32_t)i * 8u, 0);
-      }
       float gown[OWN];
 #pragma unroll
       for (int a = 0; a < OWN; ++a) gown[a] = cc[a] * (Q[a] - S);
@@ -1884,7 +1867,6 @@
 #pragma unroll
   for (int t = 0; t < TW; ++t) acc[t] = f16v{};
   const float* crow = Bk.cst + (size_t)(j0 + h) * A.Fs + fc;
-  const __amdgpu_buffer_rsrc_t sts = make_rsrc(Bk.stats, (size_t)A.F * A.in_n * 8);
   const size_t cstep = (size_t)A.JP * A.Fs;
   if (i0 < i1) {
     Frags32<DIN, TW> fr;
@@ -1937,7 +1919,6 @@
       if constexpr (DIN == 32) {
       const bool more = i + 1 < i1;
       x_dma(xs_b, A.xplane_b, xsrc(i + 3), wv, xbuf(i + 3));
-      const float lzv = Bk.lz[(size_t)i * A.Fs + fc];
       load_c<OWN>(crow + (size_t)min(i + 1, i1 - 1) * cstep, A.Fs, cnext);
       constexpr int HW = NW / 2;
       float sv[HW];
@@ -1963,9 +1944,6 @@
           float s0, s1;
           xpair32(sh, s0, s1);
           const float Sg = s0 + s1;
-          __builtin_amdgcn_raw_buffer_store_b64(
-              (unsigned __attribute__((ext_vector_type(2)))){__float_as_uint(lzv), __float_as_uint(Sg)}, sts,
-              (wv == 0 && h == 0 && fvalid) ? (uint32_t)(f * A.in_n) * 8u : kNoStore, (uint32_t)i * 8u, 0);
           float gown[OWN];
 #pragma unroll
           for (int a = 0; a < OWN; ++a) gown[a] = ccur[a] * (Q[a] - Sg);
@@ -1993,7 +1971,7 @@
       if (more) {
         par ^= 1;
         dots(unext, cnext, par);
-        xl_wait<1 + OWN + 5 * TW + 1 + OWN>();
+        xl_wait<OWN + 5 * TW + OWN>();
         __syncthreads();
       }
       }
@@ -2003,7 +1981,6 @@
       const bool more = i + 1 < i1;
       if constexpr (XL)
         x_dma(xs_b, A.xplane_b, xsrc(i + 3), wv, xbuf(i + 3));
-      const float lzv = Bk.lz[(size_t)i * A.Fs + fc];
       {
         load_c<OWN>(crow + (size_t)min(i + 1, i1 - 1) * cstep, A.Fs, cnext);
         const int in = min(i + 2, i1 - 1);
@@ -2023,9 +2000,6 @@
         xpair32(sh, s0, s1);
         S = s0 + s1;
       }
-      __builtin_amdgcn_raw_buffer_store_b64(
-          (unsigned __attribute__((ext_vector_type(2)))){__float_as_uint(lzv), __float_as_uint(S)}, sts,
-          (wv == 0 && h == 0 && fvalid) ? (uint32_t)(f * A.in_n) * 8u : kNoStore, (uint32_t)i * 8u, 0);
       float gown[OWN];
 #pragma unroll
       for (int a = 0; a < OWN; ++a) gown[a] = ccur[a] * (Q[a] - S);
@@ -2055,7 +2029,7 @@
       if (more) {
         par ^= 1;
         dots(unext, cnext, par);
-        if constexpr (XL) xl_wait<1 + OWN + 5 * TW + 1 + OWN>();
+        if constexpr (XL) xl_wait<OWN + 5 * TW + OWN>();
         __syncthreads();
       }
     };
@@ -2333,7 +2307,6 @@
   a.bsum = reinterpret_cast<const float*>(scratch);
   a.slab = fwd32_slab(p, scratch);
   a.cst = nullptr;
-  a.lzst = nullptr;
   a.JP = p.JDp / g.dout;
   a.Fs = fwd32_frame_stride(g.F());
   a.bal_G = p.bal_G;
@@ -2404,11 +2377,10 @@
 }
 
 int fwd32_pass(const Fwd32Plan& p, const DrGeom& g, bool first, const void* planes, void* scratch, const float* vc,
-               float* cst, float* lzst, hipStream_t st) {
+               float* cst, hipStream_t st) {
   Args32 a = make_args32(p, g, planes, scratch);
   a.vc = vc;
   a.cst = first ? nullptr : cst;
-  a.lzst = first ? nullptr : lzst;
   SRF_REQUIRE(2 * p.xplane * 2 < (1ull << 31) && p.ws_w < (1ull << 31), "fwd32: operand planes exceed 2 GiB");
   return dispatch_row(g, "fwd32", [&](auto di, auto dout) {
     if (first) {
@@ -2427,10 +2399,10 @@
 }
 
 int bwd32_pass(const Fwd32Plan& p, const DrGeom& g, const void* planes, void* scratch, const float* cst,
-               const float* lz, const float* gs, float* stats, float* glst, hipStream_t st) {
+               const float* gs, float* glst, hipStream_t st) {
   Args32 a = make_args32(p, g, planes, scratch);
   a.mask_first = 0;
-  const Bwd32Args b{cst, lz, gs, stats, glst};
+  const Bwd32Args b{cst, gs, glst};
   return dispatch_row(g, "bwd32", [&](auto di, auto dout) {
     return dispatch_tiles<di>(p, [&](auto nw, auto tw) {
       return launch_rpass<nw, tw>(p, "route_bwd32", route_bwd32p_kernel<di, dout, (nw > 1 ? nw : 2), (tw <= 2 ? tw : 2)>,
```

After: 3.199 million frames/s, median of 6. +2.4%, better.
